# lauradarcy/gym-craftingworld

Hardware: AMD Instinct MI355X
Metric: env-steps/sec at 65536 envs, 1/2/4/8 MI355X; bit-exact vs CPU ref (higher is better)
Workload: dtype u8

## Files before the change

### gym_craftingworld_amd/_lib.py

```python
import ctypes as C
import os

_HERE = os.path.dirname(os.path.abspath(__file__))
LIB_PATH = os.path.join(_HERE, 'libcraftingworld.so')


def lib_path():
    return os.environ.get('CW_LIB_PATH') or LIB_PATH

CW_ABI_VERSION = 5
CW_MT_N = 624
CW_MAX_TASKS = 16
CW_MAX_MENUS = 256

CW_OK, CW_ERR_INVALID, CW_ERR_HIP, CW_ERR_STATE = 0, -1, -2, -3
CW_OBS_STATE, CW_OBS_PIXELS_FULL, CW_OBS_PIXELS_DIRTY = 0, 1, 2
CW_ACT_I32, CW_ACT_I64, CW_ACT_U8 = 0, 1, 2
CW_RASTER_RAY, CW_RASTER_ALT = 0, 1


class cw_task_menu(C.Structure):
    _fields_ = [('n_selected', C.c_int32), ('number_of_tasks', C.c_int32), ('stacking', C.c_int32),
                ('reward_subset', C.c_int32), ('selected_bits', C.c_int32 * CW_MAX_TASKS)]


class cw_config(C.Structure):
    _fields_ = [('abi_version', C.c_int32), ('num_envs', C.c_int32), ('size', C.c_int32),
                ('max_steps', C.c_int32), ('n_task_list', C.c_int32), ('fixed_init_state', C.c_int32),
                ('obs_mode', C.c_int32), ('auto_reset', C.c_int32), ('keep_terminal_obs', C.c_int32),
                ('raster', C.c_int32), ('host_outputs', C.c_int32), ('n_menus', C.c_int32),
                ('menus', C.POINTER(cw_task_menu)), ('env_menu', C.POINTER(C.c_uint8))]


class cw_buffer_table(C.Structure):
    _fields_ = [('obs', C.c_void_p), ('desired_goal', C.c_void_p), ('init_obs', C.c_void_p), ('terminal_obs', C.c_void_p),
                ('reward', C.c_void_p), ('done', C.c_void_p), ('achieved', C.c_void_p),
                ('desired', C.c_void_p), ('episode_length', C.c_void_p), ('episode_return', C.c_void_p), ('hdr', C.c_void_p),
                ('slot_pos', C.c_void_p), ('counters', C.c_void_p), ('frame_bytes', C.c_size_t),
                ('host_actions', C.c_void_p), ('host_onehot', C.c_void_p)]


class cw_state_view(C.Structure):
    _fields_ = [('grid', C.c_void_p), ('init_grid', C.c_void_p), ('goal_grid', C.c_void_p),
                ('agent_rc', C.c_void_p), ('init_agent_rc', C.c_void_p), ('goal_agent_rc', C.c_void_p),
                ('hold', C.c_void_p), ('achieved', C.c_void_p), ('desired', C.c_void_p),
                ('step_num', C.c_void_p), ('ep_no', C.c_void_p)]


class cw_profile(C.Structure):
    _fields_ = [('steps', C.c_int32), ('ms_step_kernel', C.c_float), ('ms_reset_kernel', C.c_float),
                ('ms_render_kernel', C.c_float), ('ms_render_kernel_max', C.c_float), ('ms_render_kernel_min', C.c_float),
                ('ms_render_kernel_median', C.c_float)]


class cw_tuner_state(C.Structure):
    _fields_ = [('period16', C.c_int32), ('period16_head', C.c_int32), ('period16_busy', C.c_int32), ('lookahead', C.c_int32), ('resident', C.c_int32),
                ('guard_slowdowns', C.c_int32)]


_VP = C.c_void_p
ABI = {
    'cw_create': (C.c_int, [C.POINTER(cw_config), C.c_int, C.POINTER(_VP)]),
    'cw_destroy': (C.c_int, [_VP]),
    'cw_seed_mt': (C.c_int, [_VP, _VP, _VP]),
    'cw_seed_int': (C.c_int, [_VP, _VP]),
    'cw_get_mt': (C.c_int, [_VP, _VP, _VP]),
    'cw_generate_fixed_states': (C.c_int, [_VP, _VP]),
    'cw_get_fixed_states': (C.c_int, [_VP, _VP]),
    'cw_reset': (C.c_int, [_VP, _VP]),
    'cw_step': (C.c_int, [_VP, _VP, C.c_int, _VP]),
    'cw_step_many': (C.c_int, [_VP, _VP, C.c_int, C.c_int32, _VP]),
    'cw_rollout': (C.c_int, [_VP, _VP, C.c_int32, _VP, _VP, _VP]),
    'cw_render': (C.c_int, [_VP, _VP, _VP]),
    'cw_render_onehot': (C.c_int, [_VP, _VP, C.c_int32, _VP, _VP]),
    'cw_export_grid': (C.c_int, [_VP, _VP, _VP]),
    'cw_export_onehot': (C.c_int, [_VP, _VP, _VP]),
    'cw_export_onehot_of': (C.c_int, [_VP, C.c_int, _VP, _VP]),
    'cw_get_state': (C.c_int, [_VP, C.POINTER(cw_state_view)]),
    'cw_set_state': (C.c_int, [_VP, C.POINTER(cw_state_view)]),
    'cw_checkpoint_bytes': (C.c_size_t, [_VP]),
    'cw_checkpoint_save': (C.c_int, [_VP, _VP, C.c_size_t]),
    'cw_checkpoint_load': (C.c_int, [_VP, _VP, C.c_size_t]),
    'cw_profile_begin': (C.c_int, [_VP, C.c_int]),
    'cw_profile_end': (C.c_int, [_VP, C.POINTER(cw_profile)]),
    'cw_tuner': (C.c_int, [_VP, C.POINTER(cw_tuner_state)]),
    'cw_step_resident': (C.c_int, [_VP, C.c_int32, C.c_int32]),
    'cw_resident_stop': (C.c_int, [_VP]),
    'cw_render_kernel_name': (C.c_char_p, [_VP]),
    'cw_buffers': (C.c_int, [_VP, C.POINTER(cw_buffer_table)]),
    'cw_synchronize': (C.c_int, [_VP, _VP]),
    'cw_num_envs': (C.c_int, [_VP]),
    'cw_abi_version': (C.c_int, []),
    'cw_last_error': (C.c_char_p, []),
}
class cwh_guard(C.Structure):
    _fields_ = [('rate', C.c_double), ('rate_top', C.c_double), ('ms_sum', C.c_double), ('prev_mean', C.c_double), ('ref_ms', C.c_double),
                ('ref_prev', C.c_double), ('ms_n', C.c_int32), ('late', C.c_int32), ('good', C.c_int32), ('slowdowns', C.c_int32),
                ('probes', C.c_int32), ('probe_need', C.c_int32), ('recover_need', C.c_int32), ('probing', C.c_int32), ('recovering', C.c_int32)]


class cwh_tuning(C.Structure):
    _fields_ = [(f, C.c_int32) for f in ('render_chunk_rounds', 'step_envs_per_wave', 'gather', 'gather_max_size', 'small_frame_bytes',
                                         'small_blocks_per_cu', 'small_launch_mb', 'reset_blocks_per_cu', 'guard', 'verbose', 'lookahead',
                                         'la_period', 'rollout_segment', 'pad')] + \
              [(f, C.c_double) for f in ('head_notch', 'busy_notch', 'period_ns', 'rate_tbs')]


cwh_lookup = C.CFUNCTYPE(_VP, _VP, C.c_char_p)

CWH_GUARD_NONE, CWH_GUARD_SLOWDOWN, CWH_GUARD_TRIAL_UP, CWH_GUARD_TRIAL_KEPT, CWH_GUARD_TRIAL_UNDONE = range(5)
CWH_CKPT_SECTIONS = 22

HOST_HELPERS = {
    'cwh_mt_from_numpy': (C.c_int, [_VP, C.c_int]),
    'cwh_mt_to_numpy': (None, [_VP, C.c_int, _VP]),
    'cwh_mt_init_genrand': (None, [_VP, C.c_uint32]),
    'cwh_mt_untwist': (None, [_VP]),
    'cwh_mt_rewind': (None, [_VP, C.POINTER(C.c_int32), C.c_uint32]),
    'cwh_dlpack_make': (_VP, [_VP, C.c_int, C.c_int, C.c_int, C.c_int, C.POINTER(C.c_int64)]),
    'cwh_slots_to_grid': (None, [_VP, C.c_uint32, C.c_int, _VP]),
    'cwh_ckpt_section_bytes': (C.c_int, [C.c_int64, C.c_int32, C.c_int32, C.POINTER(C.c_size_t), C.POINTER(C.c_uint64)]),
    'cwh_guard_init': (None, [C.POINTER(cwh_guard), C.c_double]),
    'cwh_guard_step': (C.c_int, [C.POINTER(cwh_guard), C.c_double, C.c_double]),
    'cwh_sweep_periods': (None, [C.c_double, C.c_int32, C.c_double, C.c_double, C.POINTER(C.c_int32), C.POINTER(C.c_int32), C.POINTER(C.c_int32)]),
    'cwh_guard_scheduled_ms': (C.c_double, [C.c_double, C.c_int32, C.c_int32, C.c_double]),
    'cwh_la_adapt': (C.c_int32, [C.c_int32, C.c_int32, C.c_uint64, C.POINTER(C.c_int32)]),
    'cwh_read_tuning': (None, [cwh_lookup, _VP, C.POINTER(cwh_tuning)]),
}


def bind_host_helpers(lib):
    for name, (res, args) in HOST_HELPERS.items():
        fn = getattr(lib, name)
        fn.restype = res
        fn.argtypes = args
    return lib

_libs = {}
_lib = None


class CraftingWorldError(RuntimeError):
    pass


def load():
    global _lib
    path = lib_path()
    if path in _libs:
        _lib = _libs[path]
        return _lib
    if not os.path.exists(path):
        raise CraftingWorldError(
            'HIP extension %s is missing; build it (python -c "import __graft_entry__ as g; g.build()"). '
            'There is no CPU fallback.' % path)
    try:
        import torch
    except ImportError:
        pass
    lib = C.CDLL(path)
    for table in (ABI, HOST_HELPERS):
        for name, (res, args) in table.items():
            fn = getattr(lib, name)
            fn.restype = res
            fn.argtypes = args
    if lib.cw_abi_version() != CW_ABI_VERSION:
        raise CraftingWorldError('%s ABI %d != binding %d' % (os.path.basename(path), lib.cw_abi_version(), CW_ABI_VERSION))
    _libs[path] = _lib = lib
    return lib


def check(rc, what, lib=None):
    if rc == CW_OK:
        return
    msg = ((lib or _lib or load()).cw_last_error() or b'').decode(errors='replace')
    if rc == CW_ERR_INVALID:
        raise ValueError('%s: %s' % (what, msg))
    raise CraftingWorldError('%s failed (%d): %s' % (what, rc, msg))
```

### gym_craftingworld_amd/csrc/cw_engine.cpp

```cpp
#include <hip/hip_runtime.h>

#include <cstdarg>
#include <climits>
#include <cstdio>
#include <cstdlib>
#include <cstring>
#include <new>
#include <algorithm>
#include <vector>

#include "../../include/craftingworld.h"
#include "cw_layout.h"
#include "cw_host.h"

extern "C" {
hipError_t cwk_launch_step(const CwParams *P, const CwTuning *T, const void *actions, int act_dtype, int obs_mode, int auto_reset, hipStream_t st,
                           hipEvent_t *ev);
hipError_t cwk_launch_refill(const CwParams *P, const CwTuning *T, int all_envs, hipStream_t st);
hipError_t cwk_launch_reset_all(const CwParams *P, const CwTuning *T, int obs_mode, hipStream_t st);
hipError_t cwk_launch_pool(const CwParams *P, const CwTuning *T, hipStream_t st);
hipError_t cwk_launch_seed(const CwParams *P, const uint32_t *seeds_dev, hipStream_t st);
hipError_t cwk_launch_resident(const CwParams *P, CwResident *R, uint32_t seq0, int paint_dirty, unsigned long long idle_ticks,
                               unsigned long long life_ticks, hipStream_t st);
hipError_t cwk_launch_render_onehot(const CwParams *P, const uint8_t *onehot, int n_states, uint16_t *out, hipStream_t st);
hipError_t cwk_launch_render_restore(const CwParams *P, const CwTuning *T, hipStream_t st);
hipError_t cwk_launch_rollout(const CwParams *P, const uint8_t *actions, int T, int32_t *rewards, uint8_t *dones, hipStream_t st);
hipError_t cwk_launch_render_ext(const CwParams *P, const CwTuning *T, uint8_t *out, hipStream_t st);
hipError_t cwk_launch_sweep_calib(const CwParams *P, const CwTuning *T, hipStream_t st);
void cwk_sweep_shape(const CwParams *P, const CwTuning *T, int *n_chunks, int *waves, int *jobs_per_wave);
hipError_t cwk_launch_idle(hipStream_t st);
hipError_t cwk_launch_export(const CwParams *P, const CwTuning *T, uint8_t *out, int onehot, int which, hipStream_t st);
}

#include <time.h>

static thread_local char g_err[512] = "";

static int fail(int code, const char *fmt, ...)
{
    va_list ap;
    va_start(ap, fmt);
    vsnprintf(g_err, sizeof(g_err), fmt, ap);
    va_end(ap);
    return code;
}

#define HIP_TRY(expr)                                                                           \
    do {                                                                                        \
        hipError_t _e = (expr);                                                                 \
        if (_e != hipSuccess)                                                                   \
            return fail(CW_ERR_HIP, "%s failed: %s (%s:%d)", #expr, hipGetErrorString(_e), __FILE__, __LINE__); \
    } while (0)

struct DeviceGuard {
    int prev = -1;
    bool ok = true;
    explicit DeviceGuard(int dev)
    {
        if (hipGetDevice(&prev) != hipSuccess) prev = -1;
        if (prev != dev) ok = (hipSetDevice(dev) == hipSuccess);
    }
    ~DeviceGuard()
    {
        int cur = -1;
        if (prev >= 0 && hipGetDevice(&cur) == hipSuccess && cur != prev) (void)hipSetDevice(prev);
    }
};

struct cw_engine {
    int device = 0;
    int obs_mode = 0;
    int auto_reset = 1;
    bool has_reset = false;
    CwParams P{};
    CwTuning tune{};
    std::vector<void *> allocs;
    std::vector<void *> host_allocs;
    int32_t *host_actions = nullptr;
    std::vector<CwMenuDev> menus;
    uint32_t *seed_scratch = nullptr;
    int n = 0, S = 0, ncell = 0, K = 0;
    CwResident *res = nullptr;
    hipStream_t res_stream = nullptr;
    bool res_running = false;
    uint32_t res_seq = 0;
    hipEvent_t last_work = nullptr;
    bool last_work_set = false;
    unsigned long long res_ticks_per_us = 100;
    std::vector<hipEvent_t> prof_ev;
    bool la_refill_all = false;
    unsigned la_steps = 0;
    unsigned la_period = 16;
    unsigned la_period_max = 16;
    bool la_adaptive = true;
    int rollout_segment = -1;
    unsigned long long *la_feedback = nullptr;
    unsigned long long la_slow_seen = 0;
    int32_t la_quiet = 0;
    bool in_step_many = false;
    bool capturing_now = false;
    int sweep_waves = 1024;
    double sweep_jobs = 0, sweep_rate = 0, sweep_beside_ms = 0;
    bool guard_on = false;
    double head_notch = 0.4, busy_notch = 0.75, tune_period_ns = -1, tune_rate_tbs = -1;
    bool tune_guard = true, tune_lookahead = true, verbose = false;
    enum { GUARD_RING = 32 };
    struct GuardSample { hipEvent_t ev[6]; int period16; } guard_ring[GUARD_RING] = {};
    unsigned guard_head = 0, guard_tail = 0;
    unsigned guard_step = 0;
    cwh_guard guard{};
    int prof_cap = 0, prof_n = 0;
    hipStream_t aux = nullptr;
    hipStream_t work[4] = {nullptr, nullptr, nullptr, nullptr};
    int n_work = 0;
    bool work_overflow = false;
    bool captured = false;
};
static inline bool stream_capturing(hipStream_t st)
{
    hipStreamCaptureStatus cap = hipStreamCaptureStatusNone;
    return hipStreamIsCapturing(st, &cap) == hipSuccess && cap != hipStreamCaptureStatusNone;
}
static inline void note_work(cw_engine *e, hipStream_t st)
{
    for (int i = 0; i < e->n_work; i++) if (e->work[i] == st) return;
    if (e->n_work < 4) e->work[e->n_work++] = st; else e->work_overflow = true;
}
static hipError_t quiesce(cw_engine *e)
{
    bool all = e->work_overflow || e->captured;
    for (int i = 0; i < e->n_work && !all; i++)
        if (hipStreamSynchronize(e->work[i]) != hipSuccess) { (void)hipGetLastError(); all = true; }
    e->n_work = 0;
    e->work_overflow = false;
    if (all) return hipDeviceSynchronize();
    return e->aux ? hipStreamSynchronize(e->aux) : hipSuccess;
}
struct AuxDrain {
    cw_engine *e;
    explicit AuxDrain(cw_engine *e_) : e(e_) {}
    ~AuxDrain() { if (e && e->aux) (void)hipStreamSynchronize(e->aux); }
};
static inline hipError_t aux_copy(cw_engine *e, void *dst, const void *src, size_t bytes, hipMemcpyKind kind)
{
    return bytes ? hipMemcpyAsync(dst, src, bytes, kind, e->aux) : hipSuccess;
}
static int la_period_for(int max_steps) { const int p = max_steps / 4; return p < 8 ? 8 : p > 64 ? 64 : p; }
static void la_adapt(cw_engine *e)
{
    const unsigned long long slow = __atomic_load_n(e->la_feedback, __ATOMIC_RELAXED);
    const unsigned long long delta = slow >= e->la_slow_seen ? slow - e->la_slow_seen : 0;
    e->la_slow_seen = slow;
    e->la_period = (unsigned)cwh_la_adapt((int32_t)e->la_period, (int32_t)e->la_period_max, delta, &e->la_quiet);
}

static int resident_park(cw_engine *e)
{
    if (!e->res_running) return CW_OK;
    const unsigned long long low = __atomic_load_n(&e->res->bell, __ATOMIC_RELAXED) & 0xFFFFFFFFull;
    __atomic_store_n(&e->res->bell, low | (1ull << 32), __ATOMIC_RELEASE);
    HIP_TRY(hipStreamSynchronize(e->res_stream));
    e->res_running = false;
    __atomic_store_n(&e->res->bell, low, __ATOMIC_RELEASE);
    __atomic_store_n(&e->res->exited, 0u, __ATOMIC_RELEASE);
    return CW_OK;
}
#define PARK(e) do { if ((e)->res_running) { const int _rc = resident_park(e); if (_rc != CW_OK) return _rc; } } while (0)


template <typename T>
static int dev_alloc(cw_engine *e, T **out, size_t count)
{
    void *p = nullptr;
    size_t bytes = count * sizeof(T);
    if (bytes == 0) bytes = 16;
    HIP_TRY(hipMalloc(&p, bytes));
    HIP_TRY(hipMemset(p, 0, bytes));
    e->allocs.push_back(p);
    *out = (T *)p;
    return CW_OK;
}

template <typename T>
static int host_alloc(cw_engine *e, T **out, size_t count)
{
    void *p = nullptr, *d = nullptr;
    size_t bytes = count * sizeof(T);
    if (bytes == 0) bytes = 16;
    HIP_TRY(hipHostMalloc(&p, bytes, hipHostMallocCoherent));
    e->host_allocs.push_back(p);
    memset(p, 0, bytes);
    HIP_TRY(hipHostGetDevicePointer(&d, p, 0));
    if (d != p) return fail(CW_ERR_HIP, "cw_create: mapped host memory has a different device address (no unified addressing)");
    *out = (T *)p;
    return CW_OK;
}

static void prof_free(cw_engine *e)
{
    for (hipEvent_t ev : e->prof_ev) (void)hipEventDestroy(ev);
    e->prof_ev.clear();
    e->prof_cap = e->prof_n = 0;
}

static int timed_render_stats(cw_engine *e, double *median, double *p90, double *mean = nullptr)
{
    enum { LAUNCHES = 24, SKIP = 4 };
    hipEvent_t evs[2 * LAUNCHES] = {};
    bool ok = true;
    for (hipEvent_t &ev : evs) ok = ok && hipEventCreate(&ev) == hipSuccess;
    for (int rep = 0; rep < LAUNCHES && ok; rep++)
        ok = hipEventRecord(evs[2 * rep], e->aux) == hipSuccess && cwk_launch_sweep_calib(&e->P, &e->tune, e->aux) == hipSuccess &&
             hipEventRecord(evs[2 * rep + 1], e->aux) == hipSuccess && cwk_launch_idle(e->aux) == hipSuccess;
    ok = ok && hipStreamSynchronize(e->aux) == hipSuccess;
    float ms[LAUNCHES];
    for (int rep = 0; rep < LAUNCHES && ok; rep++) ok = hipEventElapsedTime(&ms[rep], evs[2 * rep], evs[2 * rep + 1]) == hipSuccess;
    for (hipEvent_t &ev : evs) if (ev) (void)hipEventDestroy(ev);
    if (!ok) return fail(CW_ERR_HIP, "cw_create: render calibration failed");
    std::sort(ms + SKIP, ms + LAUNCHES);
    const int n = LAUNCHES - SKIP;
    *median = ms[SKIP + n / 2];
    *p90 = ms[SKIP + (9 * n) / 10 - 1];
    if (mean) { double acc = 0; for (int i = SKIP; i < LAUNCHES; i++) acc += ms[i]; *mean = acc / n; }
    return CW_OK;
}

static double sweep_period_ns(const cw_engine *e, double tb_per_s) { return (double)e->sweep_waves * 4096.0 / (tb_per_s * 1e12) * 1e9; }
static void set_sweep_rate(cw_engine *e, double tb_per_s)
{
    cwh_sweep_periods(tb_per_s, e->sweep_waves, e->head_notch, e->busy_notch, &e->tune.period16, &e->tune.period16_head, &e->tune.period16_busy);
}

static int calibrate_sweep(cw_engine *e)
{
    CwTuning &tn = e->tune;
    int n_chunks = 1, jobs_per_wave = 1;
    cwk_sweep_shape(&e->P, &tn, &n_chunks, &e->sweep_waves, &jobs_per_wave);
    e->sweep_jobs = (double)n_chunks * jobs_per_wave;
    if (e->tune_period_ns >= 0) {
        const double ns = e->tune_period_ns;
        set_sweep_rate(e, ns > 0 ? (double)e->sweep_waves * 4096.0 / (ns * 1e-9) * 1e-12 : 0.0);
        if (ns > 0) tn.period16 = (int)(ns * 1.6 + 0.5);
        return CW_OK;
    }
    set_sweep_rate(e, 7.0);
    if (e->host_actions) { set_sweep_rate(e, 0); return CW_OK; }
    if (e->obs_mode != CW_OBS_PIXELS_FULL || (double)e->n * e->P.frame_bytes < (double)(64ll << 20)) return CW_OK;
    static const double rates[] = {7.7, 7.4, 7.2, 7.0, 6.8, 6.6, 0.0};
    char log[1024] = "";
    size_t len = 0;
    int rc = CW_OK;
    double best_p90 = 0, med = 0, p90 = 0, mean = 0;
    rc = timed_render_stats(e, &med, &p90);
    set_sweep_rate(e, 6.4);
    if (rc == CW_OK) rc = timed_render_stats(e, &med, &p90);
    e->sweep_beside_ms = med - e->sweep_jobs * sweep_period_ns(e, 6.4) * 1e-6;
    if (e->tune_rate_tbs >= 0) e->sweep_rate = e->tune_rate_tbs;
    for (size_t i = 0; i < sizeof(rates) / sizeof(rates[0]) && rc == CW_OK && e->tune_rate_tbs < 0; i++) {
        set_sweep_rate(e, rates[i]);
        rc = timed_render_stats(e, &med, &p90, &mean);
        if (len < sizeof(log) - 56) len += (size_t)snprintf(log + len, sizeof(log) - len, " %.1f TB/s (%.0f ns): %.4f/%.4f/%.4f |", rates[i], tn.period16 / 1.6, med, p90, mean);
        if (rc == CW_OK && (best_p90 == 0 || p90 < 0.995 * best_p90)) { best_p90 = p90; e->sweep_rate = rates[i]; }
    }
    set_sweep_rate(e, e->sweep_rate);
    cwh_guard_init(&e->guard, e->sweep_rate);
    e->guard_on = rc == CW_OK && e->sweep_rate > 0 && e->auto_reset && e->tune_guard;
    if (e->guard_on)
        for (auto &smp : e->guard_ring)
            for (hipEvent_t &ev : smp.ev)
                if (hipEventCreate(&ev) != hipSuccess) e->guard_on = false;
    if (e->verbose)
        fprintf(stderr, "[craftingworld] sweep clock, ms per sweep (median/90th percentile/mean of 20; 0.0 TB/s = unclocked):%s -> %s%.0f ns\n", log,
                tn.period16 ? "" : "unclocked, ", tn.period16 / 1.6);
    return rc;
}

enum { CW_GUARD_EVERY = 64 };
static hipEvent_t *sweep_guard_tick(cw_engine *e, hipStream_t st)
{
    if (++e->guard_step % CW_GUARD_EVERY) return nullptr;
    while (e->guard_tail != e->guard_head && hipEventQuery(e->guard_ring[e->guard_tail % cw_engine::GUARD_RING].ev[5]) == hipSuccess) {
        cw_engine::GuardSample &smp = e->guard_ring[e->guard_tail++ % cw_engine::GUARD_RING];
        float ms = 0.f;
        if (hipEventElapsedTime(&ms, smp.ev[4], smp.ev[5]) != hipSuccess || ms <= 0.f || smp.period16 != e->tune.period16) continue;
        const double scheduled = cwh_guard_scheduled_ms(e->sweep_jobs, e->tune.period16, e->tune.period16_busy, e->sweep_beside_ms);
        const double rate_before = e->guard.rate, prev_mean = e->guard.prev_mean;
        const int recovering = e->guard.recovering;
        const int action = cwh_guard_step(&e->guard, ms, scheduled);
        if (e->guard.rate != rate_before) set_sweep_rate(e, e->guard.rate);
        if (e->verbose && action != CWH_GUARD_NONE) {
            static const char *what[] = {"", "three samples in a row late: a notch down", "trying a notch up", "the trial pays: kept", "the trial does not pay: undone"};
            fprintf(stderr, "[craftingworld] sweep clock: %s%s -- %.4f ms against %.4f scheduled (mean at the rate left %.4f): %.1f -> %.1f TB/s (%.0f ns)\n", what[action],
                    recovering ? " (on the way back to the best rate known)" : "", ms, scheduled, prev_mean, rate_before, e->guard.rate, e->tune.period16 / 1.6);
        }
    }
    if (e->guard_head - e->guard_tail >= (unsigned)cw_engine::GUARD_RING) return nullptr;
    cw_engine::GuardSample &slot = e->guard_ring[e->guard_head++ % cw_engine::GUARD_RING];
    slot.period16 = e->tune.period16;
    return slot.ev;
}

static void read_tuning(cw_engine *e)
{
    CwTuning &tn = e->tune;
    cwh_tuning t{};
    t.render_chunk_rounds = tn.render_chunk_rounds;
    t.step_envs_per_wave = tn.step_envs_per_wave;
    t.gather = tn.gather;
    t.gather_max_size = tn.gather_max_size;
    t.small_frame_bytes = tn.small_frame_bytes;
    t.small_blocks_per_cu = tn.small_blocks_per_cu;
    t.small_launch_mb = (int32_t)(tn.small_launch_bytes >> 20);
    t.reset_blocks_per_cu = tn.reset_blocks_per_cu;
    t.guard = 1;
    t.verbose = 0;
    t.lookahead = 1;
    t.la_period = 0;
    t.rollout_segment = e->rollout_segment;
    t.head_notch = e->head_notch;
    t.busy_notch = e->busy_notch;
    t.period_ns = -1;
    t.rate_tbs = -1;
    cwh_read_tuning([](void *, const char *k) -> const char * { return getenv(k); }, nullptr, &t);
    tn.render_chunk_rounds = t.render_chunk_rounds;
    tn.step_envs_per_wave = t.step_envs_per_wave;
    tn.gather = t.gather;
    tn.gather_max_size = t.gather_max_size;
    tn.small_frame_bytes = t.small_frame_bytes;
    tn.small_blocks_per_cu = t.small_blocks_per_cu;
    tn.small_launch_bytes = (long long)t.small_launch_mb << 20;
    tn.reset_blocks_per_cu = t.reset_blocks_per_cu;
    e->head_notch = t.head_notch;
    e->busy_notch = t.busy_notch;
    e->tune_period_ns = t.period_ns;
    e->tune_rate_tbs = t.rate_tbs;
    e->tune_guard = t.guard != 0;
    e->verbose = t.verbose != 0;
    e->tune_lookahead = t.lookahead != 0;
    e->la_adaptive = t.la_period == 0;
    e->la_period = e->la_period_max = (unsigned)(t.la_period ? t.la_period : la_period_for(e->P.max_steps));
    e->rollout_segment = t.rollout_segment;
}

extern "C" {

const char *cw_last_error(void) { return g_err; }
int cw_abi_version(void) { return CW_ABI_VERSION; }
int cw_num_envs(const cw_engine *e) { return e ? e->n : 0; }

int cw_create(const cw_config *cfg, int device, cw_engine **out)
{
    if (!cfg || !out) return fail(CW_ERR_INVALID, "cw_create: null argument");
    *out = nullptr;
    if (cfg->abi_version != CW_ABI_VERSION)
        return fail(CW_ERR_INVALID, "cw_create: abi_version %d != %d", cfg->abi_version, CW_ABI_VERSION);
    if (cfg->num_envs < 1) return fail(CW_ERR_INVALID, "cw_create: num_envs must be >= 1");
    if (cfg->size < 4 || cfg->size > 255)
        return fail(CW_ERR_INVALID, "cw_create: size must be in 4..255 (square grids only; non-square is a reference defect)");
    if (cfg->max_steps < 1 || cfg->max_steps > 65535) return fail(CW_ERR_INVALID, "cw_create: max_steps must be in 1..65535");
    if (cfg->n_task_list < 9 || cfg->n_task_list > CW_MAX_TASKS)
        return fail(CW_ERR_INVALID, "cw_create: len(task_list) must be in 9..%d", CW_MAX_TASKS);
    if (cfg->fixed_init_state < 0 || cfg->fixed_init_state > 64)
        return fail(CW_ERR_INVALID, "cw_create: fixed_init_state must be in 0..64");
    if (cfg->obs_mode < CW_OBS_STATE || cfg->obs_mode > CW_OBS_PIXELS_DIRTY) return fail(CW_ERR_INVALID, "cw_create: bad obs_mode");
    if (cfg->raster != CW_RASTER_RAY && cfg->raster != CW_RASTER_ALT) return fail(CW_ERR_INVALID, "cw_create: bad raster");
    if (cfg->n_menus < 1 || cfg->n_menus > CW_MAX_MENUS || !cfg->menus) return fail(CW_ERR_INVALID, "cw_create: n_menus must be in 1..%d", CW_MAX_MENUS);
    if ((double)cfg->num_envs * 48.0 * cfg->size * cfg->size > 1.0e12)
        return fail(CW_ERR_INVALID, "cw_create: num_envs x frame size exceeds 1 TB");

    std::vector<CwMenuDev> menus(cfg->n_menus);
    for (int m = 0; m < cfg->n_menus; m++) {
        const cw_task_menu &src = cfg->menus[m];
        if (src.n_selected < 1 || src.n_selected > CW_MAX_TASKS)
            return fail(CW_ERR_INVALID, "cw_create: menu %d: len(selected_tasks) must be in 1..%d", m, CW_MAX_TASKS);
        if (src.number_of_tasks < 1) return fail(CW_ERR_INVALID, "cw_create: menu %d: number_of_tasks must be >= 1", m);
        CwMenuDev d{};
        d.n_selected = src.n_selected;
        d.number_of_tasks = src.number_of_tasks > src.n_selected ? src.n_selected : src.number_of_tasks;
        d.stacking = src.stacking ? 1 : 0;
        d.reward_subset = src.reward_subset ? 1 : 0;
        for (int i = 0; i < src.n_selected; i++) {
            if (src.selected_bits[i] < 0 || src.selected_bits[i] >= cfg->n_task_list)
                return fail(CW_ERR_INVALID, "cw_create: menu %d: selected task %d is not in task_list", m, i);
            d.sel_bits |= (uint64_t)src.selected_bits[i] << (4 * i);
        }
        menus[m] = d;
    }
    if (cfg->env_menu)
        for (int i = 0; i < cfg->num_envs; i++)
            if (cfg->env_menu[i] >= cfg->n_menus) return fail(CW_ERR_INVALID, "cw_create: env_menu[%d] out of range", i);

    int ndev = 0;
    HIP_TRY(hipGetDeviceCount(&ndev));
    if (device < 0 || device >= ndev) return fail(CW_ERR_INVALID, "cw_create: device %d not present (%d devices)", device, ndev);
    DeviceGuard guard(device);
    if (!guard.ok) return fail(CW_ERR_HIP, "cw_create: hipSetDevice(%d) failed", device);

    cw_engine *e = new (std::nothrow) cw_engine();
    if (!e) return fail(CW_ERR_INVALID, "cw_create: out of host memory");
    e->device = device;
    e->obs_mode = cfg->obs_mode;
    e->auto_reset = cfg->auto_reset ? 1 : 0;
    e->n = cfg->num_envs;
    e->S = cfg->size;
    e->ncell = cfg->size * cfg->size;
    e->K = cfg->fixed_init_state;
    e->menus = menus;
    CwParams &P = e->P;
    const size_t N = (size_t)e->n;
    P.n_envs = e->n;
    P.size = e->S;
    P.ncell = e->ncell;
    P.max_steps = cfg->max_steps;
    read_tuning(e);
    hipDeviceProp_t prop;
    if (hipGetDeviceProperties(&prop, device) == hipSuccess && prop.multiProcessorCount > 0) e->tune.n_cu = prop.multiProcessorCount;
    P.task_mask = (1u << cfg->n_task_list) - 1u;
    P.pool_k = e->K;
    P.div_magic = (uint32_t)((1ull << 32) / (uint64_t)e->S) + 1u;
    P.raster = cfg->raster;
    P.frame_bytes = cfg->raster == CW_RASTER_ALT ? 27u * (uint32_t)e->S * (uint32_t)(e->S + 1) : 48u * (uint32_t)e->ncell;

    int rc = CW_OK;
#define ALLOC(field, count)                                     \
    if (rc == CW_OK) rc = dev_alloc(e, &P.field, (count))
    ALLOC(hdr, N);
    ALLOC(pos, N);
    ALLOC(init_pos, N);
    ALLOC(init_agent, N);
    ALLOC(goal_pos, N);
    ALLOC(goal_codes, N);
    ALLOC(goal_agent, N);
    ALLOC(ep_no, N);
    ALLOC(mt, N * CW_MT_N);
    ALLOC(mt_idx, N);
    ALLOC(pool, N * (size_t)e->K * 9);
    if (rc == CW_OK) rc = dev_alloc(e, &e->seed_scratch, N);
#define ALLOC_OUT(field, count)                                 \
    if (rc == CW_OK) rc = cfg->host_outputs ? host_alloc(e, &P.field, (count)) : dev_alloc(e, &P.field, (count))
    ALLOC_OUT(reward, N);
    ALLOC_OUT(done, N);
    ALLOC_OUT(achieved_out, N);
    ALLOC_OUT(desired_out, N);
    ALLOC_OUT(episode_length, N);
    ALLOC_OUT(episode_return, N);
    ALLOC(counters, 8);
    if (rc == CW_OK) {
        int pr_least = 0, pr_greatest = 0;
        if (hipDeviceGetStreamPriorityRange(&pr_least, &pr_greatest) != hipSuccess) pr_least = pr_greatest = 0;
        if (hipStreamCreateWithPriority(&e->aux, hipStreamNonBlocking, pr_greatest) != hipSuccess &&
            hipStreamCreateWithFlags(&e->aux, hipStreamNonBlocking) != hipSuccess)
            rc = fail(CW_ERR_HIP, "cw_create: no private stream");
    }
    if (cfg->obs_mode != CW_OBS_STATE) {
        ALLOC_OUT(obs, N * P.frame_bytes);
        ALLOC_OUT(desired_img, N * P.frame_bytes);
        ALLOC_OUT(init_img, N * P.frame_bytes);
        if (cfg->keep_terminal_obs && cfg->auto_reset) ALLOC_OUT(terminal_img, N * P.frame_bytes);
    }
    if (cfg->host_outputs && rc == CW_OK) rc = host_alloc(e, &e->host_actions, N);
    P.lookahead = (cfg->auto_reset && !cfg->host_outputs && e->tune_lookahead) ? 1 : 0;
    ALLOC(nx_init_pos, P.lookahead ? N * CW_LA_DEPTH : 1);
    ALLOC(nx_goal_pos, P.lookahead ? N * CW_LA_DEPTH : 1);
    ALLOC(nx_misc, P.lookahead ? N * CW_LA_DEPTH : 1);
    ALLOC(nx_ctl, P.lookahead ? N : 1);
    if (rc == CW_OK && P.lookahead && e->la_adaptive) {
        void *fb = nullptr;
        if (hipHostMalloc(&fb, 64, hipHostMallocCoherent) == hipSuccess) {
            memset(fb, 0, 64);
            e->host_allocs.push_back(fb);
            e->la_feedback = P.la_feedback = (unsigned long long *)fb;
        }
    }
#undef ALLOC_OUT
#undef ALLOC
    CwMenuDev *dmenus = nullptr;
    if (rc == CW_OK) rc = dev_alloc(e, &dmenus, menus.size());
    if (rc == CW_OK && hipMemcpy(dmenus, menus.data(), menus.size() * sizeof(CwMenuDev), hipMemcpyHostToDevice) != hipSuccess)
        rc = fail(CW_ERR_HIP, "cw_create: menu upload failed");
    P.menus = dmenus;
    if (rc == CW_OK) {
        std::vector<uint32_t> h(N * 4, 0u);
        for (size_t i = 0; i < N; i++) {
            h[i * 4 + 0] = (uint32_t)(cfg->env_menu ? cfg->env_menu[i] : 0) << 24;
            h[i * 4 + 3] = CW_CODES_INITIAL;
        }
        if (hipMemcpy(P.hdr, h.data(), h.size() * 4, hipMemcpyHostToDevice) != hipSuccess)
            rc = fail(CW_ERR_HIP, "cw_create: header upload failed");
    }
    if (rc != CW_OK) {
        if (e->aux) (void)hipStreamDestroy(e->aux);
        for (void *p : e->allocs) (void)hipFree(p);
        for (void *p : e->host_allocs) (void)hipHostFree(p);
        delete e;
        return rc;
    }
    if (cfg->host_outputs && e->n == 1 && !e->auto_reset && e->obs_mode != CW_OBS_PIXELS_FULL) {
        void *p = nullptr;
        if (hipHostMalloc(&p, sizeof(CwResident), hipHostMallocCoherent) == hipSuccess &&
            hipStreamCreateWithFlags(&e->res_stream, hipStreamNonBlocking) == hipSuccess) {
            memset(p, 0, sizeof(CwResident));
            e->host_allocs.push_back(p);
            e->res = (CwResident *)p;
            if (host_alloc(e, &e->P.res_onehot, (size_t)e->ncell * 12) != CW_OK) e->P.res_onehot = nullptr;
            int khz = 0;
            if (hipDeviceGetAttribute(&khz, hipDeviceAttributeWallClockRate, device) == hipSuccess && khz >= 1000) e->res_ticks_per_us = (unsigned long long)khz / 1000ull;
            if (hipEventCreateWithFlags(&e->last_work, hipEventDisableTiming) != hipSuccess) {
                e->last_work = nullptr;
                e->res = nullptr;
            }
        } else {
            if (p) (void)hipHostFree(p);
            e->res_stream = nullptr;
        }
    }
    *out = e;
    std::vector<uint32_t> seeds(N);
    for (size_t i = 0; i < N; i++) seeds[i] = (uint32_t)i;
    rc = cw_seed_int(e, seeds.data());
    if (rc == CW_OK) rc = calibrate_sweep(e);
    if (rc != CW_OK) {
        cw_destroy(e);
        *out = nullptr;
    }
    return rc;
}

int cw_destroy(cw_engine *e)
{
    if (!e) return CW_OK;
    DeviceGuard guard(e->device);
    if (!guard.ok) return fail(CW_ERR_HIP, "hipSetDevice(%d) failed", e->device);
    PARK(e);
    (void)resident_park(e);
    (void)quiesce(e);
    prof_free(e);
    if (e->aux) (void)hipStreamDestroy(e->aux);
    if (e->res_stream) (void)hipStreamDestroy(e->res_stream);
    if (e->last_work) (void)hipEventDestroy(e->last_work);
    for (auto &smp : e->guard_ring) for (hipEvent_t ev : smp.ev) if (ev) (void)hipEventDestroy(ev);
    for (void *p : e->allocs) (void)hipFree(p);
    for (void *p : e->host_allocs) (void)hipHostFree(p);
    delete e;
    return CW_OK;
}

static hipError_t lookahead_drop(cw_engine *e)
{
    if (!e->P.lookahead) return hipSuccess;
    hipError_t rc = hipMemsetAsync(e->P.nx_misc, 0, (size_t)e->n * CW_LA_DEPTH * sizeof(uint4), e->aux);
    if (rc == hipSuccess) rc = hipMemsetAsync(e->P.nx_ctl, 0, (size_t)e->n * sizeof(uint32_t), e->aux);
    e->la_refill_all = true;
    return rc;
}

int cw_seed_mt(cw_engine *e, const uint32_t *keys, const int32_t *pos)
{
    if (!e || !keys || !pos) return fail(CW_ERR_INVALID, "cw_seed_mt: null argument");
    DeviceGuard guard(e->device);
    if (!guard.ok) return fail(CW_ERR_HIP, "hipSetDevice(%d) failed", e->device);
    PARK(e);
    const size_t N = (size_t)e->n;
    for (size_t i = 0; i < N; i++)
        if (pos[i] < 0 || pos[i] > CW_MT_N) return fail(CW_ERR_INVALID, "cw_seed_mt: pos[%zu]=%d outside 0..624", i, pos[i]);
    HIP_TRY(quiesce(e));
    AuxDrain drain(e);
    HIP_TRY(aux_copy(e, e->P.mt, keys, N * CW_MT_N * sizeof(uint32_t), hipMemcpyHostToDevice));
    HIP_TRY(aux_copy(e, e->P.mt_idx, pos, N * sizeof(int32_t), hipMemcpyHostToDevice));
    HIP_TRY(cwk_launch_seed(&e->P, nullptr, e->aux));
    HIP_TRY(lookahead_drop(e));
    HIP_TRY(hipStreamSynchronize(e->aux));
    return CW_OK;
}

int cw_seed_int(cw_engine *e, const uint32_t *seeds)
{
    if (!e || !seeds) return fail(CW_ERR_INVALID, "cw_seed_int: null argument");
    DeviceGuard guard(e->device);
    if (!guard.ok) return fail(CW_ERR_HIP, "hipSetDevice(%d) failed", e->device);
    PARK(e);
    HIP_TRY(quiesce(e));
    AuxDrain drain(e);
    HIP_TRY(aux_copy(e, e->seed_scratch, seeds, (size_t)e->n * sizeof(uint32_t), hipMemcpyHostToDevice));
    HIP_TRY(cwk_launch_seed(&e->P, e->seed_scratch, e->aux));
    HIP_TRY(lookahead_drop(e));
    HIP_TRY(hipStreamSynchronize(e->aux));
    return CW_OK;
}

int cw_get_mt(cw_engine *e, uint32_t *keys, int32_t *pos)
{
    if (!e || !keys || !pos) return fail(CW_ERR_INVALID, "cw_get_mt: null argument");
    DeviceGuard guard(e->device);
    if (!guard.ok) return fail(CW_ERR_HIP, "hipSetDevice(%d) failed", e->device);
    PARK(e);
    const size_t N = (size_t)e->n;
    std::vector<uint32_t> words(N * CW_MT_N);
    std::vector<uint32_t> misc(e->P.lookahead ? N * 4 * CW_LA_DEPTH : 0);
    HIP_TRY(quiesce(e));
    AuxDrain drain(e);
    HIP_TRY(aux_copy(e, words.data(), e->P.mt, words.size() * sizeof(uint32_t), hipMemcpyDeviceToHost));
    HIP_TRY(aux_copy(e, pos, e->P.mt_idx, N * sizeof(int32_t), hipMemcpyDeviceToHost));
    if (e->P.lookahead) HIP_TRY(aux_copy(e, misc.data(), e->P.nx_misc, N * 16 * CW_LA_DEPTH, hipMemcpyDeviceToHost));
    HIP_TRY(hipStreamSynchronize(e->aux));
    for (size_t i = 0; i < N; i++) cwh_mt_to_numpy(&words[i * CW_MT_N], pos[i], keys + i * CW_MT_N);
    if (e->P.lookahead) {
        for (size_t i = 0; i < N; i++) {
            uint32_t ahead = 0;
            for (size_t d = 0; d < CW_LA_DEPTH; d++)
                if (misc[(d * N + i) * 4 + 2] >> 31) ahead += misc[(d * N + i) * 4 + 3];
            if (ahead) cwh_mt_rewind(keys + i * CW_MT_N, &pos[i], ahead);
        }
    }
    for (size_t i = 0; i < N; i++)
        if (pos[i] == 0) { cwh_mt_untwist(keys + i * CW_MT_N); pos[i] = CW_MT_N; }
    return CW_OK;
}

int cw_generate_fixed_states(cw_engine *e, cw_stream_t stream)
{
    if (!e) return fail(CW_ERR_INVALID, "cw_generate_fixed_states: null engine");
    if (e->K == 0) return CW_OK;
    DeviceGuard guard(e->device);
    if (!guard.ok) return fail(CW_ERR_HIP, "hipSetDevice(%d) failed", e->device);
    PARK(e);
    if (e->P.lookahead && e->has_reset) {
        std::vector<uint32_t> keys((size_t)e->n * CW_MT_N);
        std::vector<int32_t> pos((size_t)e->n);
        int rc = cw_get_mt(e, keys.data(), pos.data());
        if (rc == CW_OK) rc = cw_seed_mt(e, keys.data(), pos.data());
        if (rc != CW_OK) return rc;
    }
    HIP_TRY(cwk_launch_pool(&e->P, &e->tune, (hipStream_t)stream));
    HIP_TRY(hipStreamSynchronize((hipStream_t)stream));
    return CW_OK;
}

int cw_reset(cw_engine *e, cw_stream_t stream)
{
    if (!e) return fail(CW_ERR_INVALID, "cw_reset: null engine");
    DeviceGuard guard(e->device);
    if (!guard.ok) return fail(CW_ERR_HIP, "hipSetDevice(%d) failed", e->device);
    PARK(e);
    note_work(e, (hipStream_t)stream);
    HIP_TRY(cwk_launch_reset_all(&e->P, &e->tune, e->obs_mode, (hipStream_t)stream));
    if (e->P.lookahead) {
        HIP_TRY(cwk_launch_refill(&e->P, &e->tune, 1, (hipStream_t)stream));
        e->la_refill_all = false;
        e->la_steps = 0;
    }
    e->has_reset = true;
    if (e->res && hipEventRecord(e->last_work, (hipStream_t)stream) == hipSuccess) e->last_work_set = true;
    return CW_OK;
}

int cw_step(cw_engine *e, const void *actions, int action_dtype, cw_stream_t stream)
{
    if (!e || !actions) return fail(CW_ERR_INVALID, "cw_step: null argument");
    if (action_dtype < CW_ACT_I32 || action_dtype > CW_ACT_U8) return fail(CW_ERR_INVALID, "cw_step: bad action dtype %d", action_dtype);
    if (!e->has_reset) return fail(CW_ERR_STATE, "cw_step called before cw_reset");
    DeviceGuard guard(e->device);
    if (!guard.ok) return fail(CW_ERR_HIP, "hipSetDevice(%d) failed", e->device);
    PARK(e);
    const bool capturing = e->in_step_many ? e->capturing_now : stream_capturing((hipStream_t)stream);
    if (capturing) e->captured = true;
    else if (e->n_work != 1 || e->work[0] != (hipStream_t)stream) note_work(e, (hipStream_t)stream);
    hipEvent_t *ev = (e->prof_n < e->prof_cap) ? &e->prof_ev[(size_t)e->prof_n * 6] : nullptr;
    const bool profiled = ev != nullptr;
    if (e->guard_on && !ev && !capturing) ev = sweep_guard_tick(e, (hipStream_t)stream);
    if (capturing && e->P.lookahead && !e->la_refill_all && e->la_steps + 1 < e->la_period && !e->in_step_many) e->la_steps = e->la_period;
    if (e->P.lookahead && (e->la_refill_all || ++e->la_steps >= e->la_period)) {
        if (e->la_feedback && !capturing) la_adapt(e);
// ... 63 lines not shown
                const hipError_t he = hipStreamSynchronize(e->res_stream);
                e->res_running = false;
                const uint32_t now_acked = __atomic_load_n(&R->ack, __ATOMIC_ACQUIRE);
                __atomic_store_n(&R->bell, (unsigned long long)now_acked << 8, __ATOMIC_RELEASE);
                __atomic_store_n(&R->exited, 0u, __ATOMIC_RELEASE);
                e->res_seq = now_acked;
                if (he == hipSuccess && now_acked == seq) return CW_OK;
                return fail(CW_ERR_HIP, "cw_step_resident: no answer from the resident kernel within 5 s (request withdrawn, kernel parked: the step was not taken)");
            }
        }
    }
}

int cw_resident_stop(cw_engine *e)
{
    if (!e) return fail(CW_ERR_INVALID, "cw_resident_stop: null engine");
    DeviceGuard guard(e->device);
    if (!guard.ok) return fail(CW_ERR_HIP, "hipSetDevice(%d) failed", e->device);
    return resident_park(e);
}

int cw_rollout(cw_engine *e, const uint8_t *actions, int32_t n_steps, int32_t *rewards, uint8_t *dones, cw_stream_t stream)
{
    if (!e || !actions) return fail(CW_ERR_INVALID, "cw_rollout: null argument");
    if (n_steps < 1) return fail(CW_ERR_INVALID, "cw_rollout: n_steps must be >= 1");
    if (e->obs_mode != CW_OBS_STATE || !e->auto_reset)
        return fail(CW_ERR_INVALID, "cw_rollout needs obs_mode CW_OBS_STATE and auto_reset (frames are not painted by the persistent kernel)");
    if (!e->has_reset) return fail(CW_ERR_STATE, "cw_rollout called before cw_reset");
    DeviceGuard guard(e->device);
    if (!guard.ok) return fail(CW_ERR_HIP, "hipSetDevice(%d) failed", e->device);
    PARK(e);
    if (stream_capturing((hipStream_t)stream)) e->captured = true; else note_work(e, (hipStream_t)stream);
    const int32_t seg = !e->P.lookahead || e->rollout_segment == 0 ? n_steps : e->rollout_segment > 0 ? e->rollout_segment : (e->P.max_steps > 64 ? e->P.max_steps : 64);
    const size_t N = (size_t)e->n;
    for (int32_t t0 = 0; t0 < n_steps; t0 += seg) {
        if (e->P.lookahead) {
            HIP_TRY(cwk_launch_refill(&e->P, &e->tune, e->la_refill_all ? 1 : 0, (hipStream_t)stream));
            e->la_refill_all = false;
            e->la_steps = 0;
        }
        const int32_t n = n_steps - t0 < seg ? n_steps - t0 : seg;
        HIP_TRY(cwk_launch_rollout(&e->P, actions + (size_t)t0 * N, n, rewards ? rewards + (size_t)t0 * N : nullptr, dones ? dones + (size_t)t0 * N : nullptr,
                                   (hipStream_t)stream));
    }
    return CW_OK;
}

int cw_render(cw_engine *e, uint8_t *out_frames, cw_stream_t stream)
{
    if (!e || !out_frames) return fail(CW_ERR_INVALID, "cw_render: null argument");
    if (!e->has_reset) return fail(CW_ERR_STATE, "cw_render called before cw_reset");
    DeviceGuard guard(e->device);
    if (!guard.ok) return fail(CW_ERR_HIP, "hipSetDevice(%d) failed", e->device);
    PARK(e);
    note_work(e, (hipStream_t)stream);
    HIP_TRY(cwk_launch_render_ext(&e->P, &e->tune, out_frames, (hipStream_t)stream));
    return CW_OK;
}

int cw_render_onehot(cw_engine *e, const uint8_t *onehot, int32_t n_states, uint16_t *out_frames, cw_stream_t stream)
{
    if (!e || !onehot || !out_frames) return fail(CW_ERR_INVALID, "cw_render_onehot: null argument");
    if (n_states < 1) return fail(CW_ERR_INVALID, "cw_render_onehot: n_states must be >= 1");
    DeviceGuard guard(e->device);
    if (!guard.ok) return fail(CW_ERR_HIP, "hipSetDevice(%d) failed", e->device);
    PARK(e);
    note_work(e, (hipStream_t)stream);
    HIP_TRY(cwk_launch_render_onehot(&e->P, onehot, n_states, out_frames, (hipStream_t)stream));
    return CW_OK;
}

int cw_export_grid(cw_engine *e, uint8_t *out, cw_stream_t stream)
{
    if (!e || !out) return fail(CW_ERR_INVALID, "cw_export_grid: null argument");
    DeviceGuard guard(e->device);
    if (!guard.ok) return fail(CW_ERR_HIP, "hipSetDevice(%d) failed", e->device);
    PARK(e);
    note_work(e, (hipStream_t)stream);
    HIP_TRY(cwk_launch_export(&e->P, &e->tune, out, 0, 0, (hipStream_t)stream));
    return CW_OK;
}

int cw_export_onehot(cw_engine *e, uint8_t *out, cw_stream_t stream)
{
    if (!e || !out) return fail(CW_ERR_INVALID, "cw_export_onehot: null argument");
    DeviceGuard guard(e->device);
    if (!guard.ok) return fail(CW_ERR_HIP, "hipSetDevice(%d) failed", e->device);
    PARK(e);
    note_work(e, (hipStream_t)stream);
    HIP_TRY(cwk_launch_export(&e->P, &e->tune, out, 1, 0, (hipStream_t)stream));
    return CW_OK;
}

int cw_export_onehot_of(cw_engine *e, int which, uint8_t *out, cw_stream_t stream)
{
    if (!e || !out) return fail(CW_ERR_INVALID, "cw_export_onehot_of: null argument");
    if (which < CW_STATE_CURRENT || which > CW_STATE_INIT) return fail(CW_ERR_INVALID, "cw_export_onehot_of: which must be CW_STATE_*");
    if (!e->has_reset) return fail(CW_ERR_STATE, "cw_export_onehot_of called before cw_reset");
    DeviceGuard guard(e->device);
    if (!guard.ok) return fail(CW_ERR_HIP, "hipSetDevice(%d) failed", e->device);
    PARK(e);
    note_work(e, (hipStream_t)stream);
    HIP_TRY(cwk_launch_export(&e->P, &e->tune, out, 1, which, (hipStream_t)stream));
    return CW_OK;
}

int cw_profile_begin(cw_engine *e, int max_steps)
{
    if (!e || max_steps < 1 || max_steps > 100000) return fail(CW_ERR_INVALID, "cw_profile_begin: bad argument");
    DeviceGuard guard(e->device);
    if (!guard.ok) return fail(CW_ERR_HIP, "hipSetDevice(%d) failed", e->device);
    PARK(e);
    prof_free(e);
    e->prof_ev.resize((size_t)max_steps * 6);
    for (auto &ev : e->prof_ev) HIP_TRY(hipEventCreate(&ev));
    e->prof_cap = max_steps;
    return CW_OK;
}

int cw_profile_end(cw_engine *e, cw_profile *out)
{
    if (!e || !out) return fail(CW_ERR_INVALID, "cw_profile_end: null argument");
    DeviceGuard guard(e->device);
    if (!guard.ok) return fail(CW_ERR_HIP, "hipSetDevice(%d) failed", e->device);
    PARK(e);
    memset(out, 0, sizeof(*out));
    const int n = e->prof_n;
    if (n > 0) {
        const bool side_recorded = e->obs_mode != CW_OBS_PIXELS_FULL;
        for (int k = 0; k < 6; k++)
            if (side_recorded || k >= 4) HIP_TRY(hipEventSynchronize(e->prof_ev[(size_t)(n - 1) * 6 + k]));
        double acc[3] = {0, 0, 0};
        float rmax = 0.f, rmin = 1e30f;
        std::vector<float> render_ms;
        render_ms.reserve((size_t)n);
        for (int i = 0; i < n; i++)
            for (int k = 0; k < 3; k++) {
                if (k != 2 && !side_recorded) continue;
                float ms = 0.f;
                HIP_TRY(hipEventElapsedTime(&ms, e->prof_ev[(size_t)i * 6 + 2 * k], e->prof_ev[(size_t)i * 6 + 2 * k + 1]));
                acc[k] += ms;
                if (k == 2) { rmax = ms > rmax ? ms : rmax; rmin = ms < rmin ? ms : rmin; render_ms.push_back(ms); }
            }
        out->steps = n;
        out->ms_step_kernel = (float)(acc[0] / n);
        out->ms_reset_kernel = (float)(acc[1] / n);
        out->ms_render_kernel = (float)(acc[2] / n);
        out->ms_render_kernel_max = rmax;
        out->ms_render_kernel_min = rmin;
        std::sort(render_ms.begin(), render_ms.end());
        out->ms_render_kernel_median = render_ms.empty() ? 0.f : render_ms[render_ms.size() / 2];
    }
    prof_free(e);
    return CW_OK;
}

const char *cw_render_kernel_name(const cw_engine *e)
{
    if (!e || e->obs_mode == CW_OBS_STATE) return "";
    if (e->obs_mode == CW_OBS_PIXELS_DIRTY) return e->auto_reset ? "cw_step_fused_kernel" : "cw_step_kernel";
    if (e->tune.gather && e->P.raster == CW_RASTER_RAY && e->S <= e->tune.gather_max_size) return "cw_render_gather_kernel";
    return "cw_render_pieces_kernel";
}

int cw_tuner(const cw_engine *e, cw_tuner_state *out)
{
    if (!e || !out) return fail(CW_ERR_INVALID, "cw_tuner: null argument");
    out->period16 = e->tune.period16;
    out->period16_head = e->tune.period16_head;
    out->period16_busy = e->tune.period16_busy;
    out->lookahead = e->P.lookahead;
    out->resident = e->res ? 1 : 0;
    out->guard_slowdowns = e->guard_on ? e->guard.slowdowns : -1;
    return CW_OK;
}

int cw_buffers(cw_engine *e, cw_buffer_table *out)
{
    if (!e || !out) return fail(CW_ERR_INVALID, "cw_buffers: null argument");
    const CwParams &P = e->P;
    out->obs = P.obs;
    out->desired_goal = P.desired_img;
    out->init_obs = P.init_img;
    out->terminal_obs = P.terminal_img;
    out->reward = P.reward;
    out->done = P.done;
    out->achieved = P.achieved_out;
    out->desired = P.desired_out;
    out->episode_length = P.episode_length;
    out->episode_return = P.episode_return;
    out->hdr = (uint8_t *)P.hdr;
    out->slot_pos = (uint16_t *)P.pos;
    out->counters = (uint64_t *)P.counters;
    out->frame_bytes = P.frame_bytes;
    out->host_actions = e->host_actions;
    out->host_onehot = P.res_onehot;
    return CW_OK;
}

int cw_synchronize(cw_engine *e, cw_stream_t stream)
{
    if (!e) return fail(CW_ERR_INVALID, "cw_synchronize: null engine");
    DeviceGuard guard(e->device);
    if (!guard.ok) return fail(CW_ERR_HIP, "hipSetDevice(%d) failed", e->device);
    PARK(e);
    HIP_TRY(hipStreamSynchronize((hipStream_t)stream));
    for (int i = 0; i < e->n_work; i++)
        if (e->work[i] == (hipStream_t)stream) { e->work[i] = e->work[--e->n_work]; break; }
    return CW_OK;
}

int cw_get_fixed_states(cw_engine *e, uint16_t *out)
{
    if (!e || !out) return fail(CW_ERR_INVALID, "cw_get_fixed_states: null argument");
    if (e->K == 0) return fail(CW_ERR_INVALID, "cw_get_fixed_states: the engine was created with fixed_init_state = 0");
    DeviceGuard guard(e->device);
    if (!guard.ok) return fail(CW_ERR_HIP, "hipSetDevice(%d) failed", e->device);
    PARK(e);
    HIP_TRY(quiesce(e));
    AuxDrain drain(e);
    HIP_TRY(aux_copy(e, out, e->P.pool, (size_t)e->n * e->K * 9 * sizeof(uint16_t), hipMemcpyDeviceToHost));
    HIP_TRY(hipStreamSynchronize(e->aux));
    return CW_OK;
}

int cw_get_state(cw_engine *e, cw_state_view *v)
{
    if (!e || !v) return fail(CW_ERR_INVALID, "cw_get_state: null argument");
    DeviceGuard guard(e->device);
    if (!guard.ok) return fail(CW_ERR_HIP, "hipSetDevice(%d) failed", e->device);
    PARK(e);
    const size_t N = (size_t)e->n;
    const int S = e->S, nc = e->ncell;
    std::vector<uint32_t> hdr(N * 4), goal_codes(N);
    std::vector<uint16_t> pos(N * 8), ipos(N * 8), gpos(N * 8), iagent(N), gagent(N);
    std::vector<int32_t> epno(N);
    HIP_TRY(quiesce(e));
    AuxDrain drain(e);
    HIP_TRY(aux_copy(e, hdr.data(), e->P.hdr, N * 16, hipMemcpyDeviceToHost));
    HIP_TRY(aux_copy(e, pos.data(), e->P.pos, N * 16, hipMemcpyDeviceToHost));
    HIP_TRY(aux_copy(e, ipos.data(), e->P.init_pos, N * 16, hipMemcpyDeviceToHost));
    HIP_TRY(aux_copy(e, gpos.data(), e->P.goal_pos, N * 16, hipMemcpyDeviceToHost));
    HIP_TRY(aux_copy(e, goal_codes.data(), e->P.goal_codes, N * 4, hipMemcpyDeviceToHost));
    HIP_TRY(aux_copy(e, iagent.data(), e->P.init_agent, N * 2, hipMemcpyDeviceToHost));
    HIP_TRY(aux_copy(e, gagent.data(), e->P.goal_agent, N * 2, hipMemcpyDeviceToHost));
    HIP_TRY(aux_copy(e, epno.data(), e->P.ep_no, N * 4, hipMemcpyDeviceToHost));
    HIP_TRY(hipStreamSynchronize(e->aux));
    for (size_t i = 0; i < N; i++) {
        const uint32_t *h = &hdr[i * 4];
        if (v->grid) cwh_slots_to_grid(&pos[i * 8], h[3], nc, v->grid + i * nc);
        if (v->init_grid) cwh_slots_to_grid(&ipos[i * 8], CW_CODES_INITIAL, nc, v->init_grid + i * nc);
        if (v->goal_grid) cwh_slots_to_grid(&gpos[i * 8], goal_codes[i], nc, v->goal_grid + i * nc);
        if (v->agent_rc) { v->agent_rc[i * 2] = h[0] & 0xFF; v->agent_rc[i * 2 + 1] = (h[0] >> 8) & 0xFF; }
        if (v->init_agent_rc) { v->init_agent_rc[i * 2] = (uint8_t)(iagent[i] / S); v->init_agent_rc[i * 2 + 1] = (uint8_t)(iagent[i] % S); }
        if (v->goal_agent_rc) { v->goal_agent_rc[i * 2] = (uint8_t)(gagent[i] / S); v->goal_agent_rc[i * 2 + 1] = (uint8_t)(gagent[i] % S); }
        if (v->hold) v->hold[i] = (h[0] >> 16) & 0xFF;
        if (v->achieved) v->achieved[i] = (uint16_t)(h[1] & 0xFFFF);
        if (v->desired) v->desired[i] = (uint16_t)(h[1] >> 16);
        if (v->step_num) v->step_num[i] = (int32_t)(h[2] & 0xFFFF);
        if (v->ep_no) v->ep_no[i] = epno[i];
    }
    return CW_OK;
}

int cw_set_state(cw_engine *e, const cw_state_view *v)
{
    if (!e || !v) return fail(CW_ERR_INVALID, "cw_set_state: null argument");
    if (!e->has_reset) return fail(CW_ERR_STATE, "cw_set_state called before cw_reset");
    DeviceGuard guard(e->device);
    if (!guard.ok) return fail(CW_ERR_HIP, "hipSetDevice(%d) failed", e->device);
    PARK(e);
    const size_t N = (size_t)e->n;
    const int S = e->S, nc = e->ncell;
    std::vector<uint32_t> hdr(N * 4);
    std::vector<uint16_t> pos(N * 8), ipos(N * 8), gpos, gagent, iagent;
    std::vector<uint32_t> gcodes;
    std::vector<int32_t> epno(N);
    const bool restore_episode = v->goal_grid || v->goal_agent_rc || v->init_agent_rc;
    HIP_TRY(quiesce(e));
    AuxDrain drain(e);
    if (restore_episode) {
        gpos.resize(N * 8); gagent.resize(N); iagent.resize(N); gcodes.resize(N);
        HIP_TRY(aux_copy(e, gpos.data(), e->P.goal_pos, N * 16, hipMemcpyDeviceToHost));
        HIP_TRY(aux_copy(e, gcodes.data(), e->P.goal_codes, N * 4, hipMemcpyDeviceToHost));
        HIP_TRY(aux_copy(e, gagent.data(), e->P.goal_agent, N * 2, hipMemcpyDeviceToHost));
        HIP_TRY(aux_copy(e, iagent.data(), e->P.init_agent, N * 2, hipMemcpyDeviceToHost));
    }
    HIP_TRY(aux_copy(e, hdr.data(), e->P.hdr, N * 16, hipMemcpyDeviceToHost));
    HIP_TRY(aux_copy(e, pos.data(), e->P.pos, N * 16, hipMemcpyDeviceToHost));
    HIP_TRY(aux_copy(e, ipos.data(), e->P.init_pos, N * 16, hipMemcpyDeviceToHost));
    HIP_TRY(aux_copy(e, epno.data(), e->P.ep_no, N * 4, hipMemcpyDeviceToHost));
    HIP_TRY(hipStreamSynchronize(e->aux));
    for (size_t i = 0; i < N; i++) {
        uint32_t *h = &hdr[i * 4];
        uint32_t hold = (h[0] >> 16) & 0xFF;
        if (v->hold) {
            if (v->hold[i] > 3) return fail(CW_ERR_INVALID, "cw_set_state: hold[%zu]=%d outside 0..3", i, v->hold[i]);
            hold = v->hold[i];
        }
        if (v->agent_rc) {
            if (v->agent_rc[i * 2] >= S || v->agent_rc[i * 2 + 1] >= S) return fail(CW_ERR_INVALID, "cw_set_state: agent of env %zu off the grid", i);
            h[0] = (h[0] & 0xFFFF0000u) | v->agent_rc[i * 2] | ((uint32_t)v->agent_rc[i * 2 + 1] << 8);
        }
        if (v->grid) {
            uint32_t codes = 0;
            int k = 0;
            const uint8_t *g = v->grid + i * nc;
            for (int c = 0; c < nc; c++) {
                if (g[c] == 0) continue;
                if (g[c] > 8) return fail(CW_ERR_INVALID, "cw_set_state: env %zu cell %d has code %d > 8", i, c, g[c]);
                if (k >= 8) return fail(CW_ERR_INVALID, "cw_set_state: env %zu has more than 8 objects (outside the reference's reachable states)", i);
                pos[i * 8 + k] = (uint16_t)c;
                codes |= (uint32_t)g[c] << (4 * k);
                k++;
            }
            if (hold) {
                if (k >= 8) return fail(CW_ERR_INVALID, "cw_set_state: env %zu: 8 objects on the grid plus a held one", i);
                pos[i * 8 + k] = CW_POS_HELD;
                codes |= hold << (4 * k);
                k++;
            }
            for (; k < 8; k++) pos[i * 8 + k] = CW_POS_GONE;
            h[3] = codes;
        } else if (v->hold) {
            return fail(CW_ERR_INVALID, "cw_set_state: hold given without grid");
        }
        h[0] = (h[0] & 0xFF00FFFFu) | (hold << 16);
        if (v->init_grid) {
            const uint8_t *g = v->init_grid + i * nc;
            for (int k = 0; k < 8; k++) ipos[i * 8 + k] = CW_POS_GONE;
            for (int c = 0; c < nc; c++) {
                if (g[c] == 0) continue;
                if (g[c] > 8) return fail(CW_ERR_INVALID, "cw_set_state: env %zu init cell %d has code %d > 8", i, c, g[c]);
                if (ipos[i * 8 + g[c] - 1] != CW_POS_GONE)
                    return fail(CW_ERR_INVALID, "cw_set_state: env %zu init grid holds object %d twice (sample_state places one of each, ray.py:605-608)", i, g[c]);
                ipos[i * 8 + g[c] - 1] = (uint16_t)c;
            }
        }
        if (v->goal_grid) {
            const uint8_t *g = v->goal_grid + i * nc;
            uint32_t codes = 0;
            int k = 0;
            for (int c = 0; c < nc; c++) {
                if (g[c] == 0) continue;
                if (g[c] > 8 || k >= 8) return fail(CW_ERR_INVALID, "cw_set_state: env %zu goal grid: code > 8 or more than 8 objects", i);
                gpos[i * 8 + k] = (uint16_t)c;
                codes |= (uint32_t)g[c] << (4 * k);
                k++;
            }
            for (; k < 8; k++) gpos[i * 8 + k] = CW_POS_GONE;
            gcodes[i] = codes;
        }
        if (v->goal_agent_rc) {
            if (v->goal_agent_rc[i * 2] >= S || v->goal_agent_rc[i * 2 + 1] >= S) return fail(CW_ERR_INVALID, "cw_set_state: goal agent of env %zu off the grid", i);
            gagent[i] = (uint16_t)(v->goal_agent_rc[i * 2] * S + v->goal_agent_rc[i * 2 + 1]);
        }
        if (v->init_agent_rc) {
            if (v->init_agent_rc[i * 2] >= S || v->init_agent_rc[i * 2 + 1] >= S) return fail(CW_ERR_INVALID, "cw_set_state: init agent of env %zu off the grid", i);
            iagent[i] = (uint16_t)(v->init_agent_rc[i * 2] * S + v->init_agent_rc[i * 2 + 1]);
        }
        if (v->achieved) h[1] = (h[1] & 0xFFFF0000u) | v->achieved[i];
        if (v->desired) h[1] = (h[1] & 0x0000FFFFu) | ((uint32_t)v->desired[i] << 16);
        if (v->step_num) {
// ... 168 lines not shown
```

### gym_craftingworld_amd/csrc/cw_host.cpp

```cpp
#include "cw_host.h"

#include <algorithm>
#include <cerrno>
#include <climits>
#include <cmath>
#include <cstdlib>
#include <cstring>

static inline uint32_t mt_twist(uint32_t cur, uint32_t nxt, uint32_t far)
{
    const uint32_t y = (cur & 0x80000000u) | (nxt & 0x7fffffffu);
    return far ^ (y >> 1) ^ ((y & 1u) ? 0x9908b0dfu : 0u);
}

extern "C" {

int cwh_mt_from_numpy(uint32_t *s, int pos)
{
    if (pos < 0) pos = 0;
    if (pos > CWH_MT_N) pos = CWH_MT_N;
    for (int k = 0; k < pos; k++)
        s[k] = mt_twist(s[k], s[(k + 1) % CWH_MT_N], s[(k + 397) % CWH_MT_N]);
    return pos % CWH_MT_N;
}
// ... 93 lines not shown
        if (pos[k] < (uint32_t)ncell) grid[pos[k]] = (uint8_t)((codes >> (4 * k)) & 15u);
}

int cwh_ckpt_section_bytes(int64_t n, int32_t k, int32_t la_depth, size_t *sizes, uint64_t *total)
{
    const size_t N = n > 0 ? (size_t)n : 0, K = k > 0 ? (size_t)k : 0, D = la_depth > 0 ? (size_t)la_depth : 0, la = D ? 1 : 0;
    const size_t sz[CWH_CKPT_SECTIONS] = {N * 16, N * 16, N * 16, N * 16, N * 4, N * 2, N * 2, N * 4, N * CWH_MT_N * 4, N * 4, N * K * 9 * 2,
                                          N * 4, N, N * 2, N * 2, N * 4, N * 4, 5 * 8,
                                          D * N * 16, D * N * 16, D * N * 16, la * N * 4};
    uint64_t sum = 0;
    for (int i = 0; i < CWH_CKPT_SECTIONS; i++) { if (sizes) sizes[i] = sz[i]; sum += sz[i]; }
    if (total) *total = sum;
    return CWH_CKPT_SECTIONS;
}

static double period_ns(int32_t sweep_waves, double tb_per_s) { return (double)sweep_waves * 4096.0 / (tb_per_s * 1e12) * 1e9; }
void cwh_sweep_periods(double rate, int32_t sweep_waves, double head_notch, double busy_notch, int32_t *period16, int32_t *period16_head, int32_t *period16_busy)
{
    const double head = rate - head_notch > CWH_GUARD_RATE_FLOOR ? rate - head_notch : CWH_GUARD_RATE_FLOOR;
    const double busy = rate - busy_notch > CWH_GUARD_RATE_FLOOR ? rate - busy_notch : CWH_GUARD_RATE_FLOOR;
    *period16 = rate > 0 ? (int32_t)(period_ns(sweep_waves, rate) * 1.6 + 0.5) : 0;
    *period16_head = rate > 0 ? (int32_t)(period_ns(sweep_waves, head) * 1.6 + 0.5) : 0;
    *period16_busy = rate > 0 ? (int32_t)(period_ns(sweep_waves, busy) * 1.6 + 0.5) : 0;
}
double cwh_guard_scheduled_ms(double sweep_jobs, int32_t period16, int32_t period16_busy, double beside_ms)
{
    return (sweep_jobs * (period16 / 1.6) + CWH_HEAD_JOBS * ((period16_busy - period16) / 1.6)) * 1e-6 + beside_ms;
}

static void guard_set_rate(cwh_guard *g, double rate)
{
    g->rate = rate;
    g->ms_sum = 0;
    g->ms_n = 0;
    g->good = g->late = 0;
    g->ref_ms = 0;
}
void cwh_guard_init(cwh_guard *g, double rate)
{
    memset(g, 0, sizeof(*g));
    g->rate = g->rate_top = rate;
    g->probe_need = CWH_GUARD_RECOVER;
    g->recover_need = CWH_GUARD_RECOVER;
}
int cwh_guard_step(cwh_guard *g, double ms, double scheduled)
{
    const double ref = std::max(scheduled, g->probing ? g->prev_mean : g->ref_ms);
    const bool late = ms > (g->probing ? 1.15 : 1.06) * ref;
    g->late = late ? g->late + 1 : 0;
    g->good = late ? std::max(0, g->good - 8) : g->good + 1;
    if (g->ms_n >= 128) { g->ms_sum *= 0.5; g->ms_n /= 2; }
    g->ms_sum += ms;
    g->ms_n++;
    const bool verdict_due = g->probing && g->ms_n >= CWH_GUARD_PROBE_SAMPLES;
    const double mean = g->ms_sum / g->ms_n;
    if (g->probing && (g->late >= 3 || (verdict_due && mean >= 0.998 * g->prev_mean))) {
        const double ref_prev = g->ref_prev;
        guard_set_rate(g, g->rate - CWH_GUARD_NOTCH);
        g->ref_ms = ref_prev;
        int32_t &need = g->recovering ? g->recover_need : g->probe_need;
        need = std::min(2 * need, (int32_t)CWH_GUARD_NEED_MAX);
        g->probing = g->recovering = 0;
        return CWH_GUARD_TRIAL_UNDONE;
    }
    if (verdict_due) {
        if (g->recovering) g->recover_need = CWH_GUARD_RECOVER;
        else { g->rate_top = g->rate; g->probe_need = CWH_GUARD_RECOVER / 4; }
        g->ref_ms = mean;
        g->probing = g->recovering = 0;
        return CWH_GUARD_TRIAL_KEPT;
    }
    if (!g->probing && g->late >= 3 && g->rate > CWH_GUARD_RATE_FLOOR + 0.1) {
        guard_set_rate(g, g->rate - CWH_GUARD_NOTCH);
        g->slowdowns++;
        return CWH_GUARD_SLOWDOWN;
    }
    if (!g->probing && g->ms_n >= CWH_GUARD_PROBE_SAMPLES && g->rate + 0.05 < CWH_GUARD_RATE_CEILING &&
        g->good >= (g->rate + 0.1 < g->rate_top ? g->recover_need : g->probe_need)) {
        g->recovering = g->rate + 0.1 < g->rate_top;
        g->prev_mean = mean;
        g->ref_prev = g->ref_ms;
        guard_set_rate(g, std::min(g->rate + CWH_GUARD_NOTCH, CWH_GUARD_RATE_CEILING));
        g->probing = 1;
        if (!g->recovering) g->probes++;
        return CWH_GUARD_TRIAL_UP;
    }
    return CWH_GUARD_NONE;
}

int32_t cwh_la_adapt(int32_t period, int32_t period_max, uint64_t slow_delta, int32_t *quiet)
{
    if (slow_delta * 8ull > (uint64_t)period) {
        *quiet = 0;
        if (period > CWH_LA_PERIOD_MIN) period = period / 2 < CWH_LA_PERIOD_MIN ? CWH_LA_PERIOD_MIN : period / 2;
    } else if (slow_delta * 32ull <= (uint64_t)period && ++*quiet >= CWH_LA_QUIET) {
        *quiet = 0;
        if (period < period_max) period = period * 2 > period_max ? period_max : period * 2;
    }
    return period;
}

}

static bool tail_is_blank(const char *end)
{
    while (*end == ' ' || (*end >= '\t' && *end <= '\r')) end++;
    return *end == '\0';
}
static void tune_int(cwh_lookup lookup, void *ctx, const char *name, int32_t *field, long lo, long hi)
{
    const char *s = lookup(ctx, name);
    if (!s) return;
    char *end = nullptr;
    errno = 0;
    const long v = strtol(s, &end, 10);
    if (end == s || errno == ERANGE || !tail_is_blank(end) || v < lo || v > hi) return;
    *field = (int32_t)v;
}
static void tune_real(cwh_lookup lookup, void *ctx, const char *name, double *field, double lo)
{
    const char *s = lookup(ctx, name);
    if (!s) return;
    char *end = nullptr;
    errno = 0;
    const double v = strtod(s, &end);
    if (end == s || errno == ERANGE || !tail_is_blank(end) || !std::isfinite(v) || v < lo) return;
    *field = v;
}

extern "C" void cwh_read_tuning(cwh_lookup lookup, void *ctx, cwh_tuning *t)
{
    tune_int(lookup, ctx, "CW_TUNE_RENDER_CHUNK_ROUNDS", &t->render_chunk_rounds, 0, INT32_MAX);
    int32_t epw = t->step_envs_per_wave;
    tune_int(lookup, ctx, "CW_TUNE_STEP_ENVS_PER_WAVE", &epw, 8, 64);
    if (epw == 8 || epw == 16 || epw == 32 || epw == 64) t->step_envs_per_wave = epw;
    tune_int(lookup, ctx, "CW_TUNE_GATHER", &t->gather, INT32_MIN, INT32_MAX);
    tune_int(lookup, ctx, "CW_TUNE_GATHER_MAX_SIZE", &t->gather_max_size, 0, 9);
    tune_int(lookup, ctx, "CW_TUNE_SMALL_FRAME_BYTES", &t->small_frame_bytes, 0, INT32_MAX);
    tune_int(lookup, ctx, "CW_TUNE_SMALL_BLOCKS", &t->small_blocks_per_cu, 1, 8);
    tune_int(lookup, ctx, "CW_TUNE_SMALL_LAUNCH_MB", &t->small_launch_mb, 0, INT32_MAX);
    tune_int(lookup, ctx, "CW_TUNE_RESET_BLOCKS", &t->reset_blocks_per_cu, 1, 16);
    tune_real(lookup, ctx, "CW_TUNE_HEAD_NOTCH", &t->head_notch, 0);
    tune_real(lookup, ctx, "CW_TUNE_BUSY_NOTCH", &t->busy_notch, 0);
    tune_real(lookup, ctx, "CW_TUNE_PERIOD_NS", &t->period_ns, 0);
    tune_real(lookup, ctx, "CW_TUNE_RATE_TBS", &t->rate_tbs, 0);
    tune_int(lookup, ctx, "CW_TUNE_GUARD", &t->guard, INT32_MIN, INT32_MAX);
    t->guard = t->guard != 0;
    if (lookup(ctx, "CW_TUNE_VERBOSE")) t->verbose = 1;
    tune_int(lookup, ctx, "CW_TUNE_LOOKAHEAD", &t->lookahead, INT32_MIN, INT32_MAX);
    t->lookahead = t->lookahead != 0;
    tune_int(lookup, ctx, "CW_TUNE_LA_PERIOD", &t->la_period, 1, INT32_MAX);
    tune_int(lookup, ctx, "CW_TUNE_ROLLOUT_SEGMENT", &t->rollout_segment, -1, INT32_MAX);
}
```

### gym_craftingworld_amd/csrc/cw_host.h

```cpp
#pragma once
#include <stddef.h>
#include <stdint.h>

#define CWH_MT_N 624

#ifdef __cplusplus
extern "C" {
#endif

int cwh_mt_from_numpy(uint32_t *s, int pos);
void cwh_mt_to_numpy(const uint32_t *s, int idx, uint32_t *key);
void cwh_mt_untwist(uint32_t *key);
void cwh_mt_rewind(uint32_t *key, int32_t *pos, uint32_t n);
void cwh_mt_init_genrand(uint32_t *s, uint32_t seed);

void *cwh_dlpack_make(void *data, int device_id, int code, int bits, int ndim, const int64_t *shape);

void cwh_slots_to_grid(const uint16_t *pos, uint32_t codes, int ncell, uint8_t *grid);

#define CWH_CKPT_SECTIONS 22
int cwh_ckpt_section_bytes(int64_t n, int32_t k, int32_t la_depth, size_t *sizes, uint64_t *total);

typedef struct cwh_guard {
    double rate;
    double rate_top;
    double ms_sum;
    double prev_mean;
    double ref_ms;
    double ref_prev;
    int32_t ms_n;
    int32_t late;
    int32_t good;
    int32_t slowdowns;
    int32_t probes;
    int32_t probe_need;
    int32_t recover_need;
    int32_t probing;
    int32_t recovering;
} cwh_guard;

enum { CWH_GUARD_NONE = 0, CWH_GUARD_SLOWDOWN = 1, CWH_GUARD_TRIAL_UP = 2, CWH_GUARD_TRIAL_KEPT = 3, CWH_GUARD_TRIAL_UNDONE = 4 };
#define CWH_GUARD_RECOVER 64
#define CWH_GUARD_PROBE_SAMPLES 32
#define CWH_GUARD_NEED_MAX 2048
#define CWH_GUARD_RATE_FLOOR 5.0
#define CWH_GUARD_RATE_CEILING 7.7
#define CWH_GUARD_NOTCH 0.2

void cwh_guard_init(cwh_guard *g, double rate);
int cwh_guard_step(cwh_guard *g, double ms, double scheduled_ms);
#define CWH_HEAD_JOBS 64
void cwh_sweep_periods(double rate, int32_t sweep_waves, double head_notch, double busy_notch, int32_t *period16, int32_t *period16_head, int32_t *period16_busy);
double cwh_guard_scheduled_ms(double sweep_jobs, int32_t period16, int32_t period16_busy, double beside_ms);

#define CWH_LA_PERIOD_MIN 8
#define CWH_LA_QUIET 8
int32_t cwh_la_adapt(int32_t period, int32_t period_max, uint64_t slow_delta, int32_t *quiet);

typedef struct cwh_tuning {
    int32_t render_chunk_rounds;
    int32_t step_envs_per_wave;
    int32_t gather;
    int32_t gather_max_size;
    int32_t small_frame_bytes;
    int32_t small_blocks_per_cu;
    int32_t small_launch_mb;
    int32_t reset_blocks_per_cu;
    int32_t guard;
    int32_t verbose;
    int32_t lookahead;
    int32_t la_period;
    int32_t rollout_segment;
    int32_t pad;
    double head_notch;
    double busy_notch;
    double period_ns;
    double rate_tbs;
} cwh_tuning;
typedef const char *(*cwh_lookup)(void *ctx, const char *name);
void cwh_read_tuning(cwh_lookup lookup, void *ctx, cwh_tuning *t);

#ifdef __cplusplus
}
#endif
```

### gym_craftingworld_amd/csrc/cw_kernels.hip

```cpp
#include <hip/hip_runtime.h>
#include <stdint.h>

#include "cw_layout.h"
#include "cw_mt.h"

#define CW_WAVE 64
#define CW_BALLOT(p) __builtin_amdgcn_ballot_w64(p)
#define CW_ALT_FRAME_PACE 2

#ifdef CW_TRACE
__device__ unsigned long long cw_trace_buf[1024 * 8];
#define CW_STAMP(env, k) do { if (lane == 0) { cw_trace_buf[((env) & 1023) * 8 + (k)] = wall_clock64(); \
                                               if ((k) == 0 || (k) == 5) cw_trace_buf[((env) & 1023) * 8 + 6 + ((k) ? 1 : 0)] = clock64(); } } while (0)
extern "C" hipError_t cwk_trace_read(unsigned long long *dst) { return hipMemcpyFromSymbol(dst, HIP_SYMBOL(cw_trace_buf), sizeof(cw_trace_buf)); }
#else
#define CW_STAMP(env, k) do { } while (0)
#endif

enum { EMPTY = 0, STICKS = 1, AXE = 2, HAMMER = 3, ROCK = 4, TREE = 5, BREAD = 6, HOUSE = 7, WHEAT = 8 };
enum { T_MAKEBREAD = 0, T_EATBREAD = 1, T_BUILDHOUSE = 2, T_CHOPTREE = 3, T_CHOPROCK = 4,
       T_GOTOHOUSE = 5, T_MOVEAXE = 6, T_MOVEHAMMER = 7, T_MOVESTICKS = 8 };

typedef uint32_t u32x3 __attribute__((ext_vector_type(3)));
typedef u32x3 u32x3_a4 __attribute__((aligned(4)));
// ... 763 lines not shown
        while (m) {
            const int l = __builtin_ctzll(m);
            m &= m - 1;
            const int env = base + l;
            const uint32_t ctl = __builtin_amdgcn_readlane(v_ctl, l);
            const uint32_t v_hx = P.hdr[env].x;
            const uint32_t head = ctl & 0xFFu;
            for (uint32_t k = 0; k < CW_LA_DEPTH; k++) {
                const uint32_t slot = head + k >= CW_LA_DEPTH ? head + k - CW_LA_DEPTH : head + k;
                if (__builtin_amdgcn_readfirstlane(P.nx_misc[(size_t)slot * P.n_envs + env].z) >> 31) continue;
                const CwResetOut r = reset_env_wave(P, env, [&]() { return __builtin_amdgcn_readfirstlane(v_hx) >> 24; }, s_mt[wave_in_block], lane);
                if (lane == 0) store_next_record(P, env, (int)slot, r);
            }
            if ((ctl & CW_CTL_QUEUED) && lane == 0) P.nx_ctl[env] = head;
        }
    }
}

__global__ __launch_bounds__(CW_RESET_WAVES *CW_WAVE) void cw_rollout_kernel(CwParams P, const uint8_t *actions, int T,
                                                                             int32_t *rewards, uint8_t *dones, int epw)
{
    __shared__ uint32_t s_mt[CW_RESET_WAVES][CW_MT_WORDS];
    const int lane = threadIdx.x & (CW_WAVE - 1);
    const int wave_in_block = __builtin_amdgcn_readfirstlane(threadIdx.x / CW_WAVE);
    const int wave = blockIdx.x * CW_RESET_WAVES + wave_in_block;
    const int env0 = wave * epw;
    if (env0 >= P.n_envs) return;
    const int env = env0 + lane;
    const bool live = lane < epw && env < P.n_envs;
    const int e = live ? env : env0;
    uint4 h = P.hdr[e];
    uint32_t sp[8];
    unpack_pos(P.pos[e], sp);
    uint4 ip = P.init_pos[e];
    uint32_t ctl = P.lookahead ? P.nx_ctl[e] : 0u;
    unsigned long long n_done = 0, n_succ = 0, n_inv = 0;
    int reward = -1;
    bool done = false;
    uint32_t achieved = 0, desired = 0, step_num = 0;
    for (int t = 0; t < T; t++) {
        const int a = actions[(size_t)t * P.n_envs + e];
        const CwStepOut o = step_env(P, h, sp, a, [&]() { return ip; });
        reward = o.reward; done = o.done; achieved = o.achieved; desired = o.desired; step_num = o.step_num;
        if (live) {
            if (rewards) rewards[(size_t)t * P.n_envs + env] = o.reward;
            if (dones) dones[(size_t)t * P.n_envs + env] = o.done ? 1 : 0;
        }
        const unsigned long long m_all = CW_BALLOT(live && o.done);
        n_done += __popcll(m_all);
        n_succ += __popcll(CW_BALLOT(live && o.success));
        n_inv += __popcll(CW_BALLOT(live && o.invalid));
        if (m_all && live && o.done) { P.episode_length[env] = (int32_t)o.step_num; P.episode_return[env] = episode_return_of(P, o); }
        bool popped = false;
        const uint32_t ctl_was = ctl;
        if (live && o.done && P.lookahead) {
            popped = pop_next_episode(P, env, ctl, h, sp, true);
            if (popped) { ip = pack_pos(sp); ctl = ((ctl & 0xFFu) + 1u == CW_LA_DEPTH ? 0u : (ctl & 0xFFu) + 1u) | CW_CTL_QUEUED; }
        }
        const unsigned long long m_pop = CW_BALLOT(popped);
        unsigned long long m = m_all & ~m_pop;
        while (m) {
            const int l = __builtin_ctzll(m);
            m &= m - 1;
            const int env_l = env0 + l;
            const uint32_t menu_id = __builtin_amdgcn_readlane(h.x, l) >> 24;
            const CwResetOut r = reset_env_wave(P, env_l, [&]() { return menu_id; }, s_mt[wave_in_block], lane);
            if (lane == 0) {
                store_episode_records(P, env_l, r, true);
                if (P.lookahead) note_slow_reset(P, env_l, __builtin_amdgcn_readlane(ctl_was, l));
            }
            if (lane == l) {
                h = reset_header(P, r, menu_id);
                unpack_pos(r.init_pos, sp);
                ip = r.init_pos;
                ctl |= CW_CTL_QUEUED;
            }
        }
    }
    if (live) {
        P.hdr[env] = h;
        P.pos[env] = pack_pos(sp);
        P.reward[env] = reward;
        P.done[env] = done ? 1 : 0;
        P.achieved_out[env] = (uint16_t)achieved;
        P.desired_out[env] = (uint16_t)desired;
        (void)step_num;
    }
    if (lane == 0) {
        atomicAdd(&P.counters[0], (unsigned long long)min(epw, P.n_envs - env0) * (unsigned long long)T);
        if (n_done) atomicAdd(&P.counters[1], n_done);
        if (n_succ) atomicAdd(&P.counters[2], n_succ);
        if (n_inv) atomicAdd(&P.counters[3], n_inv);
    }
}

__global__ __launch_bounds__(CW_WAVE) void cw_resident_kernel(CwParams P, CwResident *R, uint32_t seq0, int paint_dirty,
                                                              unsigned long long idle_ticks, unsigned long long life_ticks)
{
    const int lane = threadIdx.x;
    uint4 h = P.hdr[0];
    uint32_t sp[8];
    unpack_pos(P.pos[0], sp);
    const uint4 ip = P.init_pos[0];
    uint32_t last = seq0;
    const unsigned long long t_start = wall_clock64();
    unsigned long long t_last = t_start;
    uint32_t reason = 0;
    for (;;) {
        const unsigned long long bell = __hip_atomic_load(&R->bell, __ATOMIC_ACQUIRE, __HIP_MEMORY_SCOPE_SYSTEM);
        const uint32_t d = (uint32_t)bell;
        const uint32_t seq = d >> 8;
        if (seq != last) {
            if (lane == 0) {
                const int a = (int)(d & 0x7Fu);
                const CwStepOut o = step_env(P, h, sp, a, [&]() { return ip; });
                P.hdr[0] = h;
                P.pos[0] = pack_pos(sp);
                store_step_outputs(P, 0, o);
                if (paint_dirty && o.changed) paint_changed_cells(P, 0, h, sp, o);
                atomicAdd(&P.counters[0], 1ull);
                if (o.done) atomicAdd(&P.counters[1], 1ull);
                if (o.success) atomicAdd(&P.counters[2], 1ull);
                if (o.invalid) atomicAdd(&P.counters[3], 1ull);
            }
            if (P.res_onehot && (d & 0x80u)) {
                const uint32_t hx = __builtin_amdgcn_readlane(h.x, 0), codes = __builtin_amdgcn_readlane(h.w, 0);
                uint32_t bp[8];
#pragma unroll
                for (int k = 0; k < 8; k++) bp[k] = __builtin_amdgcn_readlane(sp[k], 0);
                const uint32_t agent_cell = agent_cell_of(P, hx), hold = hold_of(hx);
                for (int cell = lane; cell < P.ncell; cell += CW_WAVE) {
                    const uint32_t code = code_of(codes, slot_at(bp, (uint32_t)cell));
                    uint32_t bits = code ? (1u << (code - 1)) : 0u;
                    if ((uint32_t)cell == agent_cell) bits |= (1u << 8) | (hold ? (1u << (8 + hold)) : 0u);
                    *(u32x3_a4 *)(P.res_onehot + 12 * cell) = onehot_dwords(bits);
                }
            }
            __threadfence_system();
            if (lane == 0) __hip_atomic_store(&R->ack, seq, __ATOMIC_RELEASE, __HIP_MEMORY_SCOPE_SYSTEM);
            last = seq;
            t_last = wall_clock64();
            continue;
        }
        const unsigned long long now = wall_clock64();
        if (bell >> 32) { reason = 1; break; }
        if (now - t_last > idle_ticks) { reason = 2; break; }
        if (now - t_start > life_ticks) { reason = 3; break; }
    }
    if (lane == 0) __hip_atomic_store(&R->exited, reason | (last << 8), __ATOMIC_RELEASE, __HIP_MEMORY_SCOPE_SYSTEM);
}

struct CwPaintJob { uint4 pos; uint32_t codes, agent_hold_kind, env, pad; };
enum { CW_JOB_INIT = 0, CW_JOB_GOAL = 1, CW_JOB_TERMINAL = 2 };
template <int PAINT, bool TERM>
__device__ __forceinline__ void fused_step(const CwParams &P, const void *actions, int act_dtype, int epw, int wave, uint32_t *s_mt_wave,
                                           CwPaintJob *s_jobs, int *s_njobs, int *s_cnt )
{
    constexpr int paint = PAINT;
    const int lane = threadIdx.x & (CW_WAVE - 1);
    const int wave_in_block = __builtin_amdgcn_readfirstlane(threadIdx.x / CW_WAVE);
    const int env0 = wave * epw;
    const bool wave_live = env0 < P.n_envs;
    const int env = env0 + lane;
    const bool live = wave_live && lane < epw && env < P.n_envs;
    const int e = live ? env : (wave_live ? env0 : 0);
    const int a = load_action(actions, act_dtype, e);
    uint4 h = P.hdr[e];
    uint32_t sp[8];
    unpack_pos(P.pos[e], sp);
    const uint4 ip = P.init_pos[e];
    const uint32_t ctl = P.lookahead ? P.nx_ctl[e] : 0u;
    if (threadIdx.x == 0) { *s_njobs = 0; s_cnt[0] = s_cnt[1] = s_cnt[2] = 0; }
    __syncthreads();
    const CwStepOut o = step_env(P, h, sp, a, [&]() { return ip; });
    const bool done = live && o.done;
    if (live) {
        store_step_outputs(P, env, o);
        if constexpr (PAINT == 1) { if (o.changed && !o.done) paint_changed_cells(P, env, h, sp, o); }
    }
    const uint4 h_last = h;
    uint32_t sp_last[8];
    if constexpr (TERM) {
#pragma unroll
        for (int k = 0; k < 8; k++) sp_last[k] = sp[k];
    }
    const unsigned long long m_all = CW_BALLOT(done);
    const unsigned long long m_succ = CW_BALLOT(live && o.success);
    const unsigned long long m_inv = CW_BALLOT(live && o.invalid);
    if (lane == 0 && (m_all | m_inv)) {
        if (m_all) atomicAdd(&s_cnt[0], (int)__popcll(m_all));
        if (m_succ) atomicAdd(&s_cnt[1], (int)__popcll(m_succ));
        if (m_inv) atomicAdd(&s_cnt[2], (int)__popcll(m_inv));
    }
    bool popped = false;
    CwGoalState goal;
    goal.pos = make_uint4(0, 0, 0, 0); goal.codes = 0; goal.agent = 0;
    if (done && P.lookahead) popped = pop_next_episode(P, env, ctl, h, sp, true, PAINT != 0 ? &goal : nullptr);
    const unsigned long long m_pop = CW_BALLOT(popped);
    __syncthreads();
    if (threadIdx.x == 0) {
        if (blockIdx.x == 0) atomicAdd(&P.counters[0], (unsigned long long)P.n_envs);
        if (s_cnt[0]) atomicAdd(&P.counters[1], (unsigned long long)s_cnt[0]);
        if (s_cnt[1]) atomicAdd(&P.counters[2], (unsigned long long)s_cnt[1]);
        if (s_cnt[2]) atomicAdd(&P.counters[3], (unsigned long long)s_cnt[2]);
    }
    constexpr int jpe = TERM ? 3 : 2;
    int jmine = 0;
    if constexpr (PAINT != 0) {
        int jbase = 0;
        if (m_all) {
            if (lane == 0) jbase = atomicAdd(s_njobs, jpe * __popcll(m_all));
            jbase = __shfl(jbase, 0);
        }
        jmine = jbase + jpe * __popcll(m_all & ((1ull << lane) - 1ull));
        if constexpr (TERM) if (done) {
            CwPaintJob &j = s_jobs[jmine + 2];
            j.pos = pack_pos(sp_last);
            j.codes = h_last.w;
            j.agent_hold_kind = agent_cell_of(P, h_last.x) | (hold_of(h_last.x) << 16) | (CW_JOB_TERMINAL << 24);
            j.env = (uint32_t)env;
        }
        if (popped) {
            CwPaintJob &j0 = s_jobs[jmine], &j1 = s_jobs[jmine + 1];
            j0.pos = pack_pos(sp);
            j0.codes = CW_CODES_INITIAL;
            j0.agent_hold_kind = agent_cell_of(P, h.x) | (CW_JOB_INIT << 24);
            j0.env = (uint32_t)env;
            j1.pos = goal.pos;
            j1.codes = goal.codes;
            j1.agent_hold_kind = goal.agent | (CW_JOB_GOAL << 24);
            j1.env = (uint32_t)env;
        }
    }
    unsigned long long m = m_all & ~m_pop;
    while (m) {
        const int l = __builtin_ctzll(m);
        m &= m - 1;
        const int env_l = env0 + l;
        const uint32_t menu_id = __builtin_amdgcn_readlane(h.x, l) >> 24;
        const CwResetOut r = reset_env_wave(P, env_l, [&]() { return menu_id; }, s_mt_wave, lane);
        if (lane == 0) {
            store_episode_records(P, env_l, r, true);
            if (P.lookahead) note_slow_reset(P, env_l, __builtin_amdgcn_readlane(ctl, l));
        }
        if (lane == l) {
            h = reset_header(P, r, menu_id);
            unpack_pos(r.init_pos, sp);
            if constexpr (PAINT != 0) {
                CwPaintJob &j0 = s_jobs[jmine], &j1 = s_jobs[jmine + 1];
                j0.pos = r.init_pos; j0.codes = CW_CODES_INITIAL; j0.agent_hold_kind = r.init_agent | (CW_JOB_INIT << 24); j0.env = (uint32_t)env_l;
                j1.pos = r.goal_pos; j1.codes = r.goal_codes; j1.agent_hold_kind = r.goal_agent | (CW_JOB_GOAL << 24); j1.env = (uint32_t)env_l;
            }
        }
    }
    if (live) {
        P.hdr[env] = h;
        P.pos[env] = pack_pos(sp);
    }
    if constexpr (PAINT == 0) return;
    __syncthreads();
    const int n_jobs = *s_njobs;
    for (int jq = wave_in_block; jq < n_jobs; jq += CW_RESET_WAVES) {
        const CwPaintJob &j = s_jobs[jq];
        uint32_t jp[8];
        unpack_pos(make_uint4(__builtin_amdgcn_readfirstlane(j.pos.x), __builtin_amdgcn_readfirstlane(j.pos.y), __builtin_amdgcn_readfirstlane(j.pos.z),
                              __builtin_amdgcn_readfirstlane(j.pos.w)), jp);
        const uint32_t codes = __builtin_amdgcn_readfirstlane(j.codes), ahk = __builtin_amdgcn_readfirstlane(j.agent_hold_kind);
        const size_t off = (size_t)__builtin_amdgcn_readfirstlane(j.env) * P.frame_bytes;
        const uint32_t kind = ahk >> 24;
        uint8_t *d0, *d1 = nullptr;
        if (kind == CW_JOB_INIT) { d0 = P.init_img + off; if (paint == 1) d1 = P.obs + off; }
        else if (kind == CW_JOB_GOAL) d0 = P.desired_img + off;
        else d0 = P.terminal_img + off;
        paint_state_frame(P, d0, jp, codes, ahk & 0xFFFFu, (ahk >> 16) & 0xFFu, lane, d1);
    }
}
template <int PAINT, bool TERM>
__global__ __launch_bounds__(CW_RESET_WAVES *CW_WAVE) void cw_step_fused_kernel(CwParams P, const void *actions, int act_dtype, int epw)
{
    __shared__ uint32_t s_mt[CW_RESET_WAVES][CW_MT_WORDS];
    __shared__ CwPaintJob s_jobs[PAINT != 0 ? CW_RESET_WAVES * CW_WAVE * (TERM ? 3 : 2) : 1];
    __shared__ int s_njobs;
    __shared__ int s_cnt[3];
    const int wave_in_block = __builtin_amdgcn_readfirstlane(threadIdx.x / CW_WAVE);
    fused_step<PAINT, TERM>(P, actions, act_dtype, epw, blockIdx.x * CW_RESET_WAVES + wave_in_block, s_mt[wave_in_block], s_jobs, &s_njobs, s_cnt);
}
typedef void (*CwStepFusedKernel)(CwParams, const void *, int, int);
static CwStepFusedKernel cw_step_fused_variant(int paint, bool term)
{
    if (paint == 0) return cw_step_fused_kernel<0, false>;
    if (paint == 1) return term ? cw_step_fused_kernel<1, true> : cw_step_fused_kernel<1, false>;
    return term ? cw_step_fused_kernel<2, true> : cw_step_fused_kernel<2, false>;
}

__global__ __launch_bounds__(CW_RESET_WAVES *CW_WAVE) void cw_pool_kernel(CwParams P)
{
    __shared__ uint32_t s_mt[CW_RESET_WAVES][CW_MT_WORDS];
    const int lane = threadIdx.x & (CW_WAVE - 1);
    const int wave_in_block = __builtin_amdgcn_readfirstlane(threadIdx.x / CW_WAVE);
    const int n_waves = gridDim.x * CW_RESET_WAVES;
    for (int env = blockIdx.x * CW_RESET_WAVES + wave_in_block; env < P.n_envs; env += n_waves) {
        CwMtWave mt;
        mt.load(s_mt[wave_in_block], P.mt + (size_t)env * CW_MT_WORDS, P.mt_idx + env, lane);
        for (int k = 0; k < P.pool_k; k++) {
            const uint32_t v_tok = shuffle_tokens(mt, P.ncell);
            uint16_t *pp = P.pool + ((size_t)env * P.pool_k + k) * 9;
            if (lane < 9) pp[lane] = (uint16_t)v_tok;
        }
        mt.store(P.mt + (size_t)env * CW_MT_WORDS, P.mt_idx + env, lane);
    }
}

__global__ __launch_bounds__(256) void cw_render_frames_kernel(CwParams P, uint8_t *out)
{
    const int lane = threadIdx.x & (CW_WAVE - 1);
    const int wave = (blockIdx.x * blockDim.x + threadIdx.x) / CW_WAVE;
    const int n_waves = gridDim.x * blockDim.x / CW_WAVE;
    for (int env = wave; env < P.n_envs; env += n_waves) {
        uint32_t sp[8], codes, agent_cell, hold;
        load_state_uniform(P, env, CW_SRC_CURRENT, sp, codes, agent_cell, hold);
        paint_state_frame(P, out + (size_t)env * P.frame_bytes, sp, codes, agent_cell, hold, lane);
    }
}

#define CW_PIECE 4096u
#define CW_PIECE_STORES 4
#ifndef CW_HEAD_JOBS
#define CW_HEAD_JOBS 64
#endif
#define CW_BUSY_FINISHED 16ull
__device__ __attribute__((noinline)) void piece_fill_partial(uint8_t *dst_base, uint32_t a0, uint32_t a1, int lane)
{
    for (int s = 0; s < CW_PIECE_STORES; s++) {
        const uint32_t c = a0 + 1024u * s + 16u * lane;
        if (c + 16u <= a1) *(uint4 *)(dst_base + c) = make_uint4(0, 0, 0, 0);
        else for (uint32_t b = c; b < a1; b++) dst_base[b] = 0;
    }
}
template <int RASTER, int FPJ>
__device__ __forceinline__ void render_pieces(const CwParams &P, uint8_t *frames, int src, int period16, int head_extra16, int env_lo, int env_n)
{
    constexpr int JPB = CW_WAVE / FPJ;
    const int lane = threadIdx.x & (CW_WAVE - 1);
    const int wpb = blockDim.x / CW_WAVE;
    const int wave_in_block = __builtin_amdgcn_readfirstlane(threadIdx.x / CW_WAVE);
    const int n_waves = (int)gridDim.x * wpb;
    const int wave = (int)blockIdx.x * wpb + wave_in_block;
    const uint32_t S = (uint32_t)P.size, FB = P.frame_bytes, row_bytes = (RASTER == 1 ? 9u : 12u) * S;
    uint8_t *const dst_base = frames + (size_t)env_lo * FB;
    const uint32_t total = (uint32_t)env_n * FB;
    const int n_jobs = (int)((total + CW_PIECE - 1u) / CW_PIECE);
    if (wave >= n_jobs) return;
    const int q_mine = (n_jobs + n_waves - 1) / n_waves;
    const uint32_t half = (uint32_t)lane >> 5, pl = (uint32_t)lane & 31u;
    const uint32_t slot = RASTER == 1 ? (pl & 7u) : (pl >> 2), dy = pl & 3u;
    const uint32_t v_cpv = cpv_color(lane & 15), v_rgb = rgb_of_code((uint32_t)lane & 15u);
    const uint32_t m_slot = (RASTER != 1 || pl < 8u) ? 0xFFFFFFFFu : 0u, m_agent = pl == 8u ? 0xFFFFFFFFu : 0u, m_held = pl == 9u ? 0xFFFFFFFFu : 0u;
    const uint32_t m_flag = (pl >= 10u && pl < 19u) ? 0xFFFFFFFFu : 0u;
    const uint32_t sh_pos = 16u * (slot & 1u), sh_item = 4u * slot;
    const uint32_t m_p0 = (slot & 6u) == 0u ? 0xFFFFFFFFu : 0u, m_p1 = (slot & 6u) == 2u ? 0xFFFFFFFFu : 0u;
    const uint32_t m_p2 = (slot & 6u) == 4u ? 0xFFFFFFFFu : 0u, m_p3 = (slot & 6u) == 6u ? 0xFFFFFFFFu : 0u;
    const uint32_t fj = pl >= 10u ? pl - 10u : 0u, fjr = (fj >= 6u) ? 2u : (fj >= 3u) ? 1u : 0u;
    const uint32_t off_flag = (3u * S + fjr) * row_bytes + 9u + 3u * (fj - 3u * fjr);
    const bool marks = slot == 0u && (dy == 1u || dy == 2u);
    __builtin_amdgcn_s_setprio(3);
    struct Rec { int f; uint32_t hx, hw, o2; uint4 p; };
    auto fetch = [&](int base) {
        Rec r;
        const int i = base + lane / FPJ;
        const int id = i * n_waves + wave;
        r.f = -1; r.hx = 0; r.hw = 0; r.o2 = 0;
        r.p = make_uint4(0, 0, 0, 0);
        if (i < q_mine && id < n_jobs) {
            const int f = (int)(((uint32_t)id * CW_PIECE) / FB) + (lane % FPJ);
            if (f < env_n) {
                r.f = f;
                const int e = env_lo + f;
                if (src == CW_SRC_CURRENT) {
                    const uint32_t *h = (const uint32_t *)(P.hdr + e);
                    r.hx = h[0];
                    r.hw = h[3];
                    r.p = P.pos[e];
                } else {
                    r.hx = src == CW_SRC_INIT ? (uint32_t)P.init_agent[e] : (uint32_t)P.goal_agent[e];
                    r.hw = src == CW_SRC_INIT ? CW_CODES_INITIAL : P.goal_codes[e];
                    r.p = src == CW_SRC_INIT ? P.init_pos[e] : P.goal_pos[e];
                }
            }
        }
        if (src == CW_SRC_CURRENT) r.hx &= 0x00FFFFFFu;
        else { const uint32_t ar = __umulhi(r.hx, P.div_magic); r.hx = ar | ((r.hx - ar * S) << 8); }
        if (RASTER != 1) { const uint32_t hold = (r.hx >> 16) & 0xFFu; r.o2 = hold ? rgb_of_code(hold) : 0x00FFFFFFu; }
        return r;
    };
    Rec nxt = fetch(0);
    uint32_t t_next16 = ((uint32_t)__builtin_amdgcn_s_memrealtime() << 4) + (uint32_t)(((long long)wave * period16) / n_waves);
    for (int base = 0; base < q_mine; base += JPB) {
        const Rec cur = nxt;
        if (base + JPB < q_mine) nxt = fetch(base + JPB);
        const int in_batch = min(q_mine - base, JPB);
        for (int k = 0; k < in_batch; k++) {
            const int f0 = __builtin_amdgcn_readlane(cur.f, FPJ * k);
            if (f0 < 0) continue;
            const uint32_t a0 = (uint32_t)((base + k) * n_waves + wave) * CW_PIECE;
            const uint32_t a1 = min(a0 + CW_PIECE, total);
            const uint32_t win = a1 - a0;
            uint32_t hx = 0, hw = 0, o2 = 0, pd = 0;
            auto gather = [&](int pair) {
                const int from = (int)(((uint32_t)(FPJ * k + 2 * pair) + half) << 2);
                hx = (uint32_t)__builtin_amdgcn_ds_bpermute(from, (int)cur.hx);
                hw = (uint32_t)__builtin_amdgcn_ds_bpermute(from, (int)cur.hw);
                o2 = RASTER != 1 ? (uint32_t)__builtin_amdgcn_ds_bpermute(from, (int)cur.o2) : 0u;
                pd = ((uint32_t)__builtin_amdgcn_ds_bpermute(from, (int)cur.p.x) & m_p0) | ((uint32_t)__builtin_amdgcn_ds_bpermute(from, (int)cur.p.y) & m_p1) |
                     ((uint32_t)__builtin_amdgcn_ds_bpermute(from, (int)cur.p.z) & m_p2) | ((uint32_t)__builtin_amdgcn_ds_bpermute(from, (int)cur.p.w) & m_p3);
            };
            if (RASTER != 1) gather(0);
            if (period16) {
                const uint32_t now16 = (uint32_t)__builtin_amdgcn_s_memrealtime() << 4;
                const int wait16 = (int)(t_next16 - now16);
                if (wait16 > 0) {
                    for (int z = (wait16 * 5) >> 8; z > 0; z--) __builtin_amdgcn_s_sleep(1);
                    while ((int)(t_next16 - ((uint32_t)__builtin_amdgcn_s_memrealtime() << 4)) > 0) { }
                } else if (wait16 < -period16) t_next16 = now16 - (uint32_t)period16;
                t_next16 += (uint32_t)(period16 + (base + k < CW_HEAD_JOBS ? head_extra16 : 0));
            }
            uint8_t *const job = dst_base + a0;
            if (win == CW_PIECE) {
#pragma unroll
                for (int s = 0; s < CW_PIECE_STORES; s++) *(uint4 *)(job + 1024 * s + 16 * lane) = make_uint4(0, 0, 0, 0);
            } else piece_fill_partial(dst_base, a0, a1, lane);
#pragma unroll
            for (int pair = 0; pair < FPJ / 2; pair++) {
                if (FPJ > 2 && pair > 0 && ((uint32_t)f0 + 2u * pair >= (uint32_t)env_n || ((uint32_t)f0 + 2u * pair) * FB >= a1)) break;
                if (RASTER == 1 || pair > 0) gather(pair);
                const uint32_t fi = (uint32_t)f0 + 2u * (uint32_t)pair + half;
                const uint32_t f_base = __umul24(fi, FB);
                const bool frame_on = fi < (uint32_t)env_n && f_base < a1;
                const uint32_t hold = (hx >> 16) & 0xFFu;
                if (RASTER == 1) {
                    const uint32_t agent_cell = __umul24(hx & 0xFFu, S) + ((hx >> 8) & 0xFFu);
                    const uint32_t pos = (((pd >> sh_pos) & 0xFFFFu) & m_slot) | (agent_cell & ~m_slot);
                    const uint32_t item = (((hw >> sh_item) & 15u) & m_slot) | (9u & m_agent) | (hold & m_held);
                    const uint32_t r = __umulhi(pos, P.div_magic), c = pos - __umul24(r, S), kk = item - 1u;
                    const uint32_t k3 = (kk >= 6u) ? 2u : (kk >= 3u) ? 1u : 0u;
                    const uint32_t off_obj = __umul24(3u * r + k3, row_bytes) + 9u * c + 3u * (kk - 3u * k3);
                    const uint32_t col_obj = (uint32_t)__builtin_amdgcn_ds_bpermute((int)((kk & 15u) << 2), (int)v_cpv);
                    const bool is_obj = (m_flag == 0u) && pl < 10u && item != 0 && pos < (uint32_t)P.ncell;
                    const bool is_flag = (m_flag & hold) != 0;
                    uint32_t p_off = is_obj ? off_obj : is_flag ? off_flag : 0xFFFFFFFFu;
                    uint32_t p_val = is_obj ? col_obj : 0x00FFFFFFu;
                    const uint32_t held_off = (uint32_t)__builtin_amdgcn_ds_bpermute((int)((((uint32_t)lane & 32u) + 9u) << 2), (int)p_off);
                    const bool twice = pl < 8u && p_off != 0xFFFFFFFFu && p_off == held_off;
                    p_val = twice ? (((2u * (p_val & 0xFFu)) & 0xFFu) | ((2u * (p_val & 0xFF00u)) & 0xFF00u) | ((2u * (p_val & 0xFF0000u)) & 0xFF0000u)) : p_val;
                    const unsigned long long m_twice = CW_BALLOT(twice);
                    p_off = (pl == 9u && ((m_twice >> (32u * half)) & 0xFFFFFFFFull)) ? 0xFFFFFFFFu : p_off;
                    if (frame_on && p_off != 0xFFFFFFFFu) {
                        const uint32_t at = f_base + p_off;
                        if (at - a0 < win) dst_base[at] = (uint8_t)p_val;
                        if (at + 1u - a0 < win) dst_base[at + 1u] = (uint8_t)(p_val >> 8);
                        if (at + 2u - a0 < win) dst_base[at + 2u] = (uint8_t)(p_val >> 16);
                    }
                } else {
                    const uint32_t pos = (pd >> sh_pos) & 0xFFFFu, code = (hw >> sh_item) & 15u;
                    const uint32_t rgb = (uint32_t)__builtin_amdgcn_ds_bpermute((int)(code << 2), (int)v_rgb);
                    const uint32_t r = __umulhi(pos, P.div_magic), c = pos - __umul24(r, S);
                    const uint32_t seg = f_base + __umul24(4u * r + dy, row_bytes) + 12u * c;
                    const u32x3 d = cell_row_dwords(rgb);
                    const bool is_obj = frame_on && code != 0 && pos < (uint32_t)P.ncell;
                    const bool in0 = seg - a0 < win, in2 = seg + 8u - a0 < win;
                    if (is_obj && in0 && in2) *(u32x3_a4 *)(dst_base + seg) = d;
                    else if (is_obj) {
                        if (in0) *(uint32_t *)(dst_base + seg) = d.x;
                        if (seg + 4u - a0 < win) *(uint32_t *)(dst_base + seg + 4u) = d.y;
                        if (in2) *(uint32_t *)(dst_base + seg + 8u) = d.z;
                    }
                    const uint32_t aseg = f_base + __umul24(4u * (hx & 0xFFu) + dy, row_bytes) + 12u * ((hx >> 8) & 0xFFu);
                    const uint32_t o = dy == 2u ? o2 : 0x00FFFFFFu;
                    const bool is_mark = frame_on && marks;
                    if (is_mark && aseg - a0 < win) dst_base[aseg + 3u] = (uint8_t)o;
                    if (is_mark && aseg + 4u - a0 < win) *(uint32_t *)(dst_base + aseg + 4u) = (o >> 8) | (o << 16);
                    if (is_mark && aseg + 8u - a0 < win) dst_base[aseg + 8u] = (uint8_t)(o >> 16);
                }
            }
        }
    }
}
template <int RASTER, int FPJ>
__global__ __launch_bounds__(256) void cw_render_pieces_kernel(CwParams P, uint8_t *frames, int src, int period16, int period16_head, int period16_busy,
                                                               int chunk, int env_lo, int env_n)
{
    const unsigned long long done_now = P.counters[1];
    const unsigned long long finished = src == CW_SRC_CURRENT ? done_now - P.counters[4] : (unsigned long long)P.n_envs;
    const bool busy = finished >= CW_BUSY_FINISHED, storm = finished * 8ull >= (unsigned long long)P.n_envs;
    render_pieces<RASTER, FPJ>(P, frames, src, __builtin_amdgcn_readfirstlane(storm ? period16_busy : period16),
                               __builtin_amdgcn_readfirstlane(!storm && (chunk & 1) ? (busy ? period16_busy : period16_head) - period16 : 0), env_lo, env_n);
    if (src == CW_SRC_CURRENT && (chunk & 2) && blockIdx.x == 0 && threadIdx.x == 0) P.counters[4] = done_now;
}
#define CW_GATHER_MAX_S 9
template <int NF>
__global__ __launch_bounds__(256) void cw_render_gather_kernel(CwParams P, uint8_t *frames, int src, int period16, int env_lo, int env_n)
{
    constexpr int JPB = CW_WAVE / NF;
    constexpr int COL_WORDS = (NF * CW_GATHER_MAX_S * CW_GATHER_MAX_S + 255) / 256 * 256;
    __shared__ uint32_t s_col[256 / CW_WAVE][COL_WORDS];
    __shared__ uint32_t s_slot[CW_GATHER_MAX_S * CW_GATHER_MAX_S * 3];
    const int lane = threadIdx.x & (CW_WAVE - 1);
    const int wpb = blockDim.x / CW_WAVE;
    const int wave_in_block = __builtin_amdgcn_readfirstlane(threadIdx.x / CW_WAVE);
    const int n_waves = (int)gridDim.x * wpb;
    const int wave = (int)blockIdx.x * wpb + wave_in_block;
    const uint32_t S = (uint32_t)P.size, ncell = (uint32_t)P.ncell, FB = P.frame_bytes, row_bytes = 12u * S, Q = FB >> 4;
    for (uint32_t q = threadIdx.x; q < Q; q += blockDim.x) {
        const uint32_t o = 16u * q, y = o / row_bytes, x = o - y * row_bytes, c0 = x / 12u, ph = (x - 12u * c0) >> 2;
        const uint32_t cell_a = (y >> 2) * S + c0;
        uint32_t cell_b, dy_b;
        if (c0 + 1u < S) { cell_b = cell_a + 1u; dy_b = y & 3u; }
        else { const uint32_t y2 = min(y + 1u, 4u * S - 1u); cell_b = (y2 >> 2) * S; dy_b = y2 & 3u; }
        s_slot[q] = cell_a | (cell_b << 8) | ((y & 3u) << 16) | (dy_b << 18) | (ph << 20);
    }
    __syncthreads();
    uint8_t *const dst_base = frames + (size_t)env_lo * FB;
    const uint32_t total = (uint32_t)env_n * FB;
    const int n_jobs = (int)((total + CW_PIECE - 1u) / CW_PIECE);
    if (wave >= n_jobs) return;
    const int q_mine = (n_jobs + n_waves - 1) / n_waves;
    uint32_t *const col = s_col[wave_in_block];
    const uint32_t v_rgb = rgb_of_code((uint32_t)lane & 15u);
    const uint32_t fr = (uint32_t)lane >> 3, slot = (uint32_t)lane & 7u;
    const uint32_t sh_pos = 16u * (slot & 1u), sh_item = 4u * slot;
    const uint32_t m_p0 = (slot & 6u) == 0u ? 0xFFFFFFFFu : 0u, m_p1 = (slot & 6u) == 2u ? 0xFFFFFFFFu : 0u;
    const uint32_t m_p2 = (slot & 6u) == 4u ? 0xFFFFFFFFu : 0u, m_p3 = (slot & 6u) == 6u ? 0xFFFFFFFFu : 0u;
    const uint32_t q_magic = (uint32_t)((1ull << 32) / Q) + 1u;
    const int zero_rounds = __builtin_amdgcn_readfirstlane((int)((((CW_PIECE - 1u) / FB + 2u) * ncell + 255u) / 256u));
    __builtin_amdgcn_s_setprio(3);
    struct Rec { int f; uint32_t hx, hw; uint4 p; };
    auto fetch = [&](int base) {
        Rec r;
        const int i = base + lane / NF;
        const int id = i * n_waves + wave;
        r.f = -1; r.hx = 0; r.hw = 0;
        r.p = make_uint4(0, 0, 0, 0);
        if (i < q_mine && id < n_jobs) {
            const int f = (int)(((uint32_t)id * CW_PIECE) / FB) + (lane % NF);
            if (f < env_n) {
                r.f = f;
                const int e = env_lo + f;
                if (src == CW_SRC_CURRENT) {
                    const uint32_t *h = (const uint32_t *)(P.hdr + e);
                    r.hx = h[0];
                    r.hw = h[3];
                    r.p = P.pos[e];
                } else {
                    r.hx = src == CW_SRC_INIT ? (uint32_t)P.init_agent[e] : (uint32_t)P.goal_agent[e];
                    r.hw = src == CW_SRC_INIT ? CW_CODES_INITIAL : P.goal_codes[e];
                    r.p = src == CW_SRC_INIT ? P.init_pos[e] : P.goal_pos[e];
                }
            }
        }
        if (src == CW_SRC_CURRENT) r.hx &= 0x00FFFFFFu;
        else { const uint32_t ar = __umulhi(r.hx, P.div_magic); r.hx = ar | ((r.hx - ar * S) << 8); }
        return r;
    };
    Rec nxt = fetch(0);
    uint32_t t_next16 = ((uint32_t)__builtin_amdgcn_s_memrealtime() << 4) + (uint32_t)(((long long)wave * period16) / n_waves);
    for (int base = 0; base < q_mine; base += JPB) {
        const Rec cur = nxt;
        if (base + JPB < q_mine) nxt = fetch(base + JPB);
        const int in_batch = min(q_mine - base, JPB);
        for (int k = 0; k < in_batch; k++) {
            const int f0 = __builtin_amdgcn_readlane(cur.f, NF * k);
            if (f0 < 0) continue;
            const uint32_t a0 = (uint32_t)((base + k) * n_waves + wave) * CW_PIECE;
            const uint32_t a1 = min(a0 + CW_PIECE, total);
            for (int z = 0; z < zero_rounds; z++) *(uint4 *)(col + 256 * z + 4 * lane) = make_uint4(0, 0, 0, 0);
            {
                const int from = (int)(((uint32_t)(NF * k) + (fr & (uint32_t)(NF - 1))) << 2);
                const uint32_t hx = (uint32_t)__builtin_amdgcn_ds_bpermute(from, (int)cur.hx), hw = (uint32_t)__builtin_amdgcn_ds_bpermute(from, (int)cur.hw);
                const int ff = __builtin_amdgcn_ds_bpermute(from, cur.f);
                const uint32_t pd = ((uint32_t)__builtin_amdgcn_ds_bpermute(from, (int)cur.p.x) & m_p0) | ((uint32_t)__builtin_amdgcn_ds_bpermute(from, (int)cur.p.y) & m_p1) |
                                    ((uint32_t)__builtin_amdgcn_ds_bpermute(from, (int)cur.p.z) & m_p2) | ((uint32_t)__builtin_amdgcn_ds_bpermute(from, (int)cur.p.w) & m_p3);
                const uint32_t pos = (pd >> sh_pos) & 0xFFFFu, code = (hw >> sh_item) & 15u;
                const uint32_t rgb = (uint32_t)__builtin_amdgcn_ds_bpermute((int)(code << 2), (int)v_rgb);
                const bool frame_on = fr < (uint32_t)NF && ff >= 0 && (uint32_t)ff * FB < a1;
                if (frame_on && code != 0 && pos < ncell) col[fr * ncell + pos] = rgb;
                if (frame_on && slot == 0u)
                    atomicOr(&col[fr * ncell + (hx & 0xFFu) * S + ((hx >> 8) & 0xFFu)], (1u + ((hx >> 16) & 0xFFu)) << 24);
            }
            if (period16) {
                const uint32_t now16 = (uint32_t)__builtin_amdgcn_s_memrealtime() << 4;
                const int wait16 = (int)(t_next16 - now16);
                if (wait16 > 0) {
                    for (int z = (wait16 * 5) >> 8; z > 0; z--) __builtin_amdgcn_s_sleep(1);
                    while ((int)(t_next16 - ((uint32_t)__builtin_amdgcn_s_memrealtime() << 4)) > 0) { }
                } else if (wait16 < -period16) t_next16 = now16 - (uint32_t)period16;
                t_next16 += (uint32_t)period16;
            }
            const uint32_t q0 = (a0 >> 4) - (uint32_t)f0 * Q;
#pragma unroll
            for (int st = 0; st < CW_PIECE_STORES; st++) {
                const uint32_t g = q0 + 64u * st + (uint32_t)lane;
                const uint32_t i = __umulhi(g, q_magic), q = g - i * Q;
                const uint32_t e = s_slot[q];
                const uint32_t ca = col[i * ncell + (e & 0xFFu)], cb = col[i * ncell + ((e >> 8) & 0xFFu)];
                u32x3 da = cell_row_dwords(ca & 0x00FFFFFFu), db = cell_row_dwords(cb & 0x00FFFFFFu);
                const uint32_t dya = (e >> 16) & 3u, dyb = (e >> 18) & 3u, fa = ca >> 24, fb = cb >> 24;
                const uint32_t ha = fa == 2u ? (110u | (69u << 8) | (39u << 16)) : fa == 3u ? (255u | (105u << 8) | (180u << 16)) : (100u | (100u << 8) | (200u << 16));
                const uint32_t hb = fb == 2u ? (110u | (69u << 8) | (39u << 16)) : fb == 3u ? (255u | (105u << 8) | (180u << 16)) : (100u | (100u << 8) | (200u << 16));
                if (fa != 0u && (dya == 1u || dya == 2u)) da = overlay_dwords(da, (dya == 2u && fa > 1u) ? ha : 0x00FFFFFFu);
                if (fb != 0u && (dyb == 1u || dyb == 2u)) db = overlay_dwords(db, (dyb == 2u && fb > 1u) ? hb : 0x00FFFFFFu);
                const uint32_t ph = e >> 20;
                uint4 out;
                out.x = ph == 0u ? da.x : ph == 1u ? da.y : da.z;
                out.y = ph == 0u ? da.y : ph == 1u ? da.z : db.x;
                out.z = ph == 0u ? da.z : ph == 1u ? db.x : db.y;
                out.w = ph == 0u ? db.x : ph == 1u ? db.y : db.z;
                const uint32_t at = a0 + 1024u * st + 16u * (uint32_t)lane;
                if (at < a1) *(uint4 *)(dst_base + at) = out;
            }
        }
    }
}
__global__ __launch_bounds__(256) void cw_export_grid_kernel(CwParams P, uint8_t *out)
{
    const size_t total = (size_t)P.n_envs * P.ncell;
    const size_t stride = (size_t)gridDim.x * blockDim.x;
    for (size_t g = (size_t)blockIdx.x * blockDim.x + threadIdx.x; g < total; g += stride) {
        const uint32_t env = (uint32_t)(g / P.ncell);
        const uint32_t cell = (uint32_t)(g - (size_t)env * P.ncell);
        uint32_t sp[8];
        unpack_pos(P.pos[env], sp);
        out[g] = (uint8_t)code_of(P.hdr[env].w, slot_at(sp, cell));
    }
}
__global__ __launch_bounds__(256) void cw_export_onehot_kernel(CwParams P, uint8_t *out, int which)
{
    const size_t total = (size_t)P.n_envs * P.ncell;
    const size_t stride = (size_t)gridDim.x * blockDim.x;
    for (size_t g = (size_t)blockIdx.x * blockDim.x + threadIdx.x; g < total; g += stride) {
        const uint32_t env = (uint32_t)(g / P.ncell);
        const uint32_t cell = (uint32_t)(g - (size_t)env * P.ncell);
        const uint4 h = P.hdr[env];
        uint32_t sp[8];
        unpack_pos(which == 1 ? P.goal_pos[env] : which == 2 ? P.init_pos[env] : P.pos[env], sp);
        const uint32_t codes = which == 1 ? P.goal_codes[env] : which == 2 ? CW_CODES_INITIAL : h.w;
        const uint32_t code = code_of(codes, slot_at(sp, cell));
        const uint32_t agent_cell = which == 1 ? (uint32_t)P.goal_agent[env] : which == 2 ? (uint32_t)P.init_agent[env] : agent_cell_of(P, h.x);
        const uint32_t hold = which ? 0u : hold_of(h.x);
        uint32_t bits = code ? (1u << (code - 1)) : 0u;
        if (cell == agent_cell) bits |= (1u << 8) | (hold ? (1u << (8 + hold)) : 0u);
        *(u32x3_a4 *)(out + g * 12) = onehot_dwords(bits);
    }
}

__global__ __launch_bounds__(256) void cw_render_onehot_kernel(const uint8_t *__restrict__ oh, int n_states, int S, uint32_t div_magic,
                                                               uint16_t *__restrict__ out)
{
    const int lane = threadIdx.x & (CW_WAVE - 1);
    const int wave = (blockIdx.x * blockDim.x + threadIdx.x) / CW_WAVE;
    const int n_waves = gridDim.x * blockDim.x / CW_WAVE;
    const int ncell = S * S;
    for (int f = wave; f < n_states; f += n_waves) {
        const uint8_t *st = oh + (size_t)f * ncell * 12;
        uint32_t agent = 0xFFFFFFFFu, hold = 0;
        for (int cell = lane; cell < ncell; cell += CW_WAVE) {
            const uint8_t *c = st + 12 * cell;
            if (c[8] == 1) agent = min(agent, (uint32_t)cell);
            const uint32_t hv = c[9] >= c[10] && c[9] >= c[11] ? (c[9] ? 1u : 0u) : (c[10] >= c[11] ? 2u : 3u);
            hold = max(hold, hv);
        }
        for (int off = 32; off; off >>= 1) {
            agent = min(agent, (uint32_t)__shfl_xor((int)agent, off));
            hold = max(hold, (uint32_t)__shfl_xor((int)hold, off));
        }
        const uint32_t hold_rgb = rgb_of_code(hold);
        uint16_t *img = out + (size_t)f * ncell * 48;
        const uint32_t row_px = 4u * S;
        for (int cell = lane; cell < ncell; cell += CW_WAVE) {
            const uint8_t *c = st + 12 * cell;
            uint32_t r = 0, g = 0, b = 0;
#pragma unroll
            for (int k = 0; k < 8; k++) {
                const uint32_t col = rgb_of_code((uint32_t)k + 1u), v = c[k];
                r += v * (col & 0xFFu); g += v * ((col >> 8) & 0xFFu); b += v * (col >> 16);
            }
            const uint32_t cr = __umulhi((uint32_t)cell, div_magic), cc = (uint32_t)cell - cr * S;
            for (uint32_t dy = 0; dy < 4; dy++)
                for (uint32_t dx = 0; dx < 4; dx++) {
                    uint32_t pr = r, pg = g, pb = b;
                    if ((uint32_t)cell == agent && (dy == 1 || dy == 2) && (dx == 1 || dx == 2)) {
                        pr = pg = pb = 255u;
                        if (dy == 2 && hold) { pr = hold_rgb & 0xFFu; pg = (hold_rgb >> 8) & 0xFFu; pb = hold_rgb >> 16; }
                    }
                    uint16_t *px = img + ((size_t)(4u * cr + dy) * row_px + 4u * cc + dx) * 3;
                    px[0] = (uint16_t)pr; px[1] = (uint16_t)pg; px[2] = (uint16_t)pb;
                }
        }
    }
}

__global__ __launch_bounds__(256) void cw_render_onehot_alt_kernel(const uint8_t *__restrict__ oh, int n_states, int S, uint32_t div_magic,
                                                                   uint16_t *__restrict__ out)
{
    const int lane = threadIdx.x & (CW_WAVE - 1);
    const int wave = (blockIdx.x * blockDim.x + threadIdx.x) / CW_WAVE;
    const int n_waves = gridDim.x * blockDim.x / CW_WAVE;
    const int ncell = S * S;
    const uint32_t row_px = 3u * S;
    for (int f = wave; f < n_states; f += n_waves) {
        const uint8_t *st = oh + (size_t)f * ncell * 12;
        bool held = false;
        for (int cell = lane; cell < ncell; cell += CW_WAVE) {
            const uint8_t *c = st + 12 * cell;
            held = held || c[9] || c[10] || c[11];
        }
        const bool any_held = CW_BALLOT(held) != 0;
        uint16_t *img = out + (size_t)f * (size_t)(3 * S + 3) * row_px * 3;
        for (int cell = lane; cell < ncell; cell += CW_WAVE) {
            const uint8_t *c = st + 12 * cell;
            const uint32_t cr = __umulhi((uint32_t)cell, div_magic), cc = (uint32_t)cell - cr * S;
#pragma unroll
            for (int k = 0; k < 9; k++) {
                const uint32_t cnt = (uint32_t)c[k] + (k < 3 ? (uint32_t)c[9 + k] : 0u), col = cpv_color(k);
                uint16_t *px = img + ((size_t)(3u * cr + k / 3) * row_px + 3u * cc + k % 3) * 3;
                px[0] = (uint16_t)(cnt * (col & 0xFFu)); px[1] = (uint16_t)(cnt * ((col >> 8) & 0xFFu)); px[2] = (uint16_t)(cnt * (col >> 16));
            }
        }
        for (uint32_t j = (uint32_t)lane; j < 3u * row_px; j += CW_WAVE) {
            const uint32_t x = j % row_px;
            const uint16_t v = (any_held && x >= 3u && x < 6u) ? 255 : 0;
            uint16_t *px = img + ((size_t)(3u * S) * row_px + j) * 3;
            px[0] = v; px[1] = v; px[2] = v;
        }
    }
}

__global__ __launch_bounds__(256) void cw_seed_kernel(CwParams P, const uint32_t *seeds)
{
    const int i = blockIdx.x * blockDim.x + threadIdx.x;
    if (i >= P.n_envs) return;
    uint32_t *s = P.mt + (size_t)i * CW_MT_WORDS;
    int pos;
    if (seeds) {
        uint32_t x = seeds[i];
        s[0] = x;
        for (int k = 1; k < CW_MT_WORDS; k++) {
            x = 1812433253u * (x ^ (x >> 30)) + (uint32_t)k;
            s[k] = x;
        }
        pos = CW_MT_WORDS;
    } else {
        pos = min(max(P.mt_idx[i], 0), CW_MT_WORDS);
    }
    uint32_t cur = s[0];
    for (int k = 0; k < pos; k++) {
        const uint32_t nxt = s[k + 1 == CW_MT_WORDS ? 0 : k + 1];
        const uint32_t far = s[k + 397 >= CW_MT_WORDS ? k + 397 - CW_MT_WORDS : k + 397];
        const uint32_t y = (cur & 0x80000000u) | (nxt & 0x7fffffffu);
        s[k] = far ^ (y >> 1) ^ ((y & 1u) ? 0x9908b0dfu : 0u);
        cur = nxt;
    }
    P.mt_idx[i] = pos == CW_MT_WORDS ? 0 : pos;
}

static inline int cw_frames_per_job(uint32_t frame_bytes)
{
    const int most = (int)((CW_PIECE - 1u) / frame_bytes) + 2;
    int fpj = 2;
    while (fpj < most) fpj <<= 1;
    return fpj;
}
static inline int cw_piece_chunks(const CwParams &P, const CwTuning &tn, int *per)
{
    const long long waves = (long long)tn.n_cu * (256 / CW_WAVE);
    const long long cap = (long long)(tn.render_chunk_rounds > 0 ? tn.render_chunk_rounds : 1 << 20) * waves * 3072;
    const long long bytes = (long long)P.n_envs * P.frame_bytes;
    int n = (int)((bytes + cap - 1) / cap);
    if (n < 1) n = 1;
    *per = (P.n_envs + n - 1) / n;
    if (n > 1 || bytes >= (1ll << 32)) {
        *per = (int)(((long long)*per + 4095) / 4096 * 4096);
        while ((long long)*per * P.frame_bytes >= (1ll << 32) && *per > 4096) *per = (*per / 2 + 4095) / 4096 * 4096;
    }
    return (P.n_envs + *per - 1) / *per;
}
static inline int cw_render_grid(const CwTuning &tn, long long jobs)
{
    long long blocks = (jobs + 3) / 4;
    if (blocks > tn.n_cu) blocks = tn.n_cu;
    if (blocks < 1) blocks = 1;
    return (int)blocks;
}
static inline bool cw_use_gather(const CwParams &P, const CwTuning &tn) { return tn.gather && P.raster == 0 && P.size <= tn.gather_max_size; }
static inline int cw_sweep_blocks(const CwParams &P, const CwTuning &tn, long long pieces)
{
    const bool small = (int)P.frame_bytes < tn.small_frame_bytes && (cw_use_gather(P, tn) || pieces * (long long)CW_PIECE < tn.small_launch_bytes);
    const int per_cu = small && pieces > 4ll * tn.n_cu * tn.small_blocks_per_cu ? tn.small_blocks_per_cu : 1;
    return cw_render_grid(tn, pieces) * per_cu;
}
typedef void (*CwSweepKernel)(CwParams, uint8_t *, int, int, int, int, int, int, int);
static CwSweepKernel cw_sweep_kernel(int raster, int fpj)
{
    if (raster == 1) return fpj <= 2 ? cw_render_pieces_kernel<1, 2> : fpj <= 4 ? cw_render_pieces_kernel<1, 4> : fpj <= 8 ? cw_render_pieces_kernel<1, 8> : cw_render_pieces_kernel<1, 16>;
    return fpj <= 2 ? cw_render_pieces_kernel<0, 2> : fpj <= 4 ? cw_render_pieces_kernel<0, 4> : fpj <= 8 ? cw_render_pieces_kernel<0, 8> : cw_render_pieces_kernel<0, 16>;
}
static void cw_launch_sweep(const CwParams &P, const CwTuning &tn, uint8_t *frames, int src, hipStream_t st)
{
    int per = 0;
    const int n_chunks = cw_piece_chunks(P, tn, &per);
    const CwSweepKernel k = cw_sweep_kernel(P.raster, cw_frames_per_job(P.frame_bytes));
    for (int c = 0; c < n_chunks; c++) {
        const int env_n = min(per, P.n_envs - c * per);
        const long long pieces = ((long long)env_n * P.frame_bytes + CW_PIECE - 1) / CW_PIECE;
        if (cw_use_gather(P, tn)) {
            const int grid = cw_sweep_blocks(P, tn, pieces);
            if (cw_frames_per_job(P.frame_bytes) <= 4)
                hipLaunchKernelGGL(cw_render_gather_kernel<4>, dim3(grid), dim3(256), 0, st, P, frames, src, tn.period16, c * per, env_n);
            else
                hipLaunchKernelGGL(cw_render_gather_kernel<8>, dim3(grid), dim3(256), 0, st, P, frames, src, tn.period16, c * per, env_n);
            continue;
        }
        hipLaunchKernelGGL(k, dim3(cw_sweep_blocks(P, tn, pieces)), dim3(256), 0, st, P, frames, src, tn.period16, tn.period16_head, tn.period16_busy, (c == 0 ? 1 : 0) | (c == n_chunks - 1 ? 2 : 0), c * per, env_n);
    }
}

static inline int cw_wave_blocks(int waves) { return (waves + CW_RESET_WAVES - 1) / CW_RESET_WAVES; }
static inline int cw_reset_grid(const CwTuning &tn, int jobs)
{
    int blocks = cw_wave_blocks(jobs);
    if (blocks > tn.n_cu * tn.reset_blocks_per_cu) blocks = tn.n_cu * tn.reset_blocks_per_cu;
    if (blocks < 1) blocks = 1;
    return blocks;
}

static int cw_envs_per_wave(int n, int most = 64)
{
    int epw = most;
    while (epw > 8 && (n + epw - 1) / epw < 1024) epw >>= 1;
    return epw;
}

extern "C" {

hipError_t cwk_launch_step(const CwParams *P, const CwTuning *T, const void *actions, int act_dtype, int obs_mode,
                           int auto_reset, hipStream_t st, hipEvent_t *ev )
{
    const CwTuning &tn = *T;
    const int n = P->n_envs;
    const bool ev_all = ev && obs_mode != 1;
    if (ev_all) (void)hipEventRecord(ev[0], st);
    if (auto_reset) {
        const int epw = cw_envs_per_wave(n, tn.step_envs_per_wave);
        const int waves = (n + epw - 1) / epw;
        const int paint = obs_mode == 2 ? 1 : obs_mode == 1 ? 2 : 0;
        hipLaunchKernelGGL(cw_step_fused_variant(paint, paint != 0 && P->terminal_img != nullptr), dim3(cw_wave_blocks(waves)), dim3(CW_RESET_WAVES * CW_WAVE),
                           0, st, *P, actions, act_dtype, epw);
    } else {
        hipLaunchKernelGGL(cw_step_kernel, dim3((n + 255) / 256), dim3(256), 0, st, *P, actions, act_dtype, obs_mode == 2 ? 1 : 0);
    }
    if (ev_all) (void)hipEventRecord(ev[1], st);
    if (ev) for (int k = 2; k < 5; k++) (void)hipEventRecord(ev[k], st);
    if (obs_mode == 1) cw_launch_sweep(*P, tn, P->obs, CW_SRC_CURRENT, st);
    if (ev) (void)hipEventRecord(ev[5], st);
    return hipGetLastError();
}

hipError_t cwk_launch_refill(const CwParams *P, const CwTuning *T, int all_envs, hipStream_t st)
{
    hipLaunchKernelGGL(cw_refill_kernel, dim3(cw_reset_grid(*T, P->n_envs)), dim3(CW_RESET_WAVES * CW_WAVE), 0, st, *P, all_envs);
    return hipGetLastError();
}

hipError_t cwk_launch_rollout(const CwParams *P, const uint8_t *actions, int T, int32_t *rewards, uint8_t *dones, hipStream_t st)
{
    const int epw = cw_envs_per_wave(P->n_envs);
    const int waves = (P->n_envs + epw - 1) / epw;
    hipLaunchKernelGGL(cw_rollout_kernel, dim3(cw_wave_blocks(waves)), dim3(CW_RESET_WAVES * CW_WAVE), 0, st, *P, actions, T, rewards, dones, epw);
    return hipGetLastError();
}

hipError_t cwk_launch_render_restore(const CwParams *P, const CwTuning *T, hipStream_t st)
{
    cw_launch_sweep(*P, *T, P->obs, CW_SRC_CURRENT, st);
    cw_launch_sweep(*P, *T, P->init_img, CW_SRC_INIT, st);
    cw_launch_sweep(*P, *T, P->desired_img, CW_SRC_GOAL, st);
    return hipGetLastError();
}

hipError_t cwk_launch_reset_all(const CwParams *P, const CwTuning *T, int obs_mode, hipStream_t st)
{
    hipLaunchKernelGGL(cw_reset_kernel, dim3(cw_reset_grid(*T, P->n_envs)), dim3(CW_RESET_WAVES * CW_WAVE), 0, st, *P);
    if (obs_mode != 0) return cwk_launch_render_restore(P, T, st);
    return hipGetLastError();
}

hipError_t cwk_launch_render_onehot(const CwParams *P, const uint8_t *onehot, int n_states, uint16_t *out, hipStream_t st)
{
    int blocks = (n_states + 3) / 4;
    if (blocks > 1024) blocks = 1024;
    if (blocks < 1) blocks = 1;
    if (P->raster == 1) hipLaunchKernelGGL(cw_render_onehot_alt_kernel, dim3(blocks), dim3(256), 0, st, onehot, n_states, P->size, P->div_magic, out);
    else hipLaunchKernelGGL(cw_render_onehot_kernel, dim3(blocks), dim3(256), 0, st, onehot, n_states, P->size, P->div_magic, out);
    return hipGetLastError();
}

hipError_t cwk_launch_resident(const CwParams *P, CwResident *R, uint32_t seq0, int paint_dirty, unsigned long long idle_ticks,
                               unsigned long long life_ticks, hipStream_t st)
{
    hipLaunchKernelGGL(cw_resident_kernel, dim3(1), dim3(CW_WAVE), 0, st, *P, R, seq0, paint_dirty, idle_ticks, life_ticks);
    return hipGetLastError();
}

hipError_t cwk_launch_seed(const CwParams *P, const uint32_t *seeds_dev, hipStream_t st)
{
    hipLaunchKernelGGL(cw_seed_kernel, dim3((P->n_envs + 255) / 256), dim3(256), 0, st, *P, seeds_dev);
    return hipGetLastError();
}

hipError_t cwk_launch_pool(const CwParams *P, const CwTuning *T, hipStream_t st)
{
    const int n = P->n_envs;
    hipLaunchKernelGGL(cw_pool_kernel, dim3(cw_reset_grid(*T, n)), dim3(CW_RESET_WAVES * CW_WAVE), 0, st, *P);
    return hipGetLastError();
}

void cwk_sweep_shape(const CwParams *P, const CwTuning *T, int *n_chunks, int *waves, int *jobs_per_wave)
{
    int per = 0;
    *n_chunks = cw_piece_chunks(*P, *T, &per);
    const long long pieces = ((long long)min(per, P->n_envs) * P->frame_bytes + CW_PIECE - 1) / CW_PIECE;
    *waves = cw_sweep_blocks(*P, *T, pieces) * (256 / CW_WAVE);
    *jobs_per_wave = (int)((pieces + *waves - 1) / *waves);
}

hipError_t cwk_launch_sweep_calib(const CwParams *P, const CwTuning *T, hipStream_t st)
{
    cw_launch_sweep(*P, *T, P->obs, CW_SRC_CURRENT, st);
    return hipGetLastError();
}

__global__ void cw_idle_kernel(int n)
{
    for (int i = 0; i < n; i++) __builtin_amdgcn_s_sleep(127);
}
hipError_t cwk_launch_idle(hipStream_t st)
{
    hipLaunchKernelGGL(cw_idle_kernel, dim3(1), dim3(64), 0, st, 3);
    return hipGetLastError();
}

hipError_t cwk_launch_render_ext(const CwParams *P, const CwTuning *T, uint8_t *out, hipStream_t st)
{
    if (((uintptr_t)out & 15u) == 0) cw_launch_sweep(*P, *T, out, CW_SRC_CURRENT, st);
    else hipLaunchKernelGGL(cw_render_frames_kernel, dim3(cw_render_grid(*T, P->n_envs)), dim3(256), 0, st, *P, out);
    return hipGetLastError();
}

hipError_t cwk_launch_export(const CwParams *P, const CwTuning *T, uint8_t *out, int onehot, int which, hipStream_t st)
{
    const size_t total = (size_t)P->n_envs * P->ncell;
    const size_t cap = (size_t)T->n_cu * 32;
    int blocks = (int)((total + 255) / 256 < cap ? (total + 255) / 256 : cap);
    if (blocks < 1) blocks = 1;
    if (onehot) hipLaunchKernelGGL(cw_export_onehot_kernel, dim3(blocks), dim3(256), 0, st, *P, out, which);
    else hipLaunchKernelGGL(cw_export_grid_kernel, dim3(blocks), dim3(256), 0, st, *P, out);
    return hipGetLastError();
}

}
```

### gym_craftingworld_amd/csrc/cw_layout.h

```cpp
#pragma once
#include <stdint.h>

#define CW_POS_GONE 0xFFFFu
#define CW_POS_HELD 0xFFFEu

#define CW_FLAG_RESET 0x1u
#define CW_FLAG_SUBSET 0x2u


#define CW_CODES_INITIAL 0x87654321u
#define CW_CTL_QUEUED 0x100u
#define CW_LA_DEPTH 4

struct CwMenuDev {
    uint64_t sel_bits;
    int32_t n_selected;
    int32_t number_of_tasks;
    int32_t stacking;
    int32_t reward_subset;
};

struct CwTuning {
    int n_cu = 256;
    int period16 = 0;
    int period16_head = 0;
    int period16_busy = 0;
    int render_chunk_rounds = 896;
    int gather = 1;
    int gather_max_size = 7;
    int small_frame_bytes = 4096;
    int small_blocks_per_cu = 4;
    long long small_launch_bytes = 320ll << 20;
    int step_envs_per_wave = 64;
    int reset_blocks_per_cu = 4;
};

struct CwResident {
    unsigned long long bell;
    uint32_t pad0[30];
    uint32_t ack;
    uint32_t exited;
    uint32_t pad1[30];
};

struct CwParams {
    uint4 *hdr;
    uint4 *pos;
    uint4 *init_pos;
    uint16_t *init_agent;
    uint4 *goal_pos;
    uint32_t *goal_codes;
    uint16_t *goal_agent;
    int32_t *ep_no;
    uint32_t *mt;
    int32_t *mt_idx;
    uint16_t *pool;
    int32_t *reward;
    uint8_t *done;
    uint16_t *achieved_out;
    uint16_t *desired_out;
    int32_t *episode_length;
    int32_t *episode_return;
    uint8_t *obs;
    uint8_t *desired_img;
    uint8_t *init_img;
    uint8_t *terminal_img;
    uint4 *nx_init_pos;
    uint4 *nx_goal_pos;
    uint4 *nx_misc;
    uint32_t *nx_ctl;
    int32_t lookahead;
    unsigned long long *la_feedback;
    unsigned long long *counters;
    const CwMenuDev *menus;
    int32_t n_envs;
    int32_t size;
    int32_t ncell;
    int32_t max_steps;
    uint32_t task_mask;
    int32_t pool_k;
    uint32_t div_magic;
    uint32_t frame_bytes;
    int32_t raster;
    uint8_t *res_onehot;
};
```

### gym_craftingworld_amd/vec_env.py

```python
import atexit
import ctypes as C
import sys
import weakref

import numpy as np
import torch

from . import _lib as L
from . import seeding
from ._wrap import tensor_view
from .spaces import Box, Dict, Discrete, MultiDiscrete, batch_space

TASK_LIST = ['MakeBread', 'EatBread', 'BuildHouse', 'ChopTree', 'ChopRock', 'GoToHouse', 'MoveAxe',
             'MoveHammer', 'MoveSticks']
OBJECTS = ['sticks', 'axe', 'hammer', 'rock', 'tree', 'bread', 'house', 'wheat']
PICKUPABLE = ['sticks', 'axe', 'hammer']
ACTION_NAMES = ['up', 'right', 'down', 'left', 'pickup', 'drop']
UP, RIGHT, DOWN, LEFT, PICKUP, DROP = range(6)
COLORS = [(110, 69, 39), (255, 105, 180), (100, 100, 200), (100, 100, 100), (0, 128, 0), (205, 133, 63), (197, 91, 97), (240, 230, 140)]
COLORS_N = [(0, 0, 0)] + COLORS
COLORS_H = [tuple(255 - c for c in COLORS[k]) for k in range(3)]
STATE_W = STATE_H = 21
MAX_STEPS = 300

# ... 297 lines not shown
            actions = actions.to(torch.int32)
        actions = actions.contiguous()
        if actions.numel() != self.num_envs:
            raise ValueError('expected %d actions, got %d' % (self.num_envs, actions.numel()))
        self._actions_keepalive = actions
        L.check(self._lib.cw_step(self._h, C.c_void_p(actions.data_ptr()), _ACT_DTYPES[actions.dtype], self._stream()),
                'cw_step', self._lib)
        self._pending = True

    def step_wait(self):
        if not self._pending:
            raise RuntimeError('step_wait without step_async')
        self._pending = False
        if self.host_outputs:
            self._sync()
        info = {'task_success': self.achieved_mask, 'desired_goal': self.desired_mask,
                'achieved_goal': self.achieved_mask, 'episode_length': self.episode_length,
                'episode': {'r': self.episode_return, 'l': self.episode_length}}
        if self.terminal_observation is not None:
            info['terminal_observation'] = self.terminal_observation
        return self._observation(), self.reward, self.done, info

    def step(self, actions):
        self.step_async(actions)
        return self.step_wait()

    def step_many(self, actions):
        if not (type(actions) is torch.Tensor and actions.dtype in _ACT_DTYPES and actions.device == self.device and actions.is_contiguous()
                and actions.dim() == 2 and actions.shape[1] == self.num_envs):
            raise ValueError('actions must be a contiguous [K, num_envs] tensor of dtype uint8 / int32 / int64 on %s' % (self.device,))
        self._actions_keepalive = actions
        L.check(self._lib.cw_step_many(self._h, C.c_void_p(actions.data_ptr()), _ACT_DTYPES[actions.dtype], int(actions.shape[0]), self._stream()),
                'cw_step_many', self._lib)

    def capture_steps(self, actions):
        self.synchronize()
        graph = torch.cuda.CUDAGraph()
        with torch.cuda.graph(graph):
            self.step_many(actions)
        return graph

    def rollout(self, actions, record=True):
        if not torch.is_tensor(actions):
            actions = torch.as_tensor(np.asarray(actions), device=self.device)
        actions = actions.to(device=self.device)
        if actions.dtype != torch.uint8:
            if actions.dtype not in _ACT_DTYPES:
                actions = actions.to(torch.int32)
            invalid = (actions < 0) | (actions > 5)
            actions = actions.to(torch.uint8).masked_fill_(invalid, 255)
        actions = actions.contiguous()
        if actions.dim() != 2 or actions.shape[1] != self.num_envs:
            raise ValueError('actions must have shape [T, num_envs]')
        T = actions.shape[0]
        rew = torch.empty((T, self.num_envs), dtype=torch.int32, device=self.device) if record else None
        don = torch.empty((T, self.num_envs), dtype=torch.uint8, device=self.device) if record else None
        L.check(self._lib.cw_rollout(self._h, C.c_void_p(actions.data_ptr()), T,
                                     C.c_void_p(rew.data_ptr()) if record else None,
                                     C.c_void_p(don.data_ptr()) if record else None, self._stream()), 'cw_rollout', self._lib)
        self._actions_keepalive = actions
        return (rew, don.view(torch.bool)) if record else None

    def render(self, out=None):
        if out is None:
            out = torch.empty((self.num_envs,) + self.frame_shape, dtype=torch.uint8, device=self.device)
        L.check(self._lib.cw_render(self._h, C.c_void_p(out.data_ptr()), self._stream()), 'cw_render', self._lib)
        return out

    def render_exact(self):
        return self.render_states(self.one_hot())

    def render_states(self, one_hot):
        oh = torch.as_tensor(np.asarray(one_hot) if not torch.is_tensor(one_hot) else one_hot)
        oh = oh.to(device=self.device, dtype=torch.uint8).contiguous()
        if oh.dim() != 4 or tuple(oh.shape[1:]) != (self.size, self.size, 12):
            raise ValueError('states must have shape [M, %d, %d, 12]' % (self.size, self.size))
        out = torch.empty((oh.shape[0],) + self.frame_shape, dtype=torch.int16, device=self.device)
        L.check(self._lib.cw_render_onehot(self._h, C.c_void_p(oh.data_ptr()), oh.shape[0], C.c_void_p(out.data_ptr()), self._stream()),
                'cw_render_onehot', self._lib)
        self._states_keepalive = oh
        return out

    def grid(self, out=None):
        if out is None:
            out = torch.empty((self.num_envs, self.size, self.size), dtype=torch.uint8, device=self.device)
        L.check(self._lib.cw_export_grid(self._h, C.c_void_p(out.data_ptr()), self._stream()), 'cw_export_grid', self._lib)
        return out

    def one_hot(self, out=None, which='current'):
        if out is None:
            out = torch.empty((self.num_envs, self.size, self.size, 12), dtype=torch.uint8, device=self.device)
        w = {'current': 0, 'goal': 1, 'init': 2}[which]
        L.check(self._lib.cw_export_onehot_of(self._h, w, C.c_void_p(out.data_ptr()), self._stream()), 'cw_export_onehot_of', self._lib)
        return out

    def mask_to_vector(self, mask):
        bits = torch.arange(len(self.task_list), device=mask.device, dtype=torch.int32)
        return ((mask.to(torch.int32).unsqueeze(1) >> bits) & 1).to(torch.uint8)

    def fixed_states(self):
        out = np.empty((self.num_envs, max(self.fixed_init_state, 1), 9), dtype=np.uint16)
        self._settle()
        L.check(self._lib.cw_get_fixed_states(self._h, out.ctypes.data_as(C.c_void_p)), 'cw_get_fixed_states', self._lib)
        return out

    def get_state(self):
        N, S = self.num_envs, self.size
        out = dict(grid=np.empty((N, S, S), np.uint8), init_grid=np.empty((N, S, S), np.uint8),
                   goal_grid=np.empty((N, S, S), np.uint8), agent_rc=np.empty((N, 2), np.uint8),
                   init_agent_rc=np.empty((N, 2), np.uint8), goal_agent_rc=np.empty((N, 2), np.uint8),
                   hold=np.empty(N, np.uint8), achieved=np.empty(N, np.uint16), desired=np.empty(N, np.uint16),
                   step_num=np.empty(N, np.int32), ep_no=np.empty(N, np.int32))
        view = L.cw_state_view(**{k: a.ctypes.data_as(C.c_void_p) for k, a in out.items()})
        self._settle()
        L.check(self._lib.cw_get_state(self._h, C.byref(view)), 'cw_get_state', self._lib)
        return out

    def set_state(self, **fields):
        dt = dict(grid=np.uint8, init_grid=np.uint8, goal_grid=np.uint8, agent_rc=np.uint8, init_agent_rc=np.uint8,
                  goal_agent_rc=np.uint8, hold=np.uint8, achieved=np.uint16, desired=np.uint16, step_num=np.int32,
                  ep_no=np.int32)
        keep = {}
        view = L.cw_state_view()
        for k, a in fields.items():
            if k not in dt:
                raise ValueError('cannot set %r' % k)
            keep[k] = np.ascontiguousarray(a, dtype=dt[k])
            if keep[k].shape[0] != self.num_envs:
                raise ValueError('%s must have num_envs rows' % k)
            setattr(view, k, keep[k].ctypes.data_as(C.c_void_p))
        self._settle()
        L.check(self._lib.cw_set_state(self._h, C.byref(view)), 'cw_set_state', self._lib)

    def save_checkpoint(self, path):
        n = int(self._lib.cw_checkpoint_bytes(self._h))
        buf = np.empty(n, dtype=np.uint8)
        self._settle()
        L.check(self._lib.cw_checkpoint_save(self._h, buf.ctypes.data_as(C.c_void_p), n), 'cw_checkpoint_save', self._lib)
        with open(path, 'wb') as f:
            buf.tofile(f)

    def load_checkpoint(self, path):
        buf = np.fromfile(path, dtype=np.uint8)
        self._settle()
        L.check(self._lib.cw_checkpoint_load(self._h, buf.ctypes.data_as(C.c_void_p), buf.size), 'cw_checkpoint_load', self._lib)
        self._has_reset = True

    def profile_begin(self, max_steps):
        L.check(self._lib.cw_profile_begin(self._h, int(max_steps)), 'cw_profile_begin', self._lib)

    def render_kernel_name(self):
        return (self._lib.cw_render_kernel_name(self._h) or b'').decode()

    def profile_end(self):
        p = L.cw_profile()
        L.check(self._lib.cw_profile_end(self._h, C.byref(p)), 'cw_profile_end', self._lib)
        return {k: getattr(p, k) for k, _ in p._fields_}

    def tuner_state(self):
        t = L.cw_tuner_state()
        L.check(self._lib.cw_tuner(self._h, C.byref(t)), 'cw_tuner', self._lib)
        return {k: int(getattr(t, k)) for k, _ in t._fields_}

    def compute_reward_batch(self, achieved_mask, desired_mask, subset=None):
        full = (1 << len(self.task_list)) - 1
        a = achieved_mask.to(torch.int32) & full
        d = desired_mask.to(torch.int32) & full
        if subset is None:
            subset = bool(self._menus[0].reward_subset)
        if subset:
            hit = ((d & ~a) == 0) & (((~(d ^ a)) & full) != 0)
        else:
            hit = a == d
        return torch.where(hit, torch.full_like(a, self.MAX_STEPS), torch.full_like(a, -1))

    def compute_reward(self, achieved_goal, desired_goal, info=None):
        a = np.asarray(achieved_goal).reshape(-1)
        d = np.asarray(desired_goal).reshape(-1)
        if self._menus[0].reward_subset:
            return self.MAX_STEPS if np.max(d.astype(np.int64) - a.astype(np.int64)) == 0 else -1
        return self.MAX_STEPS if np.array_equal(a, d) else -1
```

### include/craftingworld.h

```cpp
#ifndef CRAFTINGWORLD_H
#define CRAFTINGWORLD_H

#include <stddef.h>
#include <stdint.h>

#ifdef __cplusplus
extern "C" {
#endif

#define CW_ABI_VERSION 5
#define CW_MT_N 624
#define CW_MAX_TASKS 16
#define CW_MAX_MENUS 256
#define CW_NUM_OBJECTS 8

#define CW_OK 0
#define CW_ERR_INVALID (-1)
#define CW_ERR_HIP (-2)
#define CW_ERR_STATE (-3)

enum { CW_EMPTY = 0, CW_STICKS = 1, CW_AXE = 2, CW_HAMMER = 3, CW_ROCK = 4, CW_TREE = 5,
       CW_BREAD = 6, CW_HOUSE = 7, CW_WHEAT = 8 };

enum {
    CW_OBS_STATE = 0,
    CW_OBS_PIXELS_FULL = 1,
    CW_OBS_PIXELS_DIRTY = 2
};

enum {
    CW_RASTER_RAY = 0,
    CW_RASTER_ALT = 1
};

enum { CW_ACT_I32 = 0, CW_ACT_I64 = 1, CW_ACT_U8 = 2 };

typedef struct cw_task_menu {
    int32_t n_selected;
    int32_t number_of_tasks;
    int32_t stacking;
    int32_t reward_subset;
    int32_t selected_bits[CW_MAX_TASKS];
} cw_task_menu;

typedef struct cw_config {
    int32_t abi_version;
    int32_t num_envs;
    int32_t size;
    int32_t max_steps;
    int32_t n_task_list;
    int32_t fixed_init_state;
    int32_t obs_mode;
    int32_t auto_reset;
    int32_t keep_terminal_obs;
    int32_t raster;
    int32_t host_outputs;
    int32_t n_menus;
    const cw_task_menu *menus;
    const uint8_t *env_menu;
} cw_config;

typedef struct cw_engine cw_engine;
typedef void *cw_stream_t;

typedef struct cw_buffer_table {
    uint8_t *obs;
    uint8_t *desired_goal;
    uint8_t *init_obs;
    uint8_t *terminal_obs;
    int32_t *reward;
    uint8_t *done;
    uint16_t *achieved;
    uint16_t *desired;
    int32_t *episode_length;
    int32_t *episode_return;
    uint8_t *hdr;
    uint16_t *slot_pos;
    uint64_t *counters;
    size_t frame_bytes;
    int32_t *host_actions;
    uint8_t *host_onehot;
} cw_buffer_table;

typedef struct cw_state_view {
    uint8_t *grid;
    uint8_t *init_grid;
    uint8_t *goal_grid;
    uint8_t *agent_rc;
    uint8_t *init_agent_rc;
    uint8_t *goal_agent_rc;
    uint8_t *hold;
    uint16_t *achieved;
    uint16_t *desired;
    int32_t *step_num;
    int32_t *ep_no;
} cw_state_view;

int cw_create(const cw_config *cfg, int device, cw_engine **out);
int cw_destroy(cw_engine *e);

int cw_seed_mt(cw_engine *e, const uint32_t *keys, const int32_t *pos);
int cw_seed_int(cw_engine *e, const uint32_t *seeds);
int cw_get_mt(cw_engine *e, uint32_t *keys, int32_t *pos);

int cw_generate_fixed_states(cw_engine *e, cw_stream_t stream);
int cw_get_fixed_states(cw_engine *e, uint16_t *out);

int cw_reset(cw_engine *e, cw_stream_t stream);

int cw_step(cw_engine *e, const void *actions, int action_dtype, cw_stream_t stream);

int cw_step_many(cw_engine *e, const void *actions, int action_dtype, int32_t n_steps, cw_stream_t stream);

int cw_rollout(cw_engine *e, const uint8_t *actions, int32_t n_steps, int32_t *rewards, uint8_t *dones,
               cw_stream_t stream);

int cw_step_resident(cw_engine *e, int32_t action, int32_t want_onehot );
int cw_resident_stop(cw_engine *e);

int cw_render(cw_engine *e, uint8_t *out_frames, cw_stream_t stream);

int cw_render_onehot(cw_engine *e, const uint8_t *onehot, int32_t n_states, uint16_t *out_frames, cw_stream_t stream);

int cw_export_grid(cw_engine *e, uint8_t *out, cw_stream_t stream);
int cw_export_onehot(cw_engine *e, uint8_t *out, cw_stream_t stream);
enum { CW_STATE_CURRENT = 0, CW_STATE_GOAL = 1, CW_STATE_INIT = 2 };
int cw_export_onehot_of(cw_engine *e, int which, uint8_t *out, cw_stream_t stream);

int cw_get_state(cw_engine *e, cw_state_view *host);
int cw_set_state(cw_engine *e, const cw_state_view *host);

size_t cw_checkpoint_bytes(cw_engine *e);
int cw_checkpoint_save(cw_engine *e, void *buf, size_t capacity);
int cw_checkpoint_load(cw_engine *e, const void *buf, size_t length);

typedef struct cw_profile {
    int32_t steps;
    float ms_step_kernel;
    float ms_reset_kernel;
    float ms_render_kernel;
    float ms_render_kernel_max;
    float ms_render_kernel_min;
    float ms_render_kernel_median;
} cw_profile;
int cw_profile_begin(cw_engine *e, int max_steps);
int cw_profile_end(cw_engine *e, cw_profile *out);
const char *cw_render_kernel_name(const cw_engine *e);

typedef struct cw_tuner_state {
    int32_t period16, period16_head, period16_busy, lookahead, resident, guard_slowdowns;
} cw_tuner_state;
int cw_tuner(const cw_engine *e, cw_tuner_state *out);

int cw_buffers(cw_engine *e, cw_buffer_table *out);
int cw_synchronize(cw_engine *e, cw_stream_t stream);
int cw_num_envs(const cw_engine *e);
int cw_abi_version(void);
const char *cw_last_error(void);

#ifdef __cplusplus
}
#endif
#endif
```

Baseline: 315.1 million.

## Fuse step and render sweep into one launch with grid-wide sync

```diff
diff --git a/gym_craftingworld_amd/_lib.py b/gym_craftingworld_amd/_lib.py
--- a/gym_craftingworld_amd/_lib.py
+++ b/gym_craftingworld_amd/_lib.py
@@ -87,6 +87,7 @@
     'cw_step_resident': (C.c_int, [_VP, C.c_int32, C.c_int32]),
     'cw_resident_stop': (C.c_int, [_VP]),
     'cw_render_kernel_name': (C.c_char_p, [_VP]),
+    'cw_one_launch': (C.c_int, [_VP]),
     'cw_buffers': (C.c_int, [_VP, C.POINTER(cw_buffer_table)]),
     'cw_synchronize': (C.c_int, [_VP, _VP]),
     'cw_num_envs': (C.c_int, [_VP]),
@@ -104,6 +105,10 @@
                                          'small_blocks_per_cu', 'small_launch_mb', 'reset_blocks_per_cu', 'guard', 'verbose', 'lookahead',
                                          'la_period', 'rollout_segment', 'pad')] + \
               [(f, C.c_double) for f in ('head_notch', 'busy_notch', 'period_ns', 'rate_tbs')]
+
+
+class cwh_one_launch(C.Structure):
+    _fields_ = [(f, C.c_int32) for f in ('on', 'fills_front', 'fills_back', 'pad')]
 
 
 cwh_lookup = C.CFUNCTYPE(_VP, _VP, C.c_char_p)
@@ -126,6 +131,9 @@
     'cwh_guard_scheduled_ms': (C.c_double, [C.c_double, C.c_int32, C.c_int32, C.c_double]),
     'cwh_la_adapt': (C.c_int32, [C.c_int32, C.c_int32, C.c_uint64, C.POINTER(C.c_int32)]),
     'cwh_read_tuning': (None, [cwh_lookup, _VP, C.POINTER(cwh_tuning)]),
+    'cwh_read_one_launch': (None, [cwh_lookup, _VP, C.POINTER(cwh_one_launch)]),
+    'cwh_one_launch_spin_ticks': (C.c_uint32, [C.c_int64, C.c_uint32, C.c_int32]),
+    'cwh_one_launch_poll': (C.c_int32, [C.POINTER(C.c_uint32), C.POINTER(C.c_int32), C.POINTER(C.c_int32)]),
 }
 
 
diff --git a/gym_craftingworld_amd/csrc/cw_engine.cpp b/gym_craftingworld_amd/csrc/cw_engine.cpp
--- a/gym_craftingworld_amd/csrc/cw_engine.cpp
+++ b/gym_craftingworld_amd/csrc/cw_engine.cpp
@@ -29,6 +29,7 @@
 hipError_t cwk_launch_sweep_calib(const CwParams *P, const CwTuning *T, hipStream_t st);
 void cwk_sweep_shape(const CwParams *P, const CwTuning *T, int *n_chunks, int *waves, int *jobs_per_wave);
 hipError_t cwk_launch_idle(hipStream_t st);
+int cwk_one_launch_eligible(const CwParams *P, const CwTuning *T, int obs_mode, int auto_reset, int host_mapped);
 hipError_t cwk_launch_export(const CwParams *P, const CwTuning *T, uint8_t *out, int onehot, int which, hipStream_t st);
 }
 
@@ -102,6 +103,8 @@
     int sweep_waves = 1024;
     double sweep_jobs = 0, sweep_rate = 0, sweep_beside_ms = 0;
     bool guard_on = false;
+    double one_launch_extra_ms = 0;
+    int32_t one_launch_reported = 0;
     double head_notch = 0.4, busy_notch = 0.75, tune_period_ns = -1, tune_rate_tbs = -1;
     bool tune_guard = true, tune_lookahead = true, verbose = false;
     enum { GUARD_RING = 32 };
@@ -255,6 +258,14 @@
     set_sweep_rate(e, 6.4);
     if (rc == CW_OK) rc = timed_render_stats(e, &med, &p90);
     e->sweep_beside_ms = med - e->sweep_jobs * sweep_period_ns(e, 6.4) * 1e-6;
+    if (tn.one_launch && rc == CW_OK) {
+        double med_dry = med, p90_dry = 0;
+        tn.one_launch_dry = 1;
+        rc = timed_render_stats(e, &med_dry, &p90_dry);
+        tn.one_launch_dry = 0;
+        e->one_launch_extra_ms = med_dry > med ? med_dry - med : 0.0;
+        if (e->verbose) fprintf(stderr, "[craftingworld] one launch per step: the step phase adds %.4f ms to a sweep's launch (%.4f against %.4f)\n", e->one_launch_extra_ms, med_dry, med);
+    }
     if (e->tune_rate_tbs >= 0) e->sweep_rate = e->tune_rate_tbs;
     for (size_t i = 0; i < sizeof(rates) / sizeof(rates[0]) && rc == CW_OK && e->tune_rate_tbs < 0; i++) {
         set_sweep_rate(e, rates[i]);
@@ -276,14 +287,24 @@
 }
 
 enum { CW_GUARD_EVERY = 64 };
+static int one_launch_check(cw_engine *e, bool report)
+{
+    int32_t unreported = 0;
+    int32_t *rep = report ? &e->one_launch_reported : &unreported;
+    if (!cwh_one_launch_poll(e->tune.one_launch_timeout_host, &e->tune.one_launch, rep) || !report) return CW_OK;
+    return fail(CW_ERR_HIP, "a grid-wide wait inside the one-launch step timed out (its workgroups were not all resident, or the card was held up): the frames of "
+                            "that step may show the step before; the engine steps with two launches from now on (CW_TUNE_ONE_LAUNCH=0 selects them from the start)");
+}
 static hipEvent_t *sweep_guard_tick(cw_engine *e, hipStream_t st)
 {
     if (++e->guard_step % CW_GUARD_EVERY) return nullptr;
+    (void)one_launch_check(e, false);
     while (e->guard_tail != e->guard_head && hipEventQuery(e->guard_ring[e->guard_tail % cw_engine::GUARD_RING].ev[5]) == hipSuccess) {
         cw_engine::GuardSample &smp = e->guard_ring[e->guard_tail++ % cw_engine::GUARD_RING];
         float ms = 0.f;
         if (hipEventElapsedTime(&ms, smp.ev[4], smp.ev[5]) != hipSuccess || ms <= 0.f || smp.period16 != e->tune.period16) continue;
-        const double scheduled = cwh_guard_scheduled_ms(e->sweep_jobs, e->tune.period16, e->tune.period16_busy, e->sweep_beside_ms);
+        const double scheduled = cwh_guard_scheduled_ms(e->sweep_jobs, e->tune.period16, e->tune.period16_busy,
+                                                        e->sweep_beside_ms + (e->tune.one_launch ? e->one_launch_extra_ms : 0.0));
         const double rate_before = e->guard.rate, prev_mean = e->guard.prev_mean;
         const int recovering = e->guard.recovering;
         const int action = cwh_guard_step(&e->guard, ms, scheduled);
@@ -342,6 +363,28 @@
     e->rollout_segment = t.rollout_segment;
 }
 
+enum { CW_ONE_LAUNCH_FILLS_FRONT = 0, CW_ONE_LAUNCH_FILLS_BACK = 0 };
+static void setup_one_launch(cw_engine *e)
+{
+    CwTuning &tn = e->tune;
+    cwh_one_launch t{1, CW_ONE_LAUNCH_FILLS_FRONT, CW_ONE_LAUNCH_FILLS_BACK, 0};
+    cwh_read_one_launch([](void *, const char *k) -> const char * { return getenv(k); }, nullptr, &t);
+    tn.one_launch = 0;
+    if (!t.on || !cwk_one_launch_eligible(&e->P, &tn, e->obs_mode, e->auto_reset, e->host_actions ? 1 : 0)) return;
+    unsigned long long *sync = nullptr;
+    if (dev_alloc(e, &sync, 32) != CW_OK) return;
+    void *word = nullptr;
+    if (hipHostMalloc(&word, 64, hipHostMallocCoherent) != hipSuccess) return;
+    memset(word, 0, 64);
+    e->host_allocs.push_back(word);
+    tn.one_launch_sync = sync;
+    tn.one_launch_timeout_host = (unsigned int *)word;
+    tn.one_launch_fills_front = t.fills_front;
+    tn.one_launch_fills_back = t.fills_back;
+    tn.one_launch_spin_ticks = cwh_one_launch_spin_ticks(e->n, e->P.frame_bytes, e->P.terminal_img ? 3 : 2);
+    tn.one_launch = 1;
+}
+
 extern "C" {
 
 const char *cw_last_error(void) { return g_err; }
@@ -518,6 +561,7 @@
     std::vector<uint32_t> seeds(N);
     for (size_t i = 0; i < N; i++) seeds[i] = (uint32_t)i;
     rc = cw_seed_int(e, seeds.data());
+    if (rc == CW_OK) setup_one_launch(e);
     if (rc == CW_OK) rc = calibrate_sweep(e);
     if (rc != CW_OK) {
         cw_destroy(e);
@@ -887,7 +931,7 @@
         out->ms_render_kernel_median = render_ms.empty() ? 0.f : render_ms[render_ms.size() / 2];
     }
     prof_free(e);
-    return CW_OK;
+    return one_launch_check(e, true);
 }
 
 const char *cw_render_kernel_name(const cw_engine *e)
@@ -942,8 +986,10 @@
     HIP_TRY(hipStreamSynchronize((hipStream_t)stream));
     for (int i = 0; i < e->n_work; i++)
         if (e->work[i] == (hipStream_t)stream) { e->work[i] = e->work[--e->n_work]; break; }
-    return CW_OK;
-}
+    return one_launch_check(e, true);
+}
+
+int cw_one_launch(const cw_engine *e) { return e && e->tune.one_launch ? 1 : 0; }
 
 int cw_get_fixed_states(cw_engine *e, uint16_t *out)
 {
diff --git a/gym_craftingworld_amd/csrc/cw_host.cpp b/gym_craftingworld_amd/csrc/cw_host.cpp
--- a/gym_craftingworld_amd/csrc/cw_host.cpp
+++ b/gym_craftingworld_amd/csrc/cw_host.cpp
@@ -269,3 +269,25 @@
     tune_int(lookup, ctx, "CW_TUNE_LA_PERIOD", &t->la_period, 1, INT32_MAX);
     tune_int(lookup, ctx, "CW_TUNE_ROLLOUT_SEGMENT", &t->rollout_segment, -1, INT32_MAX);
 }
+
+extern "C" void cwh_read_one_launch(cwh_lookup lookup, void *ctx, cwh_one_launch *t)
+{
+    tune_int(lookup, ctx, "CW_TUNE_ONE_LAUNCH", &t->on, INT32_MIN, INT32_MAX);
+    t->on = t->on != 0;
+    tune_int(lookup, ctx, "CW_TUNE_ONE_LAUNCH_FILLS_FRONT", &t->fills_front, 0, 32);
+    tune_int(lookup, ctx, "CW_TUNE_ONE_LAUNCH_FILLS_BACK", &t->fills_back, 0, 32);
+}
+extern "C" uint32_t cwh_one_launch_spin_ticks(int64_t n_envs, uint32_t frame_bytes, int32_t frames_per_env)
+{
+    const double bytes = (double)n_envs * (double)frame_bytes * (double)frames_per_env;
+    const double ticks = (bytes / 0.35e12 + 0.010) * 1e8;
+    return ticks < 4.0e9 ? (uint32_t)ticks : 4000000000u;
+}
+extern "C" int32_t cwh_one_launch_poll(const volatile uint32_t *word, int32_t *one_launch, int32_t *reported)
+{
+    if (!word || *word == 0) return 0;
+    *one_launch = 0;
+    if (*reported) return 0;
+    *reported = 1;
+    return 1;
+}
diff --git a/gym_craftingworld_amd/csrc/cw_host.h b/gym_craftingworld_amd/csrc/cw_host.h
--- a/gym_craftingworld_amd/csrc/cw_host.h
+++ b/gym_craftingworld_amd/csrc/cw_host.h
@@ -80,6 +80,13 @@
 typedef const char *(*cwh_lookup)(void *ctx, const char *name);
 void cwh_read_tuning(cwh_lookup lookup, void *ctx, cwh_tuning *t);
 
+typedef struct cwh_one_launch {
+    int32_t on, fills_front, fills_back, pad;
+} cwh_one_launch;
+void cwh_read_one_launch(cwh_lookup lookup, void *ctx, cwh_one_launch *t);
+uint32_t cwh_one_launch_spin_ticks(int64_t n_envs, uint32_t frame_bytes, int32_t frames_per_env);
+int32_t cwh_one_launch_poll(const volatile uint32_t *word, int32_t *one_launch, int32_t *reported);
+
 #ifdef __cplusplus
 }
 #endif
diff --git a/gym_craftingworld_amd/csrc/cw_kernels.hip b/gym_craftingworld_amd/csrc/cw_kernels.hip
--- a/gym_craftingworld_amd/csrc/cw_kernels.hip
+++ b/gym_craftingworld_amd/csrc/cw_kernels.hip
@@ -939,9 +939,18 @@
 
 struct CwPaintJob { uint4 pos; uint32_t codes, agent_hold_kind, env, pad; };
 enum { CW_JOB_INIT = 0, CW_JOB_GOAL = 1, CW_JOB_TERMINAL = 2 };
-template <int PAINT, bool TERM>
-__device__ __forceinline__ void fused_step(const CwParams &P, const void *actions, int act_dtype, int epw, int wave, uint32_t *s_mt_wave,
-                                           CwPaintJob *s_jobs, int *s_njobs, int *s_cnt )
+typedef unsigned int cw_u32x4 __attribute__((ext_vector_type(4)));
+__device__ __forceinline__ void store_sc1_16(uint4 *base, int n, int i, const uint4 &v)
+{
+    const __amdgpu_buffer_rsrc_t rsrc = __builtin_amdgcn_make_buffer_rsrc((void *)base, 0, n * 16, 0x00020000);
+    const cw_u32x4 d = {v.x, v.y, v.z, v.w};
+    __builtin_amdgcn_raw_buffer_store_b128(d, rsrc, i * 16, 0, 16);
+}
+struct CwNoHook { __device__ __forceinline__ void operator()() const {} };
+template <int PAINT, bool TERM, bool PUBLISH = false, typename AfterLoads = CwNoHook>
+__device__ __forceinline__ int fused_step(const CwParams &P, const void *actions, int act_dtype, int epw, int wave, uint32_t *s_mt_wave,
+                                          CwPaintJob *s_jobs, int *s_njobs, int *s_cnt ,
+                                          bool first_share = true, AfterLoads after_loads = AfterLoads())
 {
     constexpr int paint = PAINT;
     const int lane = threadIdx.x & (CW_WAVE - 1);
@@ -957,6 +966,7 @@
     unpack_pos(P.pos[e], sp);
     const uint4 ip = P.init_pos[e];
     const uint32_t ctl = P.lookahead ? P.nx_ctl[e] : 0u;
+    after_loads();
     if (threadIdx.x == 0) { *s_njobs = 0; s_cnt[0] = s_cnt[1] = s_cnt[2] = 0; }
     __syncthreads();
     const CwStepOut o = step_env(P, h, sp, a, [&]() { return ip; });
@@ -986,7 +996,7 @@
     const unsigned long long m_pop = CW_BALLOT(popped);
     __syncthreads();
     if (threadIdx.x == 0) {
-        if (blockIdx.x == 0) atomicAdd(&P.counters[0], (unsigned long long)P.n_envs);
+        if (blockIdx.x == 0 && first_share) atomicAdd(&P.counters[0], (unsigned long long)P.n_envs);
         if (s_cnt[0]) atomicAdd(&P.counters[1], (unsigned long long)s_cnt[0]);
         if (s_cnt[1]) atomicAdd(&P.counters[2], (unsigned long long)s_cnt[1]);
         if (s_cnt[2]) atomicAdd(&P.counters[3], (unsigned long long)s_cnt[2]);
@@ -1041,10 +1051,15 @@
         }
     }
     if (live) {
-        P.hdr[env] = h;
-        P.pos[env] = pack_pos(sp);
-    }
-    if constexpr (PAINT == 0) return;
+        if constexpr (PUBLISH) {
+            store_sc1_16(P.hdr, P.n_envs, env, h);
+            store_sc1_16(P.pos, P.n_envs, env, pack_pos(sp));
+        } else {
+            P.hdr[env] = h;
+            P.pos[env] = pack_pos(sp);
+        }
+    }
+    if constexpr (PAINT == 0) return 0;
     __syncthreads();
     const int n_jobs = *s_njobs;
     for (int jq = wave_in_block; jq < n_jobs; jq += CW_RESET_WAVES) {
@@ -1061,6 +1076,7 @@
         else d0 = P.terminal_img + off;
         paint_state_frame(P, d0, jp, codes, ahk & 0xFFFFu, (ahk >> 16) & 0xFFu, lane, d1);
     }
+    return n_jobs;
 }
 template <int PAINT, bool TERM>
 __global__ __launch_bounds__(CW_RESET_WAVES *CW_WAVE) void cw_step_fused_kernel(CwParams P, const void *actions, int act_dtype, int epw)
@@ -1124,8 +1140,21 @@
         else for (uint32_t b = c; b < a1; b++) dst_base[b] = 0;
     }
 }
-template <int RASTER, int FPJ>
-__device__ __forceinline__ void render_pieces(const CwParams &P, uint8_t *frames, int src, int period16, int head_extra16, int env_lo, int env_n)
+struct CwStepPhase {
+    const void *actions;
+    unsigned long long *sync;
+    unsigned int *timeout_host;
+    int act_dtype, epw, term;
+    int fills_front, fills_back;
+    int dry;
+    unsigned int spin_ticks;
+    int period16_head, period16_busy;
+};
+#define CW_STEP_LDS_BYTES (CW_RESET_WAVES * CW_MT_WORDS * 4 + CW_RESET_WAVES * CW_WAVE * 3 * 32 + 32)
+template <int M> struct CwJobMode { static constexpr int value = M; };
+template <int RASTER, int FPJ, bool STEP>
+__device__ __forceinline__ void render_pieces(const CwParams &P, uint8_t *frames, int src, int period16, int head_extra16, int env_lo, int env_n,
+                                              const CwStepPhase &sp, unsigned long long counters4, unsigned long long &done_now)
 {
     constexpr int JPB = CW_WAVE / FPJ;
     const int lane = threadIdx.x & (CW_WAVE - 1);
@@ -1137,7 +1166,7 @@
     uint8_t *const dst_base = frames + (size_t)env_lo * FB;
     const uint32_t total = (uint32_t)env_n * FB;
     const int n_jobs = (int)((total + CW_PIECE - 1u) / CW_PIECE);
-    if (wave >= n_jobs) return;
+    if constexpr (!STEP) { if (wave >= n_jobs) return; }
     const int q_mine = (n_jobs + n_waves - 1) / n_waves;
     const uint32_t half = (uint32_t)lane >> 5, pl = (uint32_t)lane & 31u;
     const uint32_t slot = RASTER == 1 ? (pl & 7u) : (pl >> 2), dy = pl & 3u;
@@ -1180,15 +1209,16 @@
         if (RASTER != 1) { const uint32_t hold = (r.hx >> 16) & 0xFFu; r.o2 = hold ? rgb_of_code(hold) : 0x00FFFFFFu; }
         return r;
     };
-    Rec nxt = fetch(0);
-    uint32_t t_next16 = ((uint32_t)__builtin_amdgcn_s_memrealtime() << 4) + (uint32_t)(((long long)wave * period16) / n_waves);
-    for (int base = 0; base < q_mine; base += JPB) {
-        const Rec cur = nxt;
-        if (base + JPB < q_mine) nxt = fetch(base + JPB);
-        const int in_batch = min(q_mine - base, JPB);
-        for (int k = 0; k < in_batch; k++) {
-            const int f0 = __builtin_amdgcn_readlane(cur.f, FPJ * k);
-            if (f0 < 0) continue;
+    uint32_t t_next16 = 0;
+    auto start_clock = [&]() { t_next16 = ((uint32_t)__builtin_amdgcn_s_memrealtime() << 4) + (uint32_t)(((long long)wave * period16) / n_waves); };
+    auto job = [&](auto mode, const Rec &cur, int base, int k) {
+            constexpr int MODE = decltype(mode)::value;
+            int f0 = 0;
+            if constexpr (MODE == 1) { if (k >= q_mine || k * n_waves + wave >= n_jobs) return; }
+            else {
+                f0 = __builtin_amdgcn_readlane(cur.f, FPJ * k);
+                if (f0 < 0) return;
+            }
             const uint32_t a0 = (uint32_t)((base + k) * n_waves + wave) * CW_PIECE;
             const uint32_t a1 = min(a0 + CW_PIECE, total);
             const uint32_t win = a1 - a0;
@@ -1201,8 +1231,8 @@
                 pd = ((uint32_t)__builtin_amdgcn_ds_bpermute(from, (int)cur.p.x) & m_p0) | ((uint32_t)__builtin_amdgcn_ds_bpermute(from, (int)cur.p.y) & m_p1) |
                      ((uint32_t)__builtin_amdgcn_ds_bpermute(from, (int)cur.p.z) & m_p2) | ((uint32_t)__builtin_amdgcn_ds_bpermute(from, (int)cur.p.w) & m_p3);
             };
-            if (RASTER != 1) gather(0);
-            if (period16) {
+            if constexpr (MODE != 1 && RASTER != 1) gather(0);
+            if (MODE != 2 && period16) {
                 const uint32_t now16 = (uint32_t)__builtin_amdgcn_s_memrealtime() << 4;
                 const int wait16 = (int)(t_next16 - now16);
                 if (wait16 > 0) {
@@ -1211,11 +1241,14 @@
                 } else if (wait16 < -period16) t_next16 = now16 - (uint32_t)period16;
                 t_next16 += (uint32_t)(period16 + (base + k < CW_HEAD_JOBS ? head_extra16 : 0));
             }
-            uint8_t *const job = dst_base + a0;
-            if (win == CW_PIECE) {
+            if constexpr (MODE != 2) {
+                uint8_t *const piece = dst_base + a0;
+                if (win == CW_PIECE) {
 #pragma unroll
-                for (int s = 0; s < CW_PIECE_STORES; s++) *(uint4 *)(job + 1024 * s + 16 * lane) = make_uint4(0, 0, 0, 0);
-            } else piece_fill_partial(dst_base, a0, a1, lane);
+                    for (int s = 0; s < CW_PIECE_STORES; s++) *(uint4 *)(piece + 1024 * s + 16 * lane) = make_uint4(0, 0, 0, 0);
+                } else piece_fill_partial(dst_base, a0, a1, lane);
+            }
+            if constexpr (MODE == 1) return;
 #pragma unroll
             for (int pair = 0; pair < FPJ / 2; pair++) {
                 if (FPJ > 2 && pair > 0 && ((uint32_t)f0 + 2u * pair >= (uint32_t)env_n || ((uint32_t)f0 + 2u * pair) * FB >= a1)) break;
@@ -1269,18 +1302,101 @@
                     if (is_mark && aseg + 8u - a0 < win) dst_base[aseg + 8u] = (uint8_t)(o >> 16);
                 }
             }
-        }
+    };
+    Rec nxt;
+    int k_filled = 0;
+    if constexpr (!STEP) {
+        nxt = fetch(0);
+        start_clock();
+    } else {
+        extern __shared__ __attribute__((aligned(16))) unsigned char cw_step_lds[];
+        uint32_t *const s_mt = (uint32_t *)cw_step_lds + wave_in_block * CW_MT_WORDS;
+        CwPaintJob *const s_jobs = (CwPaintJob *)(cw_step_lds + CW_RESET_WAVES * CW_MT_WORDS * 4);
+        int *const s_njobs = (int *)(cw_step_lds + CW_RESET_WAVES * CW_MT_WORDS * 4 + CW_RESET_WAVES * CW_WAVE * 3 * 32), *const s_cnt = s_njobs + 1;
+        const int first = min(JPB, q_mine), front = min(sp.fills_front, first), back_to = min(front + sp.fills_back, first);
+        const Rec none{};
+        int painted = 0;
+        if (sp.dry) {
+            start_clock();
+            for (int k = 0; k < front; k++) job(CwJobMode<1>(), none, 0, k);
+        } else {
+            const int n_shares = ((P.n_envs + sp.epw - 1) / sp.epw + n_waves - 1) / n_waves;
+            for (int s = 0; s < n_shares; s++) {
+                if (s) __syncthreads();
+                auto fills = [&]() {
+                    if (s) return;
+                    start_clock();
+                    for (int k = 0; k < front; k++) job(CwJobMode<1>(), none, 0, k);
+                };
+                painted += sp.term ? fused_step<2, true, true>(P, sp.actions, sp.act_dtype, sp.epw, wave + s * n_waves, s_mt, s_jobs, s_njobs, s_cnt, s == 0, fills)
+                                   : fused_step<2, false, true>(P, sp.actions, sp.act_dtype, sp.epw, wave + s * n_waves, s_mt, s_jobs, s_njobs, s_cnt, s == 0, fills);
+            }
+        }
+        k_filled = front;
+        asm volatile("s_waitcnt vmcnt(0)" ::: "memory");
+        __syncthreads();
+        unsigned long long target = 0;
+        if (threadIdx.x == 0) {
+            const unsigned long long old = __hip_atomic_fetch_add(sp.sync, 1ull, __ATOMIC_RELAXED, __HIP_MEMORY_SCOPE_AGENT);
+            target = (old / gridDim.x + 1ull) * gridDim.x;
+        }
+        if (painted == 0) {
+            for (int k = front; k < back_to; k++) job(CwJobMode<1>(), none, 0, k);
+            k_filled = back_to;
+        }
+        if (threadIdx.x == 0) {
+            const unsigned long long t0 = __builtin_amdgcn_s_memrealtime();
+            bool gave_up = __hip_atomic_load(sp.sync + 16, __ATOMIC_RELAXED, __HIP_MEMORY_SCOPE_AGENT) != 0;
+            while (!gave_up && __hip_atomic_load(sp.sync, __ATOMIC_RELAXED, __HIP_MEMORY_SCOPE_AGENT) < target) {
+                __builtin_amdgcn_s_sleep(4);
+                if (__builtin_amdgcn_s_memrealtime() - t0 > (unsigned long long)sp.spin_ticks) {
+                    gave_up = true;
+                    __hip_atomic_store(sp.sync + 16, 1ull, __ATOMIC_RELAXED, __HIP_MEMORY_SCOPE_AGENT);
+                    if (sp.timeout_host) __hip_atomic_store(sp.timeout_host, 1u, __ATOMIC_RELAXED, __HIP_MEMORY_SCOPE_SYSTEM);
+                }
+            }
+            __builtin_amdgcn_fence(__ATOMIC_ACQUIRE, "agent");
+        }
+        asm volatile("s_waitcnt vmcnt(0)" ::: "memory");
+        __syncthreads();
+        if (src == CW_SRC_CURRENT) {
+            const unsigned long long d = __hip_atomic_load(P.counters + 1, __ATOMIC_RELAXED, __HIP_MEMORY_SCOPE_AGENT);
+            done_now = ((unsigned long long)__builtin_amdgcn_readfirstlane((uint32_t)(d >> 32)) << 32) | (uint32_t)__builtin_amdgcn_readfirstlane((uint32_t)d);
+            const unsigned long long finished = done_now - counters4;
+            const bool busy = finished >= CW_BUSY_FINISHED, storm = finished * 8ull >= (unsigned long long)P.n_envs;
+            const int quiet = period16;
+            period16 = storm ? sp.period16_busy : quiet;
+            head_extra16 = !storm ? (busy ? sp.period16_busy : sp.period16_head) - quiet : 0;
+        }
+        if (k_filled == 0) start_clock();
+        nxt = fetch(0);
+    }
+    for (int base = 0; base < q_mine; base += JPB) {
+        const Rec cur = nxt;
+        if (base + JPB < q_mine) nxt = fetch(base + JPB);
+        const int in_batch = min(q_mine - base, JPB);
+        int k = 0;
+        if constexpr (STEP) { if (base == 0) for (; k < k_filled; k++) job(CwJobMode<2>(), cur, base, k); }
+        for (; k < in_batch; k++) job(CwJobMode<0>(), cur, base, k);
     }
 }
 template <int RASTER, int FPJ>
 __global__ __launch_bounds__(256) void cw_render_pieces_kernel(CwParams P, uint8_t *frames, int src, int period16, int period16_head, int period16_busy,
-                                                               int chunk, int env_lo, int env_n)
-{
+                                                               int chunk, int env_lo, int env_n, CwStepPhase sp)
+{
+    if constexpr (FPJ == 2) if (sp.actions != nullptr || sp.dry) {
+        unsigned long long done_now = 0;
+        render_pieces<RASTER, FPJ, true>(P, frames, src, period16, (chunk & 1) ? period16_head - period16 : 0, env_lo, env_n, sp, P.counters[4], done_now);
+        if (src == CW_SRC_CURRENT && (chunk & 2) && blockIdx.x == 0 && threadIdx.x == 0) P.counters[4] = done_now;
+        return;
+    }
     const unsigned long long done_now = P.counters[1];
     const unsigned long long finished = src == CW_SRC_CURRENT ? done_now - P.counters[4] : (unsigned long long)P.n_envs;
     const bool busy = finished >= CW_BUSY_FINISHED, storm = finished * 8ull >= (unsigned long long)P.n_envs;
-    render_pieces<RASTER, FPJ>(P, frames, src, __builtin_amdgcn_readfirstlane(storm ? period16_busy : period16),
-                               __builtin_amdgcn_readfirstlane(!storm && (chunk & 1) ? (busy ? period16_busy : period16_head) - period16 : 0), env_lo, env_n);
+    unsigned long long unused = 0;
+    render_pieces<RASTER, FPJ, false>(P, frames, src, __builtin_amdgcn_readfirstlane(storm ? period16_busy : period16),
+                                      __builtin_amdgcn_readfirstlane(!storm && (chunk & 1) ? (busy ? period16_busy : period16_head) - period16 : 0), env_lo, env_n,
+                                      sp, 0ull, unused);
     if (src == CW_SRC_CURRENT && (chunk & 2) && blockIdx.x == 0 && threadIdx.x == 0) P.counters[4] = done_now;
 }
 #define CW_GATHER_MAX_S 9
@@ -1584,18 +1700,20 @@
     const int per_cu = small && pieces > 4ll * tn.n_cu * tn.small_blocks_per_cu ? tn.small_blocks_per_cu : 1;
     return cw_render_grid(tn, pieces) * per_cu;
 }
-typedef void (*CwSweepKernel)(CwParams, uint8_t *, int, int, int, int, int, int, int);
+typedef void (*CwSweepKernel)(CwParams, uint8_t *, int, int, int, int, int, int, int, CwStepPhase);
 static CwSweepKernel cw_sweep_kernel(int raster, int fpj)
 {
     if (raster == 1) return fpj <= 2 ? cw_render_pieces_kernel<1, 2> : fpj <= 4 ? cw_render_pieces_kernel<1, 4> : fpj <= 8 ? cw_render_pieces_kernel<1, 8> : cw_render_pieces_kernel<1, 16>;
     return fpj <= 2 ? cw_render_pieces_kernel<0, 2> : fpj <= 4 ? cw_render_pieces_kernel<0, 4> : fpj <= 8 ? cw_render_pieces_kernel<0, 8> : cw_render_pieces_kernel<0, 16>;
 }
-static void cw_launch_sweep(const CwParams &P, const CwTuning &tn, uint8_t *frames, int src, hipStream_t st)
+static int cw_envs_per_wave(int n, int most);
+static void cw_launch_sweep(const CwParams &P, const CwTuning &tn, uint8_t *frames, int src, hipStream_t st, const CwStepPhase *step = nullptr)
 {
     int per = 0;
     const int n_chunks = cw_piece_chunks(P, tn, &per);
     const CwSweepKernel k = cw_sweep_kernel(P.raster, cw_frames_per_job(P.frame_bytes));
     for (int c = 0; c < n_chunks; c++) {
+        const CwStepPhase sp = step && c == 0 ? *step : CwStepPhase{};
         const int env_n = min(per, P.n_envs - c * per);
         const long long pieces = ((long long)env_n * P.frame_bytes + CW_PIECE - 1) / CW_PIECE;
         if (cw_use_gather(P, tn)) {
@@ -1606,8 +1724,36 @@
                 hipLaunchKernelGGL(cw_render_gather_kernel<8>, dim3(grid), dim3(256), 0, st, P, frames, src, tn.period16, c * per, env_n);
             continue;
         }
-        hipLaunchKernelGGL(k, dim3(cw_sweep_blocks(P, tn, pieces)), dim3(256), 0, st, P, frames, src, tn.period16, tn.period16_head, tn.period16_busy, (c == 0 ? 1 : 0) | (c == n_chunks - 1 ? 2 : 0), c * per, env_n);
-    }
+        hipLaunchKernelGGL(k, dim3(cw_sweep_blocks(P, tn, pieces)), dim3(256), step && c == 0 ? CW_STEP_LDS_BYTES : 0, st, P, frames, src, tn.period16, tn.period16_head,
+                           tn.period16_busy, (c == 0 ? 1 : 0) | (c == n_chunks - 1 ? 2 : 0), c * per, env_n, sp);
+    }
+}
+static bool cw_one_launch_eligible(const CwParams &P, const CwTuning &tn, int obs_mode, int auto_reset, int host_mapped)
+{
+    if (obs_mode != 1 || !auto_reset || host_mapped || cw_use_gather(P, tn) || cw_frames_per_job(P.frame_bytes) != 2) return false;
+    if ((double)P.n_envs * P.frame_bytes < (double)(64ll << 20)) return false;
+    int per = 0;
+    cw_piece_chunks(P, tn, &per);
+    const long long pieces = ((long long)min(per, P.n_envs) * P.frame_bytes + CW_PIECE - 1) / CW_PIECE;
+    const int blocks = cw_sweep_blocks(P, tn, pieces);
+    return blocks == cw_render_grid(tn, pieces) && blocks <= tn.n_cu && pieces >= 4ll * blocks;
+}
+static CwStepPhase cw_step_phase(const CwParams &P, const CwTuning &tn, const void *actions, int act_dtype, int dry)
+{
+    CwStepPhase sp{};
+    sp.actions = actions;
+    sp.sync = tn.one_launch_sync;
+    sp.timeout_host = tn.one_launch_timeout_host;
+    sp.act_dtype = act_dtype;
+    sp.epw = cw_envs_per_wave(P.n_envs, tn.step_envs_per_wave);
+    sp.term = P.terminal_img != nullptr;
+    sp.fills_front = tn.one_launch_fills_front;
+    sp.fills_back = tn.one_launch_fills_back;
+    sp.dry = dry;
+    sp.spin_ticks = tn.one_launch_spin_ticks;
+    sp.period16_head = tn.period16_head;
+    sp.period16_busy = tn.period16_busy;
+    return sp;
 }
 
 static inline int cw_wave_blocks(int waves) { return (waves + CW_RESET_WAVES - 1) / CW_RESET_WAVES; }
@@ -1634,6 +1780,13 @@
     const CwTuning &tn = *T;
     const int n = P->n_envs;
     const bool ev_all = ev && obs_mode != 1;
+    if (tn.one_launch && tn.one_launch_sync && cw_one_launch_eligible(*P, tn, obs_mode, auto_reset, 0)) {
+        const CwStepPhase sp = cw_step_phase(*P, tn, actions, act_dtype, 0);
+        if (ev) for (int k = 2; k < 5; k++) (void)hipEventRecord(ev[k], st);
+        cw_launch_sweep(*P, tn, P->obs, CW_SRC_CURRENT, st, &sp);
+        if (ev) (void)hipEventRecord(ev[5], st);
+        return hipGetLastError();
+    }
     if (ev_all) (void)hipEventRecord(ev[0], st);
     if (auto_reset) {
         const int epw = cw_envs_per_wave(n, tn.step_envs_per_wave);
@@ -1721,8 +1874,16 @@
 
 hipError_t cwk_launch_sweep_calib(const CwParams *P, const CwTuning *T, hipStream_t st)
 {
-    cw_launch_sweep(*P, *T, P->obs, CW_SRC_CURRENT, st);
+    if (T->one_launch_dry && T->one_launch_sync) {
+        const CwStepPhase sp = cw_step_phase(*P, *T, nullptr, 0, 1);
+        cw_launch_sweep(*P, *T, P->obs, CW_SRC_CURRENT, st, &sp);
+    } else cw_launch_sweep(*P, *T, P->obs, CW_SRC_CURRENT, st);
     return hipGetLastError();
+}
+
+int cwk_one_launch_eligible(const CwParams *P, const CwTuning *T, int obs_mode, int auto_reset, int host_mapped)
+{
+    return cw_one_launch_eligible(*P, *T, obs_mode, auto_reset, host_mapped) ? 1 : 0;
 }
 
 __global__ void cw_idle_kernel(int n)
diff --git a/gym_craftingworld_amd/csrc/cw_layout.h b/gym_craftingworld_amd/csrc/cw_layout.h
--- a/gym_craftingworld_amd/csrc/cw_layout.h
+++ b/gym_craftingworld_amd/csrc/cw_layout.h
@@ -33,6 +33,13 @@
     long long small_launch_bytes = 320ll << 20;
     int step_envs_per_wave = 64;
     int reset_blocks_per_cu = 4;
+    int one_launch = 0;
+    int one_launch_fills_front = 0;
+    int one_launch_fills_back = 0;
+    int one_launch_dry = 0;
+    unsigned int one_launch_spin_ticks = 0;
+    unsigned long long *one_launch_sync = nullptr;
+    unsigned int *one_launch_timeout_host = nullptr;
 };
 
 struct CwResident {
diff --git a/gym_craftingworld_amd/vec_env.py b/gym_craftingworld_amd/vec_env.py
--- a/gym_craftingworld_amd/vec_env.py
+++ b/gym_craftingworld_amd/vec_env.py
@@ -473,6 +473,9 @@
     def render_kernel_name(self):
         return (self._lib.cw_render_kernel_name(self._h) or b'').decode()
 
+    def one_launch(self):
+        return bool(self._lib.cw_one_launch(self._h))
+
     def profile_end(self):
         p = L.cw_profile()
         L.check(self._lib.cw_profile_end(self._h, C.byref(p)), 'cw_profile_end', self._lib)
diff --git a/include/craftingworld.h b/include/craftingworld.h
--- a/include/craftingworld.h
+++ b/include/craftingworld.h
@@ -146,6 +146,7 @@
 int cw_profile_begin(cw_engine *e, int max_steps);
 int cw_profile_end(cw_engine *e, cw_profile *out);
 const char *cw_render_kernel_name(const cw_engine *e);
+int cw_one_launch(const cw_engine *e);
 
 typedef struct cw_tuner_state {
     int32_t period16, period16_head, period16_busy, lookahead, resident, guard_slowdowns;
```

Measured after the change: 301.7 million. -4.2%, worse.
